# DearCaat/MHIM-MIL

Hardware: AMD Instinct MI355X
Metric: patch-instances/sec through MHIM fwd+bwd, N=10k D=1024 (higher is better)
Workload: dtype f32; 1 GPU; c2: MHIM(ABMIL) train step, one bag N=10000 D=1024 per GPU per step (teacher fwd + select + student fwd + bwd + Adam + EMA); rotating_bags_per_gpu=8, matrix_core_form=bf16x3, parallelism=dp1, launch=hipGraph replay, one graph per resident bag

## Files before the change

include/mhimx.h:

```cpp
#ifndef MHIMX_H
#define MHIMX_H

#include <stdint.h>

#ifdef __cplusplus
extern "C" {
#endif

#define MHIMX_VERSION 620

enum { MHIMX_ACT_NONE = 0, MHIMX_ACT_RELU = 1, MHIMX_ACT_GELU = 2, MHIMX_ACT_TANH = 3 };

enum { MHIMX_PREC_F32 = 0, MHIMX_PREC_F16S = 1, MHIMX_PREC_BF16X3 = 2 };

const char* mhimx_last_error(void);
int mhimx_version(void);


typedef struct {
  const float* A; int64_t lda; const int64_t* rows;
  const float* B; int64_t ldb;
  float* C; int64_t ldc;
  int64_t M, N, K;
  const float* bias;
  const float* rowv; const float* colv;
  float* pre; int64_t ldpre;
  int32_t act;
  float drop_p; uint64_t drop_seed; const uint8_t* drop_mask;
  int32_t accumulate;
  int32_t prec;
  const uint64_t* drop_tick;
  int32_t paired;
  float* ws; int64_t ws_floats;
  float* dact; int64_t lddact;
} mhimx_gemm_nt_args;
int mhimx_gemm_nt(void* stream, const mhimx_gemm_nt_args* a);

#define MHIMX_PROJ_MAX_HEADS 2
typedef struct {
  const float* wp;
  const float* bias;
  float* H; int64_t ldh;
  void* dact;
  float drop_p; uint64_t drop_seed; const uint8_t* drop_mask;
  const float* resid; int64_t ldr;
} mhimx_proj_head;
typedef struct {
  const float* wa16;
  const float* wc;
  int32_t act;
  int32_t C;
  float* s;
  float* cproj;
  float* pm; float* pl; float* pz;
  float* xch;
  uint32_t* gate;
} mhimx_proj_score;
int mhimx_pool_finalize(void* stream, const float* pm, const float* pl, const float* pz, int64_t G, int64_t E, float* stats, float* z,
                        const float* s, const float* cproj, const float* bp, int64_t C, int64_t M1, float* pscore);
int64_t mhimx_proj_score_parts(int64_t N);
int64_t mhimx_proj_score_xch_floats(int64_t N);
typedef struct {
  const float* X; int64_t ldx;
  int64_t N, D, E;
  int32_t act;
  int32_t n_heads;
  mhimx_proj_head head[MHIMX_PROJ_MAX_HEADS];
  const uint64_t* drop_tick;
  const mhimx_proj_score* score0;
} mhimx_bag_project_args;
int mhimx_bag_project(void* stream, const mhimx_bag_project_args* a);
int mhimx_bag_project_multi(void* stream, const mhimx_bag_project_args* bags, int32_t n_bags);

int mhimx_gemm_nn(void* stream, const mhimx_gemm_nt_args* a, float alpha, int32_t splits, float* ws );
int mhimx_gemm_batched(void* stream, int32_t mode, const mhimx_gemm_nt_args* args, int32_t batch, int64_t strideA,
                       int64_t strideB, int64_t strideC, float alpha, int32_t splits, float* ws);
int mhimx_bmm_affine(void* stream, int32_t mode, const mhimx_gemm_nt_args* args, int32_t batch, int64_t strideA, int64_t strideB,
                     int64_t strideC, float alpha, float ident);
int mhimx_bmm_affine2(void* stream, int32_t mode, const mhimx_gemm_nt_args* a, int32_t batch, int64_t strideA, int64_t strideB,
                      int64_t strideC, float alpha, float ident, float* C2, float alpha2, float ident2);
typedef struct {
  const void* A; const void* B; float* C; void* PN; void* PT; void* PN2; void* PT2; const float* D; const float* D2;
  float alpha, ident, alpha2, ident2, dscale, d2scale;
  int32_t kind;
} mhimx_bmm_step;
int mhimx_bmm_chain(void* stream, const mhimx_bmm_step* steps, int32_t stages, int32_t groups, uint32_t* counters);
int mhimx_bmm_affine_pair(void* stream, int32_t mode0, const mhimx_gemm_nt_args* a0, float alpha0, float ident0, int32_t mode1,
                          const mhimx_gemm_nt_args* a1, float alpha1, float ident1, int32_t batch, int64_t stride);

typedef struct {
  int32_t kind; int32_t accumulate;
  const float* parts; float* out;
  int64_t G, W, ld, K1, K2, ldo;
} mhimx_reduce_job;
#define MHIMX_REDUCE_MAX 16
#define MHIMX_SIDE_BYTES 512
typedef struct { int32_t pending; int32_t reserved; unsigned char blob[MHIMX_SIDE_BYTES]; } mhimx_side_work;
typedef struct { int32_t pending; int32_t reserved ;
                 unsigned char blob[128]; } mhimx_parked_gemm;
typedef struct { mhimx_reduce_job j[MHIMX_REDUCE_MAX]; int32_t n; mhimx_side_work side; mhimx_parked_gemm parked; mhimx_side_work pre; } mhimx_reduce_list;
int mhimx_reduce_flush(void* stream, mhimx_reduce_list* list);

typedef struct {
  const float* A; int64_t lda;
  const float* B; int64_t ldb; const int64_t* rows;
  float* C; int64_t ldc;
  int64_t M, K1, K2;
  int32_t splits; float* ws;
  int32_t accumulate;
  int32_t prec;
  int64_t ws_floats;
  mhimx_reduce_list* defer;
} mhimx_gemm_tn_args;
int mhimx_gemm_tn(void* stream, const mhimx_gemm_tn_args* a);

int mhimx_pair_planes(void* stream, const float* x, int64_t ldx, int64_t M, int64_t K, float* out);

#define MHIMX_PREP_MAX 32
typedef struct { int32_t kind; const float* in; float* out; int64_t R, C; } mhimx_prep_job;
int mhimx_prep_batch(void* stream, const mhimx_prep_job* jobs, int32_t n);

int mhimx_transpose(void* stream, const float* in, float* out, int64_t R, int64_t C);

typedef struct {
  int64_t E;
  int64_t A;
  int32_t act;
  int32_t gated;
  int32_t prec;
  const float* wa; const float* ba;
  const float* wb; const float* bb;
  const float* wc; const float* bc;
  const float* wa_frag;
  float gate_drop_p;
  uint64_t gate_drop_seed;
} mhimx_scorer;

typedef struct {
  const float* T1; int64_t M1; const float* T2; int64_t M2;
  float* s; float* stats; float* z;
  float* u_pre;
  const float* wp; int64_t C; float* cproj;
  void* ws; int64_t ws_bytes;
  const float* bp; float* pscore;
  const int64_t* rows1;
  const uint8_t* excl;
  const mhimx_prep_job* ride_jobs;
  int32_t n_ride_jobs;
  int32_t phase; int32_t tail_tokens;
  const void* ride_merge;
  const float* ride_X; int64_t ride_R; void* ride_ws; int64_t ride_ws_bytes;
  int32_t rode_merge;
  const float* tail_wa_t;
  int64_t tail_row0;
  int32_t no_backward;
} mhimx_pool_io;
int64_t mhimx_abmil_pool_ws_bytes(int64_t M, int64_t E, int64_t A, int32_t gated);
int mhimx_abmil_pool_fwd(void* stream, const mhimx_scorer* sc, mhimx_pool_io* io);

typedef struct {
  const float* g_z;
  float* dT1; float* dT2;
  float* d_wa; float* d_ba; float* d_wb; float* d_bb; float* d_wc; float* d_bc;
  const float* wa_t; const float* wb_t;
  int32_t accumulate;
  int32_t splits;
  mhimx_reduce_list* defer;
  const float* wa_t_frag;
  void* img; const void* img_dact; float* img_part; int64_t img_rows;
} mhimx_pool_grad;
int mhimx_abmil_pool_bwd(void* stream, const mhimx_scorer* sc, const mhimx_pool_io* io, const mhimx_pool_grad* g);

int mhimx_softmax_from_stats(void* stream, const float* s, const float* stats, float* attn, int64_t M);

int mhimx_lse_merge(void* stream, const float* parts, int64_t W, int64_t E, float* stats, float* z);

int mhimx_pseudo_score(void* stream, const float* s, const float* stats, const float* cproj, const float* bp,
                       float* score, float* attn_out, int64_t M, int64_t C);

int mhimx_layernorm_fwd(void* stream, const float* x, int64_t M, int64_t E, const float* w, const float* b, float* y, float* mean,
                        float* rstd);
int mhimx_layernorm_bwd(void* stream, const float* dy, const float* x, int64_t M, int64_t E, const float* w, const float* mean,
                        const float* rstd, float* dx, float* d_w, float* d_b, int32_t accumulate, float* ws);
int mhimx_layernorm_bwd_res(void* stream, const float* dy, const float* x, int64_t M, int64_t E, const float* w, const float* mean,
                            const float* rstd, const float* resid, float* dx, float* d_w, float* d_b, int32_t accumulate, float* ws);
int mhimx_dropout_apply(void* stream, const float* x, float* out, int64_t M, int64_t E, float p, uint64_t seed, const uint64_t* tick);
int mhimx_dropout_apply_proj(void* stream, const float* x, float* out, int64_t M, int64_t E, float p, uint64_t seed, const uint64_t* tick);
int mhimx_softmax_rows(void* stream, const float* x, float* y, int64_t R, int64_t L, float alpha);
int mhimx_softmax_rows_bwd(void* stream, const float* y, const float* dy, float* dx, int64_t R, int64_t L, float alpha);
int mhimx_landmark_mean(void* stream, const float* x, int64_t ldx, int64_t T, int64_t l, int64_t C, float* out);
int mhimx_landmark_mean_bwd(void* stream, const float* dout, int64_t T, int64_t l, int64_t C, float* dx, int64_t ldx, int32_t accumulate);
int mhimx_affine_ident(void* stream, const float* x, float* y, int64_t B, int64_t n, float a, float b);
int mhimx_axpby(void* stream, const float* x, float* y, int64_t n, float alpha, float beta);
int mhimx_pinv_init(void* stream, const float* a, int64_t B, int64_t n, float* z, float* stats, float* ws);
int mhimx_pinv_init_bwd(void* stream, const float* dz, const float* z0, const float* stats, int64_t B, int64_t n, float* da, float* ws);
int mhimx_resconv(void* stream, const float* v, int64_t ldv, const float* w, int64_t KS, int64_t dh, int64_t T, int64_t C, float* out,
                  int64_t ldo, int32_t accumulate, int32_t flip);
int64_t mhimx_resconv_dw_ws_floats(int64_t T, int64_t C, int64_t dh, int64_t KS);
int mhimx_resconv_dw(void* stream, const float* dout, int64_t ldo, const float* v, int64_t ldv, int64_t KS, int64_t dh, int64_t T,
                     int64_t C, float* dw, float* ws);
typedef struct mhimx_nys {
  const float* q; const float* k; const float* v;
  int64_t ld, T;
  const float* ql; const float* kl;
  int64_t ldl;
  float scale;
  float* ws;
  int64_t ws_floats;
} mhimx_nys;
int64_t mhimx_nys_ws_floats(int64_t T);
int mhimx_nys_a3v_fwd(void* stream, const mhimx_nys* a, float* a3v, float* lse3);
int mhimx_nys_out_fwd(void* stream, const mhimx_nys* a, const float* w2, float* out, int64_t ldo, float* lse1, int32_t accumulate);
int mhimx_nys_out_bwd(void* stream, const mhimx_nys* a, const float* w2, const float* dout, int64_t ldd, const float* lse1,
                      float* delta1, float* dq, int64_t lddq, float* dkl, int64_t lddl, float* dw2);
int mhimx_nys_a3v_bwd(void* stream, const mhimx_nys* a, const float* a3v, const float* da3v, const float* lse3, float* dk, float* dv,
                      int64_t lddk, int32_t accumulate_dv, float* dql, int64_t lddl);
int mhimx_nys_cls_attn(void* stream, const mhimx_nys* a, const float* lse3, const float* u, float* r);
int64_t mhimx_bn_ws_floats(int64_t M, int64_t C);
int mhimx_bn_fwd(void* stream, const float* x, int64_t M, int64_t C, const float* w, const float* b, float eps, int32_t training, float* mean,
                 float* rstd, float* var_out, float* y, float* ws);
int mhimx_bn_bwd(void* stream, const float* dy, const float* x, int64_t M, int64_t C, const float* w, const float* mean, const float* rstd,
                 int32_t training, float* dx, float* dw, float* db, float* ws);
int mhimx_sincos_add(void* stream, const float* x, const int64_t* pos_xy, int64_t N, int64_t C, float* out);
int mhimx_ppeg_combine(void* stream, const float* w7, const float* w5, const float* w3, const float* b7, const float* b5,
                       const float* b3, int64_t C, float* wc, float* bc);
int mhimx_ppeg_fwd(void* stream, const float* x, int64_t N, int64_t C, const float* wc, const float* bc, float* y,
                   int64_t grid );
int64_t mhimx_ppeg_bwd_ws_floats(int64_t N, int64_t C);
int mhimx_ppeg_bwd(void* stream, const float* dy, const float* x, int64_t N, int64_t C, const float* wc, float* dx, float* dwc, float* dbc,
                   float* ws, int64_t grid);
typedef struct { int64_t H, cell0, ncell, out0, out1; } mhimx_ppeg_band;
int64_t mhimx_ppeg_side(int64_t N, int64_t* wrapN);
int mhimx_ppeg_band_fwd(void* stream, const float* xb, const mhimx_ppeg_band* band, int64_t C, const float* wc, const float* bc, float* y);
int64_t mhimx_ppeg_band_bwd_ws_floats(int64_t n_out, int64_t C);
int mhimx_ppeg_band_bwd(void* stream, const float* dyb, const float* xb, const mhimx_ppeg_band* band, int64_t n_dw, int64_t C, const float* wc,
                        float* dx, float* dwc, float* dbc, float* ws);
int mhimx_scale_heads(void* stream, const float* v, int64_t ldv, const float* a, int64_t lda, int64_t dh, int64_t T, int64_t C, float* out);

int64_t mhimx_select_ws_bytes(int64_t N);
int mhimx_select_mask(void* stream, const float* score, int64_t N, int64_t k, int64_t n_sel, int32_t largest,
                      const int64_t* perm, const int64_t* other, int64_t n_other,
                      int64_t* mask_ids, int64_t* len_keep_dev, int64_t* topk_sorted ,
                      void* ws, int64_t ws_bytes);

int mhimx_select_rows(void* stream, const float* score, int64_t N, int64_t k, int64_t n_sel, int32_t largest,
                      uint64_t rand_seed, const uint64_t* tick, int64_t merge_R, int64_t* rows_out, int64_t* mask_ids,
                      void* ws, int64_t ws_bytes, int32_t merge_first );

int mhimx_select_rows_img(void* stream, const float* score, int64_t N, int64_t k, int64_t n_sel, int32_t largest, uint64_t rand_seed,
                          const uint64_t* tick, int64_t merge_R, int64_t* rows_out, int64_t* rows_img, int64_t img_merge_off, void* ws,
                          int64_t ws_bytes, int32_t merge_first);
int mhimx_vote_scores(void* stream, const float* attn, int64_t H, int64_t N, int64_t k, int32_t largest,
                      float* vote, void* ws, int64_t ws_bytes);

int mhimx_compose_ids(void* stream, const int64_t* a, const int64_t* b, int64_t* out, int64_t n);
int mhimx_random_perm(void* stream, int64_t n, uint64_t seed, const uint64_t* tick, const int64_t* src, int64_t* out);

typedef struct { int64_t row0, N, k, n_sel, merge_R, out0; uint64_t seed; } mhimx_select_bag;
int64_t mhimx_select_rows_many_ws_bytes(int32_t n_bags, const mhimx_select_bag* bags);
int mhimx_select_rows_many(void* stream, const float* score, int32_t n_bags, const mhimx_select_bag* bags, const uint64_t* tick,
                           int64_t* rows_out, void* ws, int64_t ws_bytes, int32_t merge_first);

typedef struct {
  int64_t E; int64_t k;
  int64_t heads; int64_t dim_head;
  const float* q_param;
  const float* ln_w; const float* ln_b;
  const float* wkv; const float* wq; const float* wo; const float* bo;
  const float* wkv_t; const float* wq_t; const float* wo_t;
  float mm;
  float drop_p; uint64_t drop_seed;
  int32_t prec;
  const uint64_t* drop_tick;
  const float* wkv_frag;
  const int64_t* x_rows;
  int32_t prepared;
  int64_t own_lo, own_n;
  float rep;
  int32_t rows_done;
} mhimx_merge;
int64_t mhimx_merge_ws_bytes(int64_t R, int64_t E, int64_t k, int64_t heads, int64_t dim_head);
int mhimx_merge_fwd(void* stream, const mhimx_merge* m, const float* X, int64_t R, float* z, float* q_new,
                    int32_t update_q, void* ws, int64_t ws_bytes);
typedef struct {
  float* d_ln_w; float* d_ln_b; float* d_wkv; float* d_wq; float* d_wo; float* d_bo;
  int32_t accumulate; int32_t splits;
  mhimx_reduce_list* defer;
} mhimx_merge_grad;
int64_t mhimx_merge_part_floats(void);
int mhimx_merge_fwd_part(void* stream, const mhimx_merge* m, const float* X, int64_t R, float* part, void* ws, int64_t ws_bytes);
int mhimx_merge_fwd_finish(void* stream, const mhimx_merge* m, const float* parts, int32_t W, int64_t R, float* z, float* q_new,
                           int32_t update_q, void* ws, int64_t ws_bytes);
int mhimx_merge_bwd(void* stream, const mhimx_merge* m, const float* X, int64_t R, const float* dz, float* dX,
                    const mhimx_merge_grad* g, void* ws, int64_t ws_bytes);
int mhimx_merge_bwd_park(const mhimx_merge* m, const float* X, int64_t R, const float* dz, float* dX, const mhimx_merge_grad* g, void* ws,
                         int64_t ws_bytes);

int mhimx_act_bwd(void* stream, float* dH, const float* H, const float* pre, int64_t M, int64_t E, int32_t act,
                  float drop_p, uint64_t drop_seed, const uint8_t* drop_mask, const int64_t* rows, float* colsum_out,
                  int32_t accumulate, void* ws, int64_t ws_bytes, const uint64_t* drop_tick);
int mhimx_mul_colsum(void* stream, float* dH, const float* dact, int64_t M, int64_t E, float* colsum_out, int32_t accumulate,
                     void* ws, int64_t ws_bytes, mhimx_reduce_list* defer );
int mhimx_rows_dpre(void* stream, const float* dH, const void* dact16, const int64_t* rows, int64_t L, int64_t E, float* dpre,
                    float* colsum_out, int32_t accumulate, void* ws, int64_t ws_bytes, mhimx_reduce_list* defer );
int64_t mhimx_wgrad_image_bytes(int64_t L, int64_t E);
int mhimx_rows_dpre_image(void* stream, const float* dH, const void* dact16, const int64_t* rows, int64_t L, int64_t E, void* img,
                          float* colsum_out, int32_t accumulate, void* ws, int64_t ws_bytes, mhimx_reduce_list* defer );
int mhimx_rows_dpre_image_c(void* stream, const float* dH_compact, const void* dact16, const int64_t* rows, int64_t L, int64_t E, void* img,
                            float* colsum_out, int32_t accumulate, void* ws, int64_t ws_bytes, mhimx_reduce_list* defer );
int mhimx_rows_dpre_image_k(void* stream, const float* dH, const void* dact16, const uint8_t* keep, int64_t N, int64_t E, void* img,
                            float* colsum_out, int32_t accumulate, void* ws, int64_t ws_bytes, mhimx_reduce_list* defer );
typedef struct {
  const void* img;
  const float* X; int64_t ldx; int64_t n_bag_rows;
  const int64_t* rows;
  int64_t L, E, D;
  float* C; int64_t ldc; int32_t accumulate;
  float* ws; int64_t ws_floats;
  mhimx_reduce_list* defer;
  int32_t ride_tail;
  const void* ximg;
} mhimx_bag_wgrad_args;
int64_t mhimx_wgrad_ws_floats(int64_t L, int64_t E, int64_t D);
int mhimx_bag_wgrad(void* stream, const mhimx_bag_wgrad_args* a);
int64_t mhimx_wgrad_multi_ws_floats(int64_t L, int64_t E, int64_t D, int32_t n_bags);
int mhimx_bag_wgrad_multi(void* stream, const mhimx_bag_wgrad_args* bags, int32_t n_bags);
int mhimx_shard_flags(void* stream, const int64_t* rows_all, int64_t R, int64_t Lk, int64_t lo, int64_t n, int64_t k_tokens,
                      int32_t tokens_live, uint8_t* excl);
int mhimx_shard_gather(void* stream, const float* H, int64_t E, const int64_t* rows, int64_t R, int64_t lo, int64_t n, float* out);
int mhimx_shard_scatter(void* stream, const float* dX, int64_t E, const int64_t* rows, int64_t R, int64_t lo, int64_t n, float* dH);
int mhimx_colsum(void* stream, const float* X, int64_t M, int64_t E, float* out, int32_t accumulate,
                 void* ws, int64_t ws_bytes);

int mhimx_head_fwd_bwd(void* stream, const float* z, const float* t, const float* wp, const float* bp,
                       const int64_t* label_dev, int64_t E, int64_t C, float temp_t, float main_alpha,
                       float aux_alpha, float inv_accum, float* logits, float* losses, float* g_z, float* d_wp,
                       float* d_bp, int32_t accumulate, const float* g_logits_in, const float* g_cl_in);

int mhimx_softmax_cols(void* stream, const float* x, float* y, int64_t M, int64_t C, float alpha);
int mhimx_softmax_cols_bwd(void* stream, const float* y, const float* dy, float* dx, int64_t M, int64_t C, float alpha);
int mhimx_colmax(void* stream, const float* x, int64_t M, int64_t C, float* vals, int64_t* idx);
int mhimx_rowmax(void* stream, const float* x, int64_t M, int64_t C, float* out);
int mhimx_dsmil_head(void* stream, const float* logits_bag, const float* logits_ins, const int64_t* label_dev, const float* Bs,
                     const float* Bt, int64_t C, int64_t V, float temp_t, float main_alpha, float aux_alpha, float inv_accum,
                     float* losses, float* g_logits_bag, float* g_logits_ins, float* g_B, const float* g_cl_in);

int mhimx_adam_ema(void* stream, float* p, const float* g, float* m, float* v, float* teacher, int64_t n_train,
                   int64_t n_all, int64_t step, float lr, float beta1, float beta2, float eps, float weight_decay,
                   float grad_scale, float ema_mm, int32_t zero_grad ,
                   const uint64_t* step_dev ,
                   const float* mm_table, int64_t mm_len );

typedef struct {
  float* p; float* g; float* m; float* v; float* teacher;
  int64_t n_train, n_all;
  int64_t step; const uint64_t* step_dev;
  float lr; const float* lr_table; int64_t lr_len;
  float beta1, beta2, eps, weight_decay, grad_scale;
  float ema_mm; const float* mm_table; int64_t mm_len;
  int32_t zero_grad;
  const float* g_extra; int64_t n_extra; int64_t extra_pitch;
  float clip_norm;
  float* ws; int64_t ws_floats;
  mhimx_reduce_list* fold;
  int64_t extra_lo;
  int32_t extra_only;
} mhimx_optim_args;
int mhimx_optim_step(void* stream, const mhimx_optim_args* a);

#define MHIMX_STEP_MAX_ROWS 262144
#define MHIMX_WINDOW_MAX 8
typedef struct {
  const float* w1; const float* b1;
  const float* wa; const float* wc;
  const float* wp; const float* bp;
  float* q;
  const float* ln_w; const float* ln_b;
  const float* wkv; const float* wq; const float* wo; const float* bo;
} mhimx_step_params;
typedef struct {
  float* w1; float* b1; float* wa; float* wc; float* wp; float* bp; float* ln_w; float* ln_b; float* wkv; float* wq; float* wo; float* bo;
} mhimx_step_grads;
typedef struct {
  int64_t D, E, A, C, k;
  int32_t act, da_act;
  int32_t attn2score;
  float drop_p_teacher, drop_p_student;
  float merge_drop_p, merge_mm;
  float temp_t, main_alpha, aux_alpha;
  mhimx_step_params student, teacher;
  mhimx_step_grads grad;
  float* p; float* g; float* m; float* v; float* p_teacher;
  int64_t n_train, n_all;
  float lr, beta1, beta2, eps, weight_decay, ema_mm;
  const float* mm_table; int64_t mm_len; const float* lr_table; int64_t lr_len;
  uint64_t* tick; uint64_t* opt_step;
  float* q_out;
  int32_t time_project;
  void* side_stream;
} mhimx_step_cfg;
typedef struct { int64_t k_top, n_sel, len_keep, Lk, R; } mhimx_step_counts;
int mhimx_step_counts_of(int64_t N, double mask_ratio_h, double mask_ratio_hr, double merge_ratio, mhimx_step_counts* out);
typedef struct { uint64_t drop_teacher, drop_student, select, mca; } mhimx_step_seeds;
typedef struct {
  int64_t total;
  int64_t logits, losses;
  int64_t score;
  int64_t rows_all;
  int64_t H_teacher, H_student;
  int64_t dact;
  int64_t z_teacher, z_student, g_z;
  int64_t dH;
} mhimx_step_layout;
int mhimx_step_layout_of(const mhimx_step_cfg* cfg, int64_t N, const mhimx_step_counts* cnt, mhimx_step_layout* out);
int mhimx_step_run(void* stream, const mhimx_step_cfg* cfg, const float* X, int64_t ldx, int64_t N, const int64_t* label_dev,
                   const mhimx_step_counts* cnt, const mhimx_step_seeds* seeds, int64_t host_step, void* ws, int64_t ws_bytes, int32_t update);
int mhimx_step_project_ms(float* ms_out, float* empty_ms_out, int32_t cap);
int mhimx_step_run_many(void* stream, const mhimx_step_cfg* cfg, int32_t n_bags, const float* const* X, const int64_t* ldx, const int64_t* N,
                        const int64_t* const* labels_dev, const mhimx_step_counts* cnt, const mhimx_step_seeds* seeds, int64_t host_step0,
                        void* ws, int64_t ws_bytes);

int mhimx_pure_step_layout_of(const mhimx_step_cfg* cfg, int64_t N, mhimx_step_layout* out);
int mhimx_pure_step_run(void* stream, const mhimx_step_cfg* cfg, const float* X, int64_t ldx, int64_t N, const int64_t* label_dev,
                        uint64_t drop_seed, int64_t host_step, void* ws, int64_t ws_bytes, int32_t update);
int mhimx_pure_step_run_many(void* stream, const mhimx_step_cfg* cfg, int32_t n_bags, const float* const* X, const int64_t* ldx, const int64_t* N,
                             const int64_t* const* labels_dev, const uint64_t* drop_seeds, int64_t host_step0, void* ws, int64_t ws_bytes);

typedef struct { int64_t total, bag0, bag_stride, grad_slab; mhimx_step_layout bag; } mhimx_window_layout;
int mhimx_window_layout_of(const mhimx_step_cfg* cfg, int32_t n_bags, int64_t N, const mhimx_step_counts* cnt, mhimx_window_layout* out);
int mhimx_window_run(void* stream, const mhimx_step_cfg* cfg, int32_t n_bags, const float* const* X, int64_t ldx, int64_t N,
                     const int64_t* const* labels_dev, const mhimx_step_counts* cnt, const mhimx_step_seeds* seeds, int64_t host_step, void* ws,
                     int64_t ws_bytes, int32_t update);
// ... 266 lines not shown
```

mhim_mil_amd/_lib.py:

```python
from __future__ import annotations

import ctypes as C
import os

HERE = os.path.dirname(os.path.abspath(__file__))
LIB_PATH = os.path.join(HERE, os.environ.get("MHIMX_LIB_NAME", "libmhimx.so"))

c_f32p = C.c_void_p
c_i64p = C.c_void_p
c_u8p = C.c_void_p

ABI_VERSION = 620

ACT = {None: 0, "none": 0, "identity": 0, "relu": 1, "gelu": 2, "tanh": 3}
PREC = {"f32": 0, "f16s": 1, "bf16x3": 2}


def act_code(name, allowed):
    n = name.lower() if isinstance(name, str) else None
    return ACT[n] if n in allowed else 0


class GemmNT(C.Structure):
    _fields_ = [("A", c_f32p), ("lda", C.c_int64), ("rows", c_i64p),
                ("B", c_f32p), ("ldb", C.c_int64),
                ("C", c_f32p), ("ldc", C.c_int64),
                ("M", C.c_int64), ("N", C.c_int64), ("K", C.c_int64),
                ("bias", c_f32p), ("rowv", c_f32p), ("colv", c_f32p),
                ("pre", c_f32p), ("ldpre", C.c_int64),
                ("act", C.c_int32),
                ("drop_p", C.c_float), ("drop_seed", C.c_uint64), ("drop_mask", c_u8p),
                ("accumulate", C.c_int32), ("prec", C.c_int32), ("drop_tick", C.c_void_p),
                ("paired", C.c_int32), ("ws", C.c_void_p), ("ws_floats", C.c_int64),
                ("dact", C.c_void_p), ("lddact", C.c_int64)]


class ProjHead(C.Structure):
    _fields_ = [("wp", c_f32p), ("bias", c_f32p), ("H", c_f32p), ("ldh", C.c_int64), ("dact", C.c_void_p),
                ("drop_p", C.c_float), ("drop_seed", C.c_uint64), ("drop_mask", c_u8p), ("resid", c_f32p), ("ldr", C.c_int64)]


class ProjScore(C.Structure):
    _fields_ = [("wa16", c_f32p), ("wc", c_f32p), ("act", C.c_int32), ("C", C.c_int32), ("s", c_f32p), ("cproj", c_f32p),
                ("pm", c_f32p), ("pl", c_f32p), ("pz", c_f32p), ("xch", c_f32p), ("gate", C.c_void_p)]


class BagProject(C.Structure):
    _fields_ = [("X", c_f32p), ("ldx", C.c_int64), ("N", C.c_int64), ("D", C.c_int64), ("E", C.c_int64),
                ("act", C.c_int32), ("n_heads", C.c_int32), ("head", ProjHead * 2), ("drop_tick", C.c_void_p), ("score0", C.c_void_p)]


class BagWgrad(C.Structure):
    _fields_ = [("img", C.c_void_p), ("X", c_f32p), ("ldx", C.c_int64), ("n_bag_rows", C.c_int64), ("rows", C.c_void_p),
                ("L", C.c_int64), ("E", C.c_int64), ("D", C.c_int64), ("C", c_f32p), ("ldc", C.c_int64), ("accumulate", C.c_int32),
                ("ws", c_f32p), ("ws_floats", C.c_int64), ("defer", C.c_void_p), ("ride_tail", C.c_int32), ("ximg", C.c_void_p)]


class PpegBand(C.Structure):
    _fields_ = [("H", C.c_int64), ("cell0", C.c_int64), ("ncell", C.c_int64), ("out0", C.c_int64), ("out1", C.c_int64)]


class PrepJob(C.Structure):
    _fields_ = [("kind", C.c_int32), ("inp", C.c_void_p), ("out", C.c_void_p), ("R", C.c_int64), ("C", C.c_int64)]


class ReduceJob(C.Structure):
    _fields_ = [("kind", C.c_int32), ("accumulate", C.c_int32), ("parts", c_f32p), ("out", c_f32p),
                ("G", C.c_int64), ("W", C.c_int64), ("ld", C.c_int64), ("K1", C.c_int64), ("K2", C.c_int64), ("ldo", C.c_int64)]


REDUCE_MAX = 16


SIDE_BYTES = 512


class SideWork(C.Structure):
    _fields_ = [("pending", C.c_int32), ("reserved", C.c_int32), ("blob", C.c_ubyte * SIDE_BYTES)]


class ParkedGemm(C.Structure):
    _fields_ = [("pending", C.c_int32), ("reserved", C.c_int32), ("blob", C.c_ubyte * 128)]


class ReduceListC(C.Structure):
    _fields_ = [("j", ReduceJob * REDUCE_MAX), ("n", C.c_int32), ("side", SideWork), ("parked", ParkedGemm), ("pre", SideWork)]


class GemmTN(C.Structure):
    _fields_ = [("A", c_f32p), ("lda", C.c_int64),
                ("B", c_f32p), ("ldb", C.c_int64), ("rows", c_i64p),
                ("C", c_f32p), ("ldc", C.c_int64),
                ("M", C.c_int64), ("K1", C.c_int64), ("K2", C.c_int64),
                ("splits", C.c_int32), ("ws", c_f32p),
                ("accumulate", C.c_int32), ("prec", C.c_int32), ("ws_floats", C.c_int64),
                ("defer", C.c_void_p)]


class Scorer(C.Structure):
    _fields_ = [("E", C.c_int64), ("A", C.c_int64), ("act", C.c_int32), ("gated", C.c_int32), ("prec", C.c_int32),
                ("wa", c_f32p), ("ba", c_f32p), ("wb", c_f32p), ("bb", c_f32p), ("wc", c_f32p), ("bc", c_f32p),
                ("wa_frag", c_f32p), ("gate_drop_p", C.c_float), ("gate_drop_seed", C.c_uint64)]


class PoolIO(C.Structure):
    _fields_ = [("T1", c_f32p), ("M1", C.c_int64), ("T2", c_f32p), ("M2", C.c_int64),
                ("s", c_f32p), ("stats", c_f32p), ("z", c_f32p), ("u_pre", c_f32p),
                ("wp", c_f32p), ("C", C.c_int64), ("cproj", c_f32p),
                ("ws", C.c_void_p), ("ws_bytes", C.c_int64), ("bp", c_f32p), ("pscore", c_f32p), ("rows1", c_i64p),
                ("excl", C.c_void_p), ("ride_jobs", C.c_void_p), ("n_ride_jobs", C.c_int32),
                ("phase", C.c_int32), ("tail_tokens", C.c_int32), ("ride_merge", C.c_void_p), ("ride_X", c_f32p), ("ride_R", C.c_int64),
                ("ride_ws", C.c_void_p), ("ride_ws_bytes", C.c_int64), ("rode_merge", C.c_int32), ("tail_wa_t", c_f32p), ("tail_row0", C.c_int64),
                ("no_backward", C.c_int32)]


class PoolGrad(C.Structure):
    _fields_ = [("g_z", c_f32p), ("dT1", c_f32p), ("dT2", c_f32p),
                ("d_wa", c_f32p), ("d_ba", c_f32p), ("d_wb", c_f32p), ("d_bb", c_f32p), ("d_wc", c_f32p),
                ("d_bc", c_f32p), ("wa_t", c_f32p), ("wb_t", c_f32p),
                ("accumulate", C.c_int32), ("splits", C.c_int32), ("defer", C.c_void_p), ("wa_t_frag", c_f32p),
                ("img", C.c_void_p), ("img_dact", C.c_void_p), ("img_part", c_f32p), ("img_rows", C.c_int64)]


class Merge(C.Structure):
    _fields_ = [("E", C.c_int64), ("k", C.c_int64), ("heads", C.c_int64), ("dim_head", C.c_int64),
                ("q_param", c_f32p), ("ln_w", c_f32p), ("ln_b", c_f32p),
                ("wkv", c_f32p), ("wq", c_f32p), ("wo", c_f32p), ("bo", c_f32p),
                ("wkv_t", c_f32p), ("wq_t", c_f32p), ("wo_t", c_f32p),
                ("mm", C.c_float), ("drop_p", C.c_float), ("drop_seed", C.c_uint64), ("prec", C.c_int32), ("drop_tick", C.c_void_p),
                ("wkv_frag", c_f32p), ("x_rows", c_i64p), ("prepared", C.c_int32), ("own_lo", C.c_int64), ("own_n", C.c_int64),
                ("rep", C.c_float), ("rows_done", C.c_int32)]


class MergeGrad(C.Structure):
    _fields_ = [("d_ln_w", c_f32p), ("d_ln_b", c_f32p), ("d_wkv", c_f32p), ("d_wq", c_f32p), ("d_wo", c_f32p),
                ("d_bo", c_f32p), ("accumulate", C.c_int32), ("splits", C.c_int32), ("defer", C.c_void_p)]


_P = C.c_void_p
_I64 = C.c_int64
_I32 = C.c_int32
_F = C.c_float
_U64 = C.c_uint64


class Nys(C.Structure):
    _fields_ = [("q", C.c_void_p), ("k", C.c_void_p), ("v", C.c_void_p), ("ld", C.c_int64), ("T", C.c_int64),
                ("ql", C.c_void_p), ("kl", C.c_void_p), ("ldl", C.c_int64), ("scale", C.c_float),
                ("ws", C.c_void_p), ("ws_floats", C.c_int64)]


class BmmStep(C.Structure):
    _fields_ = [("A", C.c_void_p), ("B", C.c_void_p), ("C", C.c_void_p), ("PN", C.c_void_p), ("PT", C.c_void_p),
                ("PN2", C.c_void_p), ("PT2", C.c_void_p), ("D", C.c_void_p), ("D2", C.c_void_p), ("alpha", C.c_float), ("ident", C.c_float),
                ("alpha2", C.c_float), ("ident2", C.c_float), ("dscale", C.c_float), ("d2scale", C.c_float), ("kind", C.c_int32)]


class OptimArgs(C.Structure):
    _fields_ = [("p", C.c_void_p), ("g", C.c_void_p), ("m", C.c_void_p), ("v", C.c_void_p), ("teacher", C.c_void_p),
                ("n_train", C.c_int64), ("n_all", C.c_int64), ("step", C.c_int64), ("step_dev", C.c_void_p),
                ("lr", C.c_float), ("lr_table", C.c_void_p), ("lr_len", C.c_int64),
                ("beta1", C.c_float), ("beta2", C.c_float), ("eps", C.c_float), ("weight_decay", C.c_float), ("grad_scale", C.c_float),
                ("ema_mm", C.c_float), ("mm_table", C.c_void_p), ("mm_len", C.c_int64), ("zero_grad", C.c_int32),
                ("g_extra", C.c_void_p), ("n_extra", C.c_int64), ("extra_pitch", C.c_int64), ("clip_norm", C.c_float),
                ("ws", C.c_void_p), ("ws_floats", C.c_int64), ("fold", C.c_void_p), ("extra_lo", C.c_int64), ("extra_only", C.c_int32)]


class StepParams(C.Structure):
    _fields_ = [(n, C.c_void_p) for n in ("w1", "b1", "wa", "wc", "wp", "bp", "q", "ln_w", "ln_b", "wkv", "wq", "wo", "bo")]


class StepGrads(C.Structure):
    _fields_ = [(n, C.c_void_p) for n in ("w1", "b1", "wa", "wc", "wp", "bp", "ln_w", "ln_b", "wkv", "wq", "wo", "bo")]


class StepCfg(C.Structure):
    _fields_ = [("D", C.c_int64), ("E", C.c_int64), ("A", C.c_int64), ("C", C.c_int64), ("k", C.c_int64),
                ("act", C.c_int32), ("da_act", C.c_int32), ("attn2score", C.c_int32),
                ("drop_p_teacher", C.c_float), ("drop_p_student", C.c_float), ("merge_drop_p", C.c_float), ("merge_mm", C.c_float),
                ("temp_t", C.c_float), ("main_alpha", C.c_float), ("aux_alpha", C.c_float),
                ("student", StepParams), ("teacher", StepParams), ("grad", StepGrads),
                ("p", C.c_void_p), ("g", C.c_void_p), ("m", C.c_void_p), ("v", C.c_void_p), ("p_teacher", C.c_void_p),
                ("n_train", C.c_int64), ("n_all", C.c_int64),
                ("lr", C.c_float), ("beta1", C.c_float), ("beta2", C.c_float), ("eps", C.c_float), ("weight_decay", C.c_float), ("ema_mm", C.c_float),
                ("mm_table", C.c_void_p), ("mm_len", C.c_int64), ("lr_table", C.c_void_p), ("lr_len", C.c_int64),
                ("tick", C.c_void_p), ("opt_step", C.c_void_p), ("q_out", C.c_void_p), ("time_project", C.c_int32), ("side_stream", C.c_void_p)]


class StepCounts(C.Structure):
    _fields_ = [("k_top", C.c_int64), ("n_sel", C.c_int64), ("len_keep", C.c_int64), ("Lk", C.c_int64), ("R", C.c_int64)]


class StepSeeds(C.Structure):
    _fields_ = [("drop_teacher", C.c_uint64), ("drop_student", C.c_uint64), ("select", C.c_uint64), ("mca", C.c_uint64)]


class StepLayout(C.Structure):
    _fields_ = [(n, C.c_int64) for n in ("total", "logits", "losses", "score", "rows_all", "H_teacher", "H_student", "dact", "z_teacher",
                                        "z_student", "g_z", "dH")]


class WindowLayout(C.Structure):
    _fields_ = [("total", C.c_int64), ("bag0", C.c_int64), ("bag_stride", C.c_int64), ("grad_slab", C.c_int64), ("bag", StepLayout)]


WINDOW_MAX = 8
STEP_MAX_ROWS = 262144


class InferCfg(C.Structure):
    _fields_ = [("D", C.c_int64), ("E", C.c_int64), ("A", C.c_int64), ("C", C.c_int64), ("act", C.c_int32), ("da_act", C.c_int32),
                ("p", StepParams)]


class InferBag(C.Structure):
    _fields_ = [("X", c_f32p), ("ldx", C.c_int64), ("N", C.c_int64)]


class InferOut(C.Structure):
    _fields_ = [(n, c_f32p) for n in ("logits", "z", "stats", "score", "attn", "loss")]


class InferDsmilCfg(C.Structure):
    _fields_ = [("D", C.c_int64), ("E", C.c_int64), ("C", C.c_int64), ("act", C.c_int32), ("cls_attn", C.c_int32), ("no_norm", C.c_int32),
                ("pad", C.c_int32)] + [(n, c_f32p) for n in ("w1", "b1", "wi", "bi", "wq0", "bq0", "wq2", "bq2", "wv", "bv", "wfcc", "bfcc")]


class InferDsmilOut(C.Structure):
    _fields_ = [(n, c_f32p) for n in ("logits_bag", "logits_ins", "logits", "B")] + [("crit", C.c_void_p)] + [(n, c_f32p) for n in ("attn", "loss")]


INFER_MAX = 32


class TransmilLayer(C.Structure):
    _fields_ = [(n, c_f32p) for n in ("ln_w", "ln_b", "w_qkv", "w_out", "b_out", "conv_w")]


class InferTransmilCfg(C.Structure):
    _fields_ = ([("D", C.c_int64), ("C", C.c_int64), ("act", C.c_int32), ("pad", C.c_int32)]
                + [(n, c_f32p) for n in ("w1", "b1", "cls_token")] + [("layer", TransmilLayer * 2)]
                + [(n, c_f32p) for n in ("w7", "w5", "w3", "b7", "b5", "b3", "norm_w", "norm_b", "wp", "bp")])


class InferTransmilLayout(C.Structure):
    _fields_ = ([("n_bags", C.c_int64), ("tokens", C.c_int64)] + [(n, C.c_int64 * INFER_MAX) for n in ("tok0", "T", "pad")]
                + [(n, C.c_int64 * 2) for n in ("x", "qkv", "lm", "a2", "z", "a3v", "lse3", "w2", "out", "y")]
                + [("cls", C.c_int64), ("total", C.c_int64)])
INFER_MAX_ROWS = 4194304
X_F32, X_F16, X_BF16 = 0, 1, 2

TOPK_MAX_K = 4096

SURV_MAX_N = 16777216
CINDEX_MAX_N = 4194304
CINDEX_MAX_B = 65535
CINDEX_MAX_BN = 134217728


class TopkSeg(C.Structure):
    _fields_ = [("row0", C.c_int64), ("N", C.c_int64)]


class SelectBag(C.Structure):
    _fields_ = [(n, C.c_int64) for n in ("row0", "N", "k", "n_sel", "merge_R", "out0")] + [("seed", C.c_uint64)]


PURE_WINDOW_MAX = 32
PURE_WINDOW_MAX_ROWS = 524288


class PureWindowBag(C.Structure):
    _fields_ = [("X", c_f32p), ("ldx", C.c_int64), ("N", C.c_int64), ("label_dev", C.c_void_p), ("drop_seed", C.c_uint64)]


class PureWindowLayout(C.Structure):
    _fields_ = [(n, C.c_int64) for n in ("total", "rows", "logits", "losses", "H", "dact", "s", "stats", "z", "g_z")] + [
        ("row0", C.c_int64 * PURE_WINDOW_MAX)]


DSMIL_WINDOW_MAX = 32
DSMIL_WINDOW_MAX_ROWS = 262144
_DSMIL_NAMES = ("w1", "b1", "wi", "bi", "wq0", "bq0", "wq2", "bq2", "wv", "bv", "wfcc", "bfcc")

# ... 247 lines not shown
```

mhim_mil_amd/csrc/mca2.hip:

```cpp
#include <math.h>
#include <string.h>

#include "mca2_rows.hpp"

namespace mhimx {

int64_t merge2_part_floats() { return M2_PART_FLOATS; }
int64_t merge2_rows_tiles(int64_t R) { return cdiv(R, m2_tile_rows(R)); }
int64_t merge2_ws_bytes(int64_t R, int64_t k) {
  Arena ar(nullptr, 0);
  return merge2_ws_layout(ar, R, k, nullptr);
}

bool merge2_ok(const mhimx_merge* m, int64_t R) {
  return m->E == M2_E && m->heads == M2_H && m->dim_head == M2_DH && m->k >= 1 && m->heads * m->k <= M2_JP && R >= 1 && R <= 32768 &&
         m->prec != MHIMX_PREC_F32 && aligned16(m->wq) && aligned16(m->wkv) && aligned16(m->wo) && aligned16(m->ln_w) && aligned16(m->ln_b) &&
         aligned16(m->q_param);
}

__global__ __launch_bounds__(M2_THREADS) void merge2_prep_kernel(Merge2PrepArgs a) {
  __shared__ __attribute__((aligned(16))) float lds[6 * M2_E + 6 * 64];
  merge2_prep_body((int)blockIdx.x, lds, a.q_param, a.ln_w, a.ln_b, a.wq, a.wkv, a.k, a.scale, a.w);
}

template <int RT>
__global__ __launch_bounds__(M2_THREADS) void merge2_rows_fwd_kernel(const float* __restrict__ X, const int64_t* __restrict__ xrows, int64_t R,
                                                                    const float* __restrict__ ln_w, const float* __restrict__ ln_b, int J,
                                                                    float drop_p, uint64_t seed0, const uint64_t* __restrict__ tick, Merge2Ws w, BagBatch bb) {
  extern __shared__ __attribute__((aligned(16))) float m2sm[];
  if (blockIdx.z) {
    MHIMX_BAG(X); MHIMX_BAG(xrows);
    seed0 = bag_mca_seed(seed0, bb);
    bag_move(w, bb);
  }
  merge2_rows_fwd_body<RT>((int)blockIdx.x, m2sm, X, xrows, R, ln_w, ln_b, J, drop_p, seed0, tick, w);
}

template <int MODE>
__global__ __launch_bounds__(M2_THREADS) void merge2_partials_kernel(M2Parts in, int live_only, const float* __restrict__ ln_w,
                                                                    const float* __restrict__ ln_b, float* __restrict__ out,
                                                                    float* __restrict__ stats, float* __restrict__ raw_stats, BagBatch bb) {
  __shared__ float lds[M2_PARTIALS_LDS];
  if (blockIdx.z) {
    in.pm = bag_ptr(in.pm, bb); in.pl = bag_ptr(in.pl, bb); in.psd = bag_ptr(in.psd, bb); in.y = bag_ptr(in.y, bb);
    MHIMX_BAG(out); MHIMX_BAG(stats); MHIMX_BAG(raw_stats);
  }
  merge2_partials_body<MODE>((int)blockIdx.x, lds, in, live_only != 0, ln_w, ln_b, out, stats, raw_stats);
}

__global__ __launch_bounds__(M2_THREADS) void merge2_o_kernel(const float* __restrict__ wkv, int k, Merge2Ws w, BagBatch bb) {
  __shared__ __attribute__((aligned(16))) float ys[6 * M2_E];
  bag_move(w, bb);
  const int tid = threadIdx.x;
  const int h = blockIdx.x >> 2, qd = blockIdx.x & 3;
  M2HeadRows wr;
  m2_head_rows_load<16>(wkv + (int64_t)(M2_I + h * 64 + qd * 16) * M2_E, wr);
  m2_zero_tail(ys, k);
  for (int idx = tid; idx < k * (M2_E / 4); idx += M2_THREADS)
    reinterpret_cast<m2_f4*>(ys)[idx] = reinterpret_cast<const m2_f4*>(w.Y + (int64_t)h * k * M2_E)[idx];
  __syncthreads();
  m2_head_dots_use<16>(wr, ys, k, nullptr, 16, w.O + h * 64 + qd * 16);
}

__global__ __launch_bounds__(M2_THREADS) void merge2_bwd_pre_kernel(const float* __restrict__ dz, const float* __restrict__ wo_t,
                                                                   const float* __restrict__ wkv, int k, float drop_p, uint64_t seed0,
                                                                   const uint64_t* __restrict__ tick, float* __restrict__ d_bo, int accumulate,
                                                                   Merge2Ws w, float rep, BagBatch bb) {
  __shared__ __attribute__((aligned(16))) float lds[M2_BWD_PRE_LDS];
  if (blockIdx.z) {
    MHIMX_BAG(dz); MHIMX_BAG(wo_t); MHIMX_BAG(d_bo);
    seed0 = bag_mca_seed(seed0, bb);
    bag_move(w, bb);
  }
  merge2_bwd_pre_body((int)blockIdx.x, lds, dz, wo_t, wkv, k, drop_p, seed0, tick, d_bo, accumulate, w, rep);
}

template <int RT>
__global__ __launch_bounds__(M2_THREADS) void merge2_rows_bwd_kernel(const float* __restrict__ X, const int64_t* __restrict__ xrows, int64_t R,
                                                                    const float* __restrict__ ln_w, const float* __restrict__ ln_b, int J,
                                                                    float drop_p, uint64_t seed0, const uint64_t* __restrict__ tick,
                                                                    float* __restrict__ dX, Merge2Ws w, BagBatch bb) {
  extern __shared__ __attribute__((aligned(16))) float m2sm[];
  if (blockIdx.z) {
    MHIMX_BAG(X); MHIMX_BAG(xrows); MHIMX_BAG(dX);
    seed0 = bag_mca_seed(seed0, bb);
    bag_move(w, bb);
  }
  merge2_rows_bwd_body<RT>((int)blockIdx.x, m2sm, X, xrows, R, ln_w, ln_b, J, drop_p, seed0, tick, dX, w);
}

__global__ __launch_bounds__(M2_THREADS) void merge2_grads1_kernel(Merge2Side a, BagBatch bb) {
  __shared__ __attribute__((aligned(16))) float lds[M2_GRADS1_LDS];
  bag_move(a, bb);
  merge2_grads1_body((int)blockIdx.x, lds, a);
}

__global__ __launch_bounds__(M2_THREADS) void merge2_grads2_kernel(Merge2Side a, BagBatch bb) {
  __shared__ __attribute__((aligned(16))) float lds[M2_GRADS2_LDS];
  bag_move(a, bb);
  merge2_grads2_body((int)blockIdx.x, lds, a);
}

int mca_out(hipStream_t st, const float* O, const float* wo, const float* bo, int k, int E, int I, float p, uint64_t seed0, const uint64_t* tick,
            float* z, const float* q, float* q_new, float mm);
int reduce_parts2(hipStream_t st, const float* part0, const float* part1, int G, int W, int ld, float* out0, float* out1, int accumulate);

int merge2_side_launch(hipStream_t st, int stage, const Merge2Side& sd) {
  if (stage == 1) hipLaunchKernelGGL(merge2_partials_kernel<0>, bgrid((unsigned)(sd.J * 4)), dim3(M2_THREADS), 0, st, m2_parts_tiles(sd.w, sd.w.upart),
                                     sd.w.own_n > 0 ? 1 : 0, sd.ln_w, sd.ln_b, const_cast<float*>(sd.U), (float*)nullptr, (float*)nullptr, cur_batch());
  else if (stage == 2) hipLaunchKernelGGL(merge2_grads1_kernel, bgrid(M2_GRADS1_BLOCKS), dim3(M2_THREADS), 0, st, sd, cur_batch());
  else hipLaunchKernelGGL(merge2_grads2_kernel, bgrid(M2_GRADS2_BLOCKS), dim3(M2_THREADS), 0, st, sd, cur_batch());
  MHIMX_LAUNCH_CHECK();
  return 0;
}
int merge2_side_finish(hipStream_t st, mhimx_side_work* side, int upto_stage) {
  Merge2Side sd;
  while (side->pending != 0 && side->pending <= upto_stage) {
    memcpy(&sd, side->blob, sizeof(sd));
    if (int r = merge2_side_launch(st, side->pending, sd)) return r;
    side->pending = side->pending == 3 ? 0 : side->pending + 1;
  }
  return 0;
}

int merge2_fwd_rows_args(const mhimx_merge* m, const float* X, int64_t R, void* ws, int64_t ws_bytes, M2RowsFwd* out) {
  if (!m || !X || !merge2_ok(m, R) || !m->prepared || m->own_n != 0) return 1;
  Arena ar(ws, ws_bytes);
  Merge2Ws w;
  merge2_ws_layout(ar, R, m->k, &w);
  MHIMX_CHECK_ARG(ar.ok(), "merge rows rider: workspace too small (%lld < %lld)", (long long)ws_bytes, (long long)ar.off);
  if (w.rt != 16) return 1;
  w.own_lo = 0; w.own_n = 0;
  *out = M2RowsFwd{X, m->x_rows, R, m->ln_w, m->ln_b, M2_H * (int)m->k, m->drop_p, m->drop_seed, m->drop_tick, w};
  return 0;
}

static int merge2_fwd_rows(hipStream_t st, const mhimx_merge* m, const float* X, int64_t R, void* ws, int64_t ws_bytes, Merge2Ws* wout) {
  Arena ar(ws, ws_bytes);
  Merge2Ws w;
  merge2_ws_layout(ar, R, m->k, &w);
  MHIMX_CHECK_ARG(ar.ok(), "merge_fwd: workspace too small (%lld < %lld)", (long long)ws_bytes, (long long)ar.off);
  MHIMX_CHECK_ARG(m->own_n >= 0 && (m->own_n == 0 || m->x_rows), "merge_fwd: a shard's row range needs the bag-level row list (x_rows)");
  w.own_lo = m->own_n > 0 ? m->own_lo : 0;
  w.own_n = m->own_n;
  const int k = (int)m->k, J = M2_H * k;
  const float scale = 1.0f / sqrtf((float)M2_DH);
  if (m->rows_done) {
    *wout = w;
    return 0;
  }
  if (!m->prepared) {
    hipLaunchKernelGGL(merge2_prep_kernel, dim3(64), dim3(M2_THREADS), 0, st, Merge2PrepArgs{m->q_param, m->ln_w, m->ln_b, m->wq, m->wkv, k, scale, w});
    MHIMX_LAUNCH_CHECK();
  }
  MHIMX_ONCE_PER_DEVICE(MHIMX_HIP(hipFuncSetAttribute((const void*)merge2_rows_fwd_kernel<32>, hipFuncAttributeMaxDynamicSharedMemorySize, (int)m2_fwd_smem(32)));
                        MHIMX_HIP(hipFuncSetAttribute((const void*)merge2_rows_fwd_kernel<16>, hipFuncAttributeMaxDynamicSharedMemorySize, (int)m2_fwd_smem(16))));
  if (w.rt == 16)
    hipLaunchKernelGGL(merge2_rows_fwd_kernel<16>, bgrid((unsigned)w.T), dim3(M2_THREADS), m2_fwd_smem(16), st, X, m->x_rows, R, m->ln_w, m->ln_b, J, m->drop_p,
                       m->drop_seed, m->drop_tick, w, cur_batch());
  else
    hipLaunchKernelGGL(merge2_rows_fwd_kernel<32>, bgrid((unsigned)w.T), dim3(M2_THREADS), m2_fwd_smem(32), st, X, m->x_rows, R, m->ln_w, m->ln_b, J, m->drop_p,
                       m->drop_seed, m->drop_tick, w, cur_batch());
  MHIMX_LAUNCH_CHECK();
  *wout = w;
  return 0;
}
static int merge2_fwd_tail(hipStream_t st, const mhimx_merge* m, float* z, float* q_new, int update_q, const Merge2Ws& w) {
  const int k = (int)m->k;
  hipLaunchKernelGGL(merge2_o_kernel, bgrid(M2_H * 4), dim3(M2_THREADS), 0, st, m->wkv, k, w, cur_batch());
  MHIMX_LAUNCH_CHECK();
  return mca_out(st, w.O, m->wo, m->bo, k, M2_E, M2_I, m->drop_p, m->drop_seed + 0x9E3779B97F4A7C15ull, m->drop_tick, z, m->q_param,
                 update_q ? q_new : (float*)nullptr, m->mm);
}

int merge2_fwd(hipStream_t st, const mhimx_merge* m, const float* X, int64_t R, float* z, float* q_new, int update_q, void* ws, int64_t ws_bytes) {
  MHIMX_CHECK_ARG(!update_q || q_new, "merge_fwd: update_q needs q_new");
  MHIMX_CHECK_ARG(m->own_n == 0, "merge_fwd: a shard of an instance-sharded bag runs mhimx_merge_fwd_part + mhimx_merge_fwd_finish");
  Merge2Ws w;
  if (int r = merge2_fwd_rows(st, m, X, R, ws, ws_bytes, &w)) return r;
  const int J = M2_H * (int)m->k;
  hipLaunchKernelGGL(merge2_partials_kernel<1>, bgrid((unsigned)(J * 4)), dim3(M2_THREADS), 0, st, m2_parts_tiles(w, w.ypart), 0, m->ln_w, m->ln_b, w.Y,
                     w.stats, (float*)nullptr, cur_batch());
  MHIMX_LAUNCH_CHECK();
  return merge2_fwd_tail(st, m, z, q_new, update_q, w);
}

int merge2_fwd_part(hipStream_t st, const mhimx_merge* m, const float* X, int64_t R, float* part, void* ws, int64_t ws_bytes) {
  MHIMX_CHECK_ARG(part && aligned16(part), "merge_fwd_part: null / unaligned output block");
  Merge2Ws w;
  if (int r = merge2_fwd_rows(st, m, X, R, ws, ws_bytes, &w)) return r;
  const int J = M2_H * (int)m->k;
  hipLaunchKernelGGL(merge2_partials_kernel<2>, dim3((unsigned)(J * 4)), dim3(M2_THREADS), 0, st, m2_parts_tiles(w, w.ypart), 0, m->ln_w, m->ln_b,
                     part + 3 * M2_JP, (float*)nullptr, part, BagBatch{});
  MHIMX_LAUNCH_CHECK();
  return 0;
}
int merge2_fwd_finish(hipStream_t st, const mhimx_merge* m, const float* parts, int W, int64_t R, float* z, float* q_new, int update_q, void* ws,
                      int64_t ws_bytes) {
  MHIMX_CHECK_ARG(parts && W >= 1 && W <= 256 && z, "merge_fwd_finish: 1..256 shard blocks");
  MHIMX_CHECK_ARG(!update_q || q_new, "merge_fwd_finish: update_q needs q_new");
  Arena ar(ws, ws_bytes);
  Merge2Ws w;
  merge2_ws_layout(ar, R, m->k, &w);
  MHIMX_CHECK_ARG(ar.ok(), "merge_fwd_finish: workspace too small");
  const int J = M2_H * (int)m->k;
  hipLaunchKernelGGL(merge2_partials_kernel<1>, dim3((unsigned)(J * 4)), dim3(M2_THREADS), 0, st, m2_parts_shards(parts, W), 0, m->ln_w, m->ln_b, w.Y,
                     w.stats, (float*)nullptr, BagBatch{});
  MHIMX_LAUNCH_CHECK();
  return merge2_fwd_tail(st, m, z, q_new, update_q, w);
}

int gemm_tn_rider(hipStream_t st, const mhimx_gemm_tn_args& g, const Merge2Side* rider, int stage);

static int merge2_side_of(const mhimx_merge* m, const float* X, int64_t R, const float* dz, float* dX, const mhimx_merge_grad* gr, void* ws,
                          int64_t ws_bytes, Merge2Side* out) {
  Arena ar(ws, ws_bytes);
  Merge2Ws w;
  merge2_ws_layout(ar, R, m->k, &w);
  MHIMX_CHECK_ARG(ar.ok(), "merge_bwd: workspace too small");
  MHIMX_CHECK_ARG(m->own_n >= 0 && (m->own_n == 0 || m->x_rows), "merge_bwd: a shard's row range needs the bag-level row list (x_rows)");
  w.own_lo = m->own_n > 0 ? m->own_lo : 0;
  w.own_n = m->own_n;
  MHIMX_CHECK_ARG(m->wo_t && aligned16(m->wo_t), "merge_bwd: transposed to_out weight missing");
  const int k = (int)m->k, J = M2_H * k;
  Merge2Side sd = {};
  sd.w = w; sd.dz = dz; sd.U = w.aq; sd.ln_w = m->ln_w; sd.ln_b = m->ln_b; sd.wkv = m->wkv; sd.wq = m->wq; sd.q_param = m->q_param; sd.wo_t = m->wo_t;
  sd.d_wkv = gr->d_wkv; sd.d_wo = gr->d_wo; sd.d_wq = gr->d_wq; sd.d_ln_w = gr->d_ln_w; sd.d_ln_b = gr->d_ln_b; sd.d_bo = gr->d_bo; sd.tick = m->drop_tick;
  sd.oseed = m->drop_seed + 0x9E3779B97F4A7C15ull; sd.scale = 1.0f / sqrtf((float)M2_DH); sd.drop_p = m->drop_p; sd.k = k; sd.accumulate = gr->accumulate;
  sd.J = J;
  sd.rep = m->own_n > 0 ? m->rep : 1.f;
  sd.X = X; sd.xrows = m->x_rows; sd.R = R; sd.dX = dX; sd.seed0 = m->drop_seed;
  *out = sd;
  return 0;
}

int merge2_bwd_park(const mhimx_merge* m, const float* X, int64_t R, const float* dz, float* dX, const mhimx_merge_grad* gr, void* ws, int64_t ws_bytes) {
  if (!gr->defer || gr->defer->pre.pending != 0) return 0;
  Merge2Side sd;
  if (int r = merge2_side_of(m, X, R, dz, dX, gr, ws, ws_bytes, &sd)) return r;
  static_assert(sizeof(Merge2Side) <= sizeof(gr->defer->pre.blob), "Merge2Side must fit mhimx_reduce_list.pre");
  memcpy(gr->defer->pre.blob, &sd, sizeof(sd));
  gr->defer->pre.pending = 1;
  return 0;
}

int merge2_bwd(hipStream_t st, const mhimx_merge* m, const float* X, int64_t R, const float* dz, float* dX, const mhimx_merge_grad* gr, void* ws,
               int64_t ws_bytes) {
  Merge2Side sd;
  if (int r = merge2_side_of(m, X, R, dz, dX, gr, ws, ws_bytes, &sd)) return r;
  const Merge2Ws& w = sd.w;
  const int k = sd.k, J = sd.J;
  const int acc = gr->accumulate;
  const uint64_t oseed = sd.oseed;
  bool pre_done = false, rows_done = false;
  if (gr->defer && gr->defer->pre.pending) {
    pre_done = gr->defer->pre.pending == 2;
    gr->defer->pre.pending = 0;
  }
  if (gr->defer && gr->defer->parked.pending) {
    mhimx_gemm_tn_args pg;
    memcpy(&pg, gr->defer->parked.blob, sizeof(pg));
    gr->defer->parked.pending = 0;
    if (pre_done) {
      const int rc = gemm_tn_rider(st, pg, &sd, 4);
      if (rc < 0) return rc;
      rows_done = rc == 1;
    } else {
      const int rc = gemm_tn_rider(st, pg, pre_done ? nullptr : &sd, 0);
      if (rc < 0) return rc;
      pre_done = pre_done || rc == 1;
    }
  }
  if (!pre_done) {
    hipLaunchKernelGGL(merge2_bwd_pre_kernel, bgrid(M2_BWD_PRE_BLOCKS), dim3(M2_THREADS), 0, st, dz, m->wo_t, m->wkv, k, m->drop_p, oseed, m->drop_tick, gr->d_bo, acc, w, sd.rep, cur_batch());
    MHIMX_LAUNCH_CHECK();
  }
  if (!rows_done) {
    MHIMX_ONCE_PER_DEVICE(MHIMX_HIP(hipFuncSetAttribute((const void*)merge2_rows_bwd_kernel<32>, hipFuncAttributeMaxDynamicSharedMemorySize, (int)m2_bwd_smem(32)));
                          MHIMX_HIP(hipFuncSetAttribute((const void*)merge2_rows_bwd_kernel<16>, hipFuncAttributeMaxDynamicSharedMemorySize, (int)m2_bwd_smem(16))));
    if (w.rt == 16)
      hipLaunchKernelGGL(merge2_rows_bwd_kernel<16>, bgrid((unsigned)w.T), dim3(M2_THREADS), m2_bwd_smem(16), st, X, m->x_rows, R, m->ln_w, m->ln_b, J, m->drop_p,
                         m->drop_seed, m->drop_tick, dX, w, cur_batch());
    else
      hipLaunchKernelGGL(merge2_rows_bwd_kernel<32>, bgrid((unsigned)w.T), dim3(M2_THREADS), m2_bwd_smem(32), st, X, m->x_rows, R, m->ln_w, m->ln_b, J, m->drop_p,
                         m->drop_seed, m->drop_tick, dX, w, cur_batch());
    MHIMX_LAUNCH_CHECK();
  }
  if (gr->defer && gr->defer->side.pending == 0) {
    memcpy(gr->defer->side.blob, &sd, sizeof(sd));
    gr->defer->side.pending = 1;
  } else {
    for (int stage = 1; stage <= 3; ++stage)
      if (int r = merge2_side_launch(st, stage, sd)) return r;
  }
  return 0;
}

}

namespace mhimx {
int merge2_prep_args(const mhimx_merge* m, int64_t R, void* ws, int64_t ws_bytes, Merge2PrepArgs* out) {
  MHIMX_CHECK_ARG(m && merge2_ok(m, R), "prep_batch: the Merge preparation job needs the projection-free form (E = 512, 8 x 64, k <= 6, R <= 32768)");
  Arena ar(ws, ws_bytes);
  Merge2Ws w;
  merge2_ws_layout(ar, R, m->k, &w);
  MHIMX_CHECK_ARG(ar.ok(), "prep_batch: Merge workspace too small (%lld < %lld)", (long long)ws_bytes, (long long)ar.off);
  *out = Merge2PrepArgs{m->q_param, m->ln_w, m->ln_b, m->wq, m->wkv, (int)m->k, 1.0f / sqrtf((float)M2_DH), w};
  return 0;
}
}
```

mhim_mil_amd/csrc/rows.hip:

```cpp
#include <math.h>
#include <string.h>

#include "mca2_rows.hpp"
#include "reduce_jobs.hpp"

namespace mhimx {

int gemm_nt(hipStream_t st, const mhimx_gemm_nt_args& g);
int gemm_tn(hipStream_t st, const mhimx_gemm_tn_args& g);
bool scorer_fused_ok(int64_t E, int64_t A, int gated, int prec, const float* T, const float* wa, const float* wp, int64_t C);
int scorer_fused_fwd(hipStream_t st, const float* T, int64_t M, const float* wa, const float* wa_frag, const float* ba, int act, const float* wc,
                     const float* bc, const float* wp, int C, float* u_pre, float* s_out, float* cproj, float* pm, float* pl,
                     float* pz, int max_parts, const int64_t* rows, const uint8_t* excl, const mhimx_prep_job* ride_jobs, int n_ride_jobs,
                     const void* merge_rows);
int merge2_fwd_rows_args(const mhimx_merge* m, const float* X, int64_t R, void* ws, int64_t ws_bytes, M2RowsFwd* out);
int prep_batch(hipStream_t st, const mhimx_prep_job* jobs, int n);
int scorer_fused_bwd(hipStream_t st, const float* T, int64_t M, const float* u_pre, const float* s_in, const float* stats,
                     const float* g_z, const float* z, const float* wc, int act, const float* wa_t, const float* wa_t_frag, float* du,
                     float* dT, float* dwc_part, float* dbc_part, int max_parts, const int64_t* rows, const void* pre_side, int64_t gate_row0,
                     void* img, const void* img_dact, float* img_part, int64_t img_rows);

constexpr int ROWS_THREADS = 256;
constexpr int MAX_PART = 512;
constexpr int TN_SLABS = 128;

MHIMX_DEV float sigmoidf_(float x) { return 1.f / (1.f + __expf(-x)); }

constexpr int FWD_WAVES = 16;
template <int EPL>
__global__ __launch_bounds__(64 * FWD_WAVES) void score_rows_fwd_kernel(
    const float* __restrict__ T, int64_t M, int E, int A, int act, int gated, const float* __restrict__ u_pre,
    const float* __restrict__ wc, const float* __restrict__ bc, const float* __restrict__ wp, int C,
    float* __restrict__ s_out, float* __restrict__ cproj, float* __restrict__ pm, float* __restrict__ pl,
    float* __restrict__ pz, float gdrop_p, uint64_t gdrop_seed, int64_t row0 ) {
  extern __shared__ __attribute__((aligned(16))) float sm[];
  constexpr int NWV = FWD_WAVES;
  const int lane = threadIdx.x & 63, wave = threadIdx.x >> 6;
  const int ldu = A * (1 + gated);
  const float bias_c = bc ? bc[0] : 0.f;

  float mw = -INFINITY, lw = 0.f, zacc[EPL];
#pragma unroll
  for (int q = 0; q < EPL; ++q) zacc[q] = 0.f;

  for (int64_t n = (int64_t)blockIdx.x * NWV + wave; n < M; n += (int64_t)gridDim.x * NWV) {
    const float* up = u_pre + n * ldu;
    float part = 0.f;
    const bool gdrop = gated && gdrop_p > 0.f;
    const uint32_t rkey = gdrop ? drop_row_key(gdrop_seed, (uint64_t)(row0 + n)) : 0u;
    const float ginv = gdrop ? 1.f / (1.f - gdrop_p) : 1.f;
    for (int j = lane; j < A; j += 64) {
      float u = act_fwd(up[j], act);
      if (gated) {
        float sg = sigmoidf_(up[A + j]);
        if (gdrop) {
          u = drop_keep_k(rkey, (uint32_t)j, gdrop_p) ? u * ginv : 0.f;
          sg = drop_keep_k(rkey, (uint32_t)(A + j), gdrop_p) ? sg * ginv : 0.f;
        }
        u *= sg;
      }
      part += wc[j] * u;
    }
    const float s = wave_sum(part) + bias_c;
    const float* h = T + n * (int64_t)E;
    float hv[EPL];
#pragma unroll
    for (int q = 0; q < EPL; ++q) hv[q] = h[lane + 64 * q];
    if (wp) {
      for (int c = 0; c < C; ++c) {
        float d = 0.f;
#pragma unroll
        for (int q = 0; q < EPL; ++q) d += hv[q] * wp[c * E + lane + 64 * q];
        d = wave_sum(d);
        if (lane == 0) cproj[n * C + c] = d;
      }
    }
    if (lane == 0) s_out[n] = s;
    if (s > mw) {
      const float sc = (mw == -INFINITY) ? 0.f : __expf(mw - s);
      lw = lw * sc + 1.f;
#pragma unroll
      for (int q = 0; q < EPL; ++q) zacc[q] = zacc[q] * sc + hv[q];
      mw = s;
    } else {
      const float p = __expf(s - mw);
      lw += p;
#pragma unroll
      for (int q = 0; q < EPL; ++q) zacc[q] += p * hv[q];
    }
  }
  float* zs = sm;
  float* ms = sm + NWV * E;
  float* ls = ms + NWV;
#pragma unroll
  for (int q = 0; q < EPL; ++q) zs[wave * E + lane + 64 * q] = zacc[q];
  if (lane == 0) { ms[wave] = mw; ls[wave] = lw; }
  __syncthreads();
  float mb = ms[0];
#pragma unroll
  for (int i = 1; i < NWV; ++i) mb = fmaxf(mb, ms[i]);
  float w[NWV];
#pragma unroll
  for (int i = 0; i < NWV; ++i) w[i] = (ms[i] == -INFINITY) ? 0.f : __expf(ms[i] - mb);
  for (int e = threadIdx.x; e < E; e += 64 * NWV) {
    float a = 0.f;
#pragma unroll
    for (int i = 0; i < NWV; ++i) a += zs[i * E + e] * w[i];
    pz[(int64_t)blockIdx.x * E + e] = a;
  }
  if (threadIdx.x == 0) {
    float l = 0.f;
#pragma unroll
    for (int i = 0; i < NWV; ++i) l += ls[i] * w[i];
    pm[blockIdx.x] = mb;
    pl[blockIdx.x] = l;
  }
}

constexpr int FIN_THREADS = 1024;
__global__ __launch_bounds__(FIN_THREADS) void pool_finalize_kernel(const float* __restrict__ pm, const float* __restrict__ pl,
                                                                     const float* __restrict__ pz, int G, int E,
                                                                     float* __restrict__ stats, float* __restrict__ z,
                                                                     const float* __restrict__ s, const float* __restrict__ cproj,
                                                                     const float* __restrict__ bp, int C, int64_t M1,
                                                                     float* __restrict__ pscore, BagBatch bb) {
  __shared__ float red[16];
  __shared__ float wgt[2 * MAX_PART];
  __shared__ float acc16[16][64];
  if (blockIdx.z) {
    MHIMX_BAG(pm); MHIMX_BAG(pl); MHIMX_BAG(pz); MHIMX_BAG(stats); MHIMX_BAG(z); MHIMX_BAG(s); MHIMX_BAG(cproj); MHIMX_BAG(pscore);
  }
  const int lane = threadIdx.x & 63, wave = threadIdx.x >> 6;
  const int b1 = threadIdx.x;
  const float pm1 = b1 < G ? pm[b1] : -INFINITY, pl1 = b1 < G ? pl[b1] : 0.f;
  float m = wave_max(pm1);
  if (lane == 0) red[wave] = m;
  __syncthreads();
  float mx = red[0];
#pragma unroll
  for (int w = 1; w < 16; ++w) mx = fmaxf(mx, red[w]);
  __syncthreads();
  float lp = 0.f;
  if (b1 < G) {
    const float w = (pm1 == -INFINITY) ? 0.f : __expf(pm1 - mx);
    wgt[b1] = w;
    lp = pl1 * w;
  }
  lp = wave_sum(lp);
  if (lane == 0) red[wave] = lp;
  __syncthreads();
  float L = 0.f;
#pragma unroll
  for (int w = 0; w < 16; ++w) L += red[w];
  const int zblocks = (E + 63) / 64;
  if ((int)blockIdx.x >= zblocks) {
    const float invL = 1.f / L, b0 = bp ? bp[0] : 0.f;
    const int nb = (int)gridDim.x - zblocks;
    for (int64_t n = (int64_t)((int)blockIdx.x - zblocks) * FIN_THREADS + threadIdx.x; n < M1; n += (int64_t)nb * FIN_THREADS) {
      const float an = __expf(s[n] - mx) * invL;
      float cm = -INFINITY;
      for (int c = 0; c < C; ++c) cm = fmaxf(cm, an * cproj[n * C + c] + b0);
      float den = 0.f;
      for (int c = 0; c < C; ++c) den += expf((an * cproj[n * C + c] + b0) - cm);
      pscore[n] = 1.f / den;
    }
    return;
  }
  const int e = blockIdx.x * 64 + lane;
  float acc = 0.f;
  if (e < E) {
#pragma unroll 8
    for (int b = wave; b < G; b += 16) acc += pz[(int64_t)b * E + e] * wgt[b];
  }
  acc16[wave][lane] = acc;
  __syncthreads();
  if (wave == 0 && e < E) {
    float a = 0.f;
#pragma unroll
    for (int w = 0; w < 16; ++w) a += acc16[w][lane];
    z[e] = a / L;
  }
  if (blockIdx.x == 0 && threadIdx.x == 0) { stats[0] = mx; stats[1] = L; }
}

constexpr int FIN_MAXTOK = 6;
#ifdef MHIMX_FT_PROF
__device__ unsigned long long ft_prof[16];
#define FT_STAMP(i) do { __syncthreads(); if (threadIdx.x == 0 && blockIdx.x == 0) ft_prof[i] = wall_clock64(); } while (0)
#else
#define FT_STAMP(i)
#endif
__global__ __launch_bounds__(FIN_THREADS) void pool_finalize_tok_kernel(const float* __restrict__ pm, const float* __restrict__ pl,
                                                                         const float* __restrict__ pz, int G, int E, float* __restrict__ stats,
                                                                         float* __restrict__ z, const float* __restrict__ T,
                                                                         const int64_t* __restrict__ rows_tail, int64_t row0, int K,
                                                                         const float* __restrict__ wa, const float* __restrict__ wa_t,
                                                                         const float* __restrict__ ba, const float* __restrict__ wc,
                                                                         const float* __restrict__ bc, int A, int act,
                                                                         float* __restrict__ u_pre_tail, float* __restrict__ s_tail, BagBatch bb) {
  if (blockIdx.z) {
    MHIMX_BAG(pm); MHIMX_BAG(pl); MHIMX_BAG(pz); MHIMX_BAG(stats); MHIMX_BAG(z); MHIMX_BAG(T); MHIMX_BAG(rows_tail); MHIMX_BAG(wa_t); MHIMX_BAG(u_pre_tail);
    MHIMX_BAG(s_tail);
  }
  __shared__ float red[16];
  __shared__ float wgt[2 * MAX_PART];
  __shared__ float acc16[16][64];
  __shared__ __attribute__((aligned(16))) float tks[FIN_MAXTOK][512];
  __shared__ float up[8][FIN_MAXTOK][128];
  __shared__ float us[FIN_MAXTOK][128];
  __shared__ float stok[8];
  const int tid = threadIdx.x, lane = tid & 63, wave = tid >> 6;
  FT_STAMP(0);
  const float pm1 = tid < G ? pm[tid] : -INFINITY, pl1 = tid < G ? pl[tid] : 0.f;
  const int e = blockIdx.x * 64 + lane;
  float pzv[8];
#pragma unroll
  for (int q = 0; q < 8; ++q) {
    const int b = wave + 16 * q;
    pzv[q] = (e < E && b < G) ? pz[(int64_t)b * E + e] : 0.f;
  }
  for (int idx = tid; idx < FIN_MAXTOK * (E / 4); idx += FIN_THREADS) {
    const int i = idx / (E / 4), c4 = idx - i * (E / 4);
    float4 v = make_float4(0.f, 0.f, 0.f, 0.f);
    if (i < K) {
      const int64_t r = rows_tail ? rows_tail[i] : row0 + i;
      v = reinterpret_cast<const float4*>(T + r * E)[c4];
    }
    reinterpret_cast<float4*>(&tks[i][0])[c4] = v;
  }
  if (wa_t && A == 128 && E == 512) {
    const int a = tid & 127, ch = tid >> 7;
    const float* wp = wa_t + (int64_t)(ch * 64) * A + a;
    float acc[FIN_MAXTOK];
#pragma unroll
    for (int i = 0; i < FIN_MAXTOK; ++i) acc[i] = 0.f;
    float wv[64];
#pragma unroll
    for (int u = 0; u < 64; ++u) wv[u] = wp[(int64_t)u * A];
    asm volatile("s_waitcnt vmcnt(0)" ::: "memory");
    __syncthreads();
    FT_STAMP(1);
#pragma unroll
    for (int u4 = 0; u4 < 64; u4 += 4) {
#pragma unroll
      for (int i = 0; i < FIN_MAXTOK; ++i) {
        const float4 tv = *reinterpret_cast<const float4*>(&tks[i][ch * 64 + u4]);
        acc[i] += tv.x * wv[u4] + tv.y * wv[u4 + 1] + tv.z * wv[u4 + 2] + tv.w * wv[u4 + 3];
      }
    }
#pragma unroll
    for (int i = 0; i < FIN_MAXTOK; ++i) up[ch][i][a] = acc[i];
    __syncthreads();
    if (tid < K * 128) {
      const int i = tid >> 7, aa = tid & 127;
      float v = ((up[0][i][aa] + up[1][i][aa]) + (up[2][i][aa] + up[3][i][aa])) + ((up[4][i][aa] + up[5][i][aa]) + (up[6][i][aa] + up[7][i][aa]));
      us[i][aa] = v + (ba ? ba[aa] : 0.f);
    }
  } else {
    float4 w0[8], w1[8];
#pragma unroll
    for (int q = 0; q < 8; ++q) {
      const int a = wave * 8 + q;
      const float* wr = wa + (int64_t)(a < A ? a : 0) * E + lane * 8;
      w0[q] = *reinterpret_cast<const float4*>(wr);
      w1[q] = *reinterpret_cast<const float4*>(wr + 4);
    }
    __syncthreads();
#pragma unroll
    for (int q = 0; q < 8; ++q) {
      const int a = wave * 8 + q;
      for (int i = 0; i < K; ++i) {
        const float4 t0 = *reinterpret_cast<const float4*>(&tks[i][lane * 8]), t1 = *reinterpret_cast<const float4*>(&tks[i][lane * 8 + 4]);
        float d = t0.x * w0[q].x + t0.y * w0[q].y + t0.z * w0[q].z + t0.w * w0[q].w + t1.x * w1[q].x + t1.y * w1[q].y + t1.z * w1[q].z + t1.w * w1[q].w;
        d = wave_sum(d);
        if (lane == 0 && a < A) us[i][a] = d + (ba ? ba[a] : 0.f);
      }
    }
  }
  __syncthreads();
  FT_STAMP(2);
  if (blockIdx.x == 0)
    for (int idx = tid; idx < K * A; idx += FIN_THREADS) u_pre_tail[idx] = us[idx / A][idx % A];
  if (wave < K) {
    float v = 0.f;
    for (int a = lane; a < A; a += 64) v += wc[a] * act_fwd(us[wave][a], act);
    v = wave_sum(v) + (bc ? bc[0] : 0.f);
    if (lane == 0) {
      stok[wave] = v;
      if (blockIdx.x == 0) s_tail[wave] = v;
    }
  }
  FT_STAMP(3);
  float m = wave_max(pm1);
  if (lane == 0) red[wave] = m;
  __syncthreads();
  float mx = red[0];
#pragma unroll
  for (int w = 1; w < 16; ++w) mx = fmaxf(mx, red[w]);
  for (int i = 0; i < K; ++i) mx = fmaxf(mx, stok[i]);
  __syncthreads();
  float lp = 0.f;
  if (tid < G) {
    const float w = (pm1 == -INFINITY) ? 0.f : __expf(pm1 - mx);
    wgt[tid] = w;
    lp = pl1 * w;
  }
  lp = wave_sum(lp);
  if (lane == 0) red[wave] = lp;
  __syncthreads();
  float L = 0.f;
#pragma unroll
  for (int w = 0; w < 16; ++w) L += red[w];
  float wt[FIN_MAXTOK];
#pragma unroll
  for (int i = 0; i < FIN_MAXTOK; ++i) {
    wt[i] = i < K ? __expf(stok[i] - mx) : 0.f;
    L += wt[i];
  }
  FT_STAMP(4);
  float acc = 0.f;
  if (e < E) {
#pragma unroll
    for (int q = 0; q < 8; ++q)
      if (wave + 16 * q < G) acc += pzv[q] * wgt[wave + 16 * q];
#pragma unroll 8
    for (int b = wave + 128; b < G; b += 16) acc += pz[(int64_t)b * E + e] * wgt[b];
  }
  acc16[wave][lane] = acc;
  __syncthreads();
  if (wave == 0 && e < E) {
    float a = 0.f;
#pragma unroll
    for (int w = 0; w < 16; ++w) a += acc16[w][lane];
#pragma unroll
    for (int i = 0; i < FIN_MAXTOK; ++i)
      if (i < K) a += wt[i] * tks[i][e];
    z[e] = a / L;
  }
  if (blockIdx.x == 0 && tid == 0) { stats[0] = mx; stats[1] = L; }
  FT_STAMP(5);
}

template <int EPL>
__global__ __launch_bounds__(ROWS_THREADS) void score_rows_bwd_kernel(
    const float* __restrict__ T, int64_t M, int E, int A, int act, int gated, const float* __restrict__ u_pre,
    const float* __restrict__ wc, const float* __restrict__ s_in, const float* __restrict__ stats,
    const float* __restrict__ g_z, const float* __restrict__ z, float* __restrict__ du, float* __restrict__ attn,
    float* __restrict__ dwc_part, float* __restrict__ dbc_part, float gdrop_p, uint64_t gdrop_seed, int64_t row0) {
  extern __shared__ __attribute__((aligned(16))) float sm[];
  const int lane = threadIdx.x & 63, wave = threadIdx.x >> 6;
  const int ldu = A * (1 + gated);
  float gz[EPL];
  float c0 = 0.f;
#pragma unroll
  for (int q = 0; q < EPL; ++q) {
    gz[q] = g_z[lane + 64 * q];
    c0 += gz[q] * z[lane + 64 * q];
  }
  c0 = wave_sum(c0);
  const float mx = stats[0], invL = 1.f / stats[1];
  constexpr int MAXJ = 8;
  float dwc[MAXJ];
#pragma unroll
  for (int i = 0; i < MAXJ; ++i) dwc[i] = 0.f;
  float dbc = 0.f;

  for (int64_t n = (int64_t)blockIdx.x * 4 + wave; n < M; n += (int64_t)gridDim.x * 4) {
    const float* h = T + n * (int64_t)E;
    float gh = 0.f;
#pragma unroll
    for (int q = 0; q < EPL; ++q) gh += gz[q] * h[lane + 64 * q];
    gh = wave_sum(gh);
    const float an = __expf(s_in[n] - mx) * invL;
    const float ds = an * (gh - c0);
    if (lane == 0) attn[n] = an;
    dbc += ds;
    const float* up = u_pre + n * ldu;
    float* dp = du + n * ldu;
    const bool gdrop = gated && gdrop_p > 0.f;
    const uint32_t rkey = gdrop ? drop_row_key(gdrop_seed, (uint64_t)(row0 + n)) : 0u;
    const float ginv = gdrop ? 1.f / (1.f - gdrop_p) : 1.f;
#pragma unroll
    for (int i = 0; i < MAXJ; ++i) {
      const int j = lane + 64 * i;
      if (j < A) {
        const float a = up[j];
        const float ya = act_fwd(a, act);
        const float ga = act_grad(a, ya, act);
        if (gated) {
          const float sg = sigmoidf_(up[A + j]);
          const float ma = gdrop ? (drop_keep_k(rkey, (uint32_t)j, gdrop_p) ? ginv : 0.f) : 1.f;
          const float mb = gdrop ? (drop_keep_k(rkey, (uint32_t)(A + j), gdrop_p) ? ginv : 0.f) : 1.f;
          dp[j] = ds * wc[j] * (sg * mb) * ga * ma;
          dp[A + j] = ds * wc[j] * (ya * ma) * sg * (1.f - sg) * mb;
          dwc[i] += ds * (ya * ma) * (sg * mb);
        } else {
          dp[j] = ds * wc[j] * ga;
          dwc[i] += ds * ya;
        }
      }
    }
  }
  float* ws = sm;
  float* bs = sm + 4 * A;
#pragma unroll
  for (int i = 0; i < MAXJ; ++i) {
    const int j = lane + 64 * i;
    if (j < A) ws[wave * A + j] = dwc[i];
  }
  if (lane == 0) bs[wave] = dbc;
  __syncthreads();
  for (int j = threadIdx.x; j < A; j += ROWS_THREADS)
    dwc_part[(int64_t)blockIdx.x * A + j] = ws[j] + ws[A + j] + ws[2 * A + j] + ws[3 * A + j];
  if (threadIdx.x == 0) dbc_part[blockIdx.x] = bs[0] + bs[1] + bs[2] + bs[3];
}

constexpr int RP_THREADS = 1024;
__global__ __launch_bounds__(RP_THREADS) void reduce_parts_kernel(const float* __restrict__ part, int G, int W, int ld,
                                                                   float* __restrict__ out, int accumulate) {
  __shared__ float red[32][33];
  const int c = threadIdx.x & 31, rg = threadIdx.x >> 5;
  for (int j0 = blockIdx.x * 32; j0 < W; j0 += gridDim.x * 32) {
    const int j = j0 + c;
    float acc = 0.f;
    if (j < W) {
#pragma unroll 8
      for (int b = rg; b < G; b += 32) acc += part[(int64_t)b * ld + j];
    }
    red[rg][c] = acc;
    __syncthreads();
    if (rg == 0 && j < W) {
      float v = 0.f;
#pragma unroll
      for (int q = 0; q < 32; ++q) v += red[q][c];
      out[j] = accumulate ? out[j] + v : v;
    }
    __syncthreads();
  }
}

int reduce_parts_now(hipStream_t st, const float* part, int64_t G, int64_t W, int64_t ld, float* out, int accumulate) {
  MHIMX_CHECK_ARG(cur_batch().n == 0, "reduce: a bag-batched launch queues its reductions (mhimx_reduce_list full?)");
  hipLaunchKernelGGL(reduce_parts_kernel, dim3((unsigned)cdiv(W, 32)), dim3(RP_THREADS), 0, st, part, (int)G, (int)W, (int)ld, out, accumulate);
  MHIMX_LAUNCH_CHECK();
  return 0;
}

struct ReduceJobs { ReduceTable t; int side_blocks; Merge2Side side; };
__global__ __launch_bounds__(RP_THREADS) void reduce_batch_kernel(ReduceJobs rj, BagBatch bb) {
  if ((int)blockIdx.x < rj.side_blocks) {
    __shared__ __attribute__((aligned(16))) float side_lds[M2_GRADS2_LDS];
    Merge2Side side = rj.side;
    bag_move(side, bb);
    if (threadIdx.x < M2_THREADS) merge2_side_stage(3, (int)blockIdx.x, side_lds, side);
    return;
  }
  __shared__ float red[32][33];
  reduce_jobs_block<RP_THREADS, true>(rj.t, (int)blockIdx.x - rj.side_blocks, red, bb);
}

__global__ __launch_bounds__(RP_THREADS) void reduce_parts2_kernel(const float* __restrict__ part0, const float* __restrict__ part1,
                                                                    int G, int W, int ld, float* __restrict__ out0,
                                                                    float* __restrict__ out1, int accumulate) {
  __shared__ float red[32][33];
  const float* part = blockIdx.y ? part1 : part0;
  float* out = blockIdx.y ? out1 : out0;
  const int c = threadIdx.x & 31, rg = threadIdx.x >> 5;
  for (int j0 = blockIdx.x * 32; j0 < W; j0 += gridDim.x * 32) {
    const int j = j0 + c;
    float acc = 0.f;
    if (j < W) {
#pragma unroll 8
      for (int b = rg; b < G; b += 32) acc += part[(int64_t)b * ld + j];
    }
    red[rg][c] = acc;
    __syncthreads();
    if (rg == 0 && j < W) {
      float v = 0.f;
#pragma unroll
      for (int q = 0; q < 32; ++q) v += red[q][c];
      out[j] = accumulate ? out[j] + v : v;
    }
    __syncthreads();
  }
}

__global__ void softmax_from_stats_kernel(const float* __restrict__ s, const float* __restrict__ stats,
                                          float* __restrict__ attn, int64_t M, BagBatch bb) {
  if (blockIdx.z) { MHIMX_BAG(s); MHIMX_BAG(stats); MHIMX_BAG(attn); }
  const float mx = stats[0], invL = 1.f / stats[1];
  for (int64_t n = (int64_t)blockIdx.x * blockDim.x + threadIdx.x; n < M; n += (int64_t)gridDim.x * blockDim.x)
    attn[n] = __expf(s[n] - mx) * invL;
// ... 269 lines not shown
  if ((int)blockIdx.x < side_blocks) {
    __shared__ float side_lds[M2_PARTIALS_LDS];
    merge2_side_stage(1, (int)blockIdx.x, side_lds, side);
    return;
  }
  const int bid = (int)blockIdx.x - side_blocks;
  typedef _Float16 h4v __attribute__((ext_vector_type(4)));
  const int e4 = E / 4;
  const int64_t mb = (int64_t)bid * chunk;
  const int64_t me = mb + chunk < L ? mb + chunk : L;
  for (int c = threadIdx.x; c < e4; c += 256) {
    f4v cs = f4v{0.f, 0.f, 0.f, 0.f};
    for (int64_t m = mb; m < me; ++m) {
      const int64_t r = rows ? rows[m] : m;
      const h4v d = reinterpret_cast<const h4v*>(dact + r * E)[c];
      const f4v g = reinterpret_cast<const f4v*>(dH + r * E)[c] * f4v{(float)d[0], (float)d[1], (float)d[2], (float)d[3]};
      reinterpret_cast<f4v*>(dpre + m * E)[c] = g;
      cs += g;
    }
    if (part) *(reinterpret_cast<f4v*>(part + (int64_t)bid * E) + c) = cs;
  }
}

__global__ __launch_bounds__(1024) void colmax_kernel(const float* __restrict__ x, int64_t M, int C, float* __restrict__ vals,
                                                      int64_t* __restrict__ idx) {
  __shared__ float bv[16][16];
  __shared__ int64_t bi[16][16];
  const int lane = threadIdx.x & 63, wave = threadIdx.x >> 6;
  for (int c = 0; c < C; ++c) {
    float best = -INFINITY;
    int64_t arg = 0;
    for (int64_t m = threadIdx.x; m < M; m += 1024) {
      const float v = x[m * C + c];
      if (v > best) { best = v; arg = m; }
    }
#pragma unroll
    for (int o = 32; o > 0; o >>= 1) {
      const float ov = __shfl_xor(best, o, 64);
      const int64_t oi = __shfl_xor(arg, o, 64);
      if (ov > best || (ov == best && oi < arg)) { best = ov; arg = oi; }
    }
    if (lane == 0) { bv[c][wave] = best; bi[c][wave] = arg; }
  }
  __syncthreads();
  if (threadIdx.x < C) {
    const int c = threadIdx.x;
    float best = bv[c][0];
    int64_t arg = bi[c][0];
    for (int w = 1; w < 16; ++w)
      if (bv[c][w] > best || (bv[c][w] == best && bi[c][w] < arg)) { best = bv[c][w]; arg = bi[c][w]; }
    vals[c] = best;
    idx[c] = arg;
  }
}
__global__ void rowmax_kernel(const float* __restrict__ x, int64_t M, int C, float* __restrict__ out) {
  for (int64_t m = (int64_t)blockIdx.x * blockDim.x + threadIdx.x; m < M; m += (int64_t)gridDim.x * blockDim.x) {
    float v = x[m * C];
    for (int c = 1; c < C; ++c) v = fmaxf(v, x[m * C + c]);
    out[m] = v;
  }
}

__global__ void colsum_part_kernel(const float* __restrict__ X, int64_t M, int E, int64_t chunk, float* __restrict__ part) {
  const int e = blockIdx.x * blockDim.x + threadIdx.x;
  if (e >= E) return;
  const int64_t mb = (int64_t)blockIdx.y * chunk;
  const int64_t me = mb + chunk < M ? mb + chunk : M;
  float acc = 0.f;
#pragma unroll 8
  for (int64_t m = mb; m < me; ++m) acc += X[m * (int64_t)E + e];
  part[(int64_t)blockIdx.y * E + e] = acc;
}

__global__ void compose_ids_kernel(const int64_t* __restrict__ a, const int64_t* __restrict__ b, int64_t* __restrict__ out, int64_t n) {
  for (int64_t i = (int64_t)blockIdx.x * blockDim.x + threadIdx.x; i < n; i += (int64_t)gridDim.x * blockDim.x) out[i] = a[b[i]];
}

static int grid_for_ln(int64_t M) {
  int64_t g = cdiv(M, 4);
  if (g < 1) g = 1;
  if (g > MAX_PART) g = MAX_PART;
  return (int)g;
}

static int grid_for_rows(int64_t M) {
  int64_t g = cdiv(M, 20);
  if (g < 1) g = 1;
  if (g > MAX_PART) g = MAX_PART;
  return (int)g;
}

struct PoolWs {
  float *pm, *pl, *pz, *attn, *du, *dwc_part, *dbc_part, *u_pre, *tn_ws, *nt_ws;
};

static int64_t pool_ws_layout(Arena& ar, int64_t M, int64_t E, int64_t A, int gated, PoolWs* w) {
  const int64_t G = 2 * MAX_PART;
  PoolWs t;
  t.pm = ar.take<float>(G);
  t.pl = ar.take<float>(G);
  t.pz = ar.take<float>(G * E);
  t.attn = ar.take<float>(M);
  t.du = ar.take<float>(M * A * (1 + gated));
  t.dwc_part = ar.take<float>(G * A);
  t.dbc_part = ar.take<float>(G);
  t.u_pre = ar.take<float>(M * A * (1 + gated));
  t.tn_ws = ar.take<float>((int64_t)TN_SLABS * A * E);
  t.nt_ws = ar.take<float>(4 * M * A);
  if (w) *w = t;
  return ar.off;
}

template <typename F>
static int dispatch_epl(int64_t E, F&& f) {
  switch (E) {
    case 256: return f(std::integral_constant<int, 4>());
    case 512: return f(std::integral_constant<int, 8>());
    case 1024: return f(std::integral_constant<int, 16>());
    default: return fail(-1, "token width E=%lld unsupported (256, 512 or 1024)", (long long)E);
  }
}

static int check_scorer(const mhimx_scorer* sc) {
  MHIMX_CHECK_ARG(sc && sc->wa && sc->wc, "scorer: null weights");
  MHIMX_CHECK_ARG(sc->A > 0 && sc->A <= 512 && sc->A % 4 == 0, "scorer: A must be a multiple of 4, <= 512");
  MHIMX_CHECK_ARG(!sc->gated || sc->wb, "scorer: gated needs wb");
  return 0;
}

int abmil_pool_fwd(hipStream_t st, const mhimx_scorer* sc, mhimx_pool_io* io) {
  if (int r = check_scorer(sc)) return r;
  MHIMX_CHECK_ARG(io && io->T1 && io->M1 > 0 && io->s && io->stats && io->z, "pool_fwd: null io");
  MHIMX_CHECK_ARG(io->M2 == 0 || io->T2, "pool_fwd: M2>0 needs T2");
  MHIMX_CHECK_ARG(!io->cproj || (io->wp && io->C > 0), "pool_fwd: cproj needs wp, C");
  MHIMX_CHECK_ARG(!io->rows1 || (io->M2 == 0 && scorer_fused_ok(sc->E, sc->A, sc->gated, sc->prec, io->T1, sc->wa, io->cproj ? io->wp : nullptr, io->C)),
                  "pool_fwd: gathered tokens (rows1) need the one-pass scorer (E = 512, A = 128, plain form, not f32) and a single segment");
  MHIMX_CHECK_ARG(!io->excl || scorer_fused_ok(sc->E, sc->A, sc->gated, sc->prec, io->T1, sc->wa, io->cproj ? io->wp : nullptr, io->C),
                  "pool_fwd: excluded rows (excl) need the one-pass scorer (E = 512, A = 128, plain form, not f32)");
  const int64_t M = io->M1 + io->M2, E = sc->E, A = sc->A;
  const int gated = sc->gated ? 1 : 0;
  Arena ar(io->ws, io->ws_bytes);
  PoolWs w;
  pool_ws_layout(ar, M, E, A, gated, &w);
  MHIMX_CHECK_ARG(ar.ok(), "pool_fwd: workspace too small (%lld < %lld)", (long long)io->ws_bytes, (long long)ar.off);
  float* u_pre = io->u_pre ? io->u_pre : w.u_pre;
  const int64_t ldu = A * (1 + gated);
  if (io->phase != 0) {
    const int64_t K = io->tail_tokens, Ms1 = io->M1 - K;
    MHIMX_CHECK_ARG((io->phase == 1 || io->phase == 2) && K >= 1 && K <= FIN_MAXTOK && Ms1 >= 1 && io->M2 == 0 && !io->cproj && !io->pscore && !io->excl &&
                        E == 512 && A == 128 && scorer_fused_ok(E, A, gated, sc->prec, io->T1, sc->wa, nullptr, 0),
                    "pool_fwd: the two-call forward takes the one-pass scorer shapes, one segment, 1..%d tail tokens, no class projections", FIN_MAXTOK);
    const int tiles = (int)cdiv(Ms1, 32);
    const int G1 = tiles < MAX_PART ? tiles : MAX_PART;
    if (io->phase == 1) {
      M2RowsFwd mfbuf;
      const void* mf = nullptr;
      io->rode_merge = 0;
      if (io->ride_merge) {
        const int rc = merge2_fwd_rows_args(reinterpret_cast<const mhimx_merge*>(io->ride_merge), io->ride_X, io->ride_R, io->ride_ws, io->ride_ws_bytes,
                                            &mfbuf);
        if (rc < 0) return rc;
        if (rc == 0) { mf = &mfbuf; io->rode_merge = 1; }
      }
      const int g1 = scorer_fused_fwd(st, io->T1, Ms1, sc->wa, sc->wa_frag, sc->ba, sc->act, sc->wc, sc->bc, nullptr, 0, u_pre, io->s, nullptr, w.pm, w.pl,
                                      w.pz, MAX_PART, io->rows1, nullptr, io->ride_jobs, io->n_ride_jobs, mf);
      return g1 < 0 ? g1 : 0;
    }
    hipLaunchKernelGGL(pool_finalize_tok_kernel, bgrid((unsigned)cdiv(E, 64)), dim3(FIN_THREADS), 0, st, w.pm, w.pl, w.pz, G1, (int)E, io->stats, io->z, io->T1,
                       (io->rows1 && io->tail_row0 < 0) ? io->rows1 + Ms1 : nullptr, io->rows1 ? io->tail_row0 : Ms1, (int)K, sc->wa, io->tail_wa_t, sc->ba, sc->wc,
                       sc->bc, (int)A, sc->act, u_pre + Ms1 * ldu, io->s + Ms1, cur_batch());
    MHIMX_LAUNCH_CHECK();
    return 0;
  }

  const float* Ts[2] = {io->T1, io->T2};
  const int64_t Ms[2] = {io->M1, io->M2};
  int64_t off = 0;
  int G = 0;
  bool rode = false;
  for (int seg = 0; seg < 2; ++seg) {
    if (Ms[seg] == 0) continue;
    if (scorer_fused_ok(E, A, gated, sc->prec, Ts[seg], sc->wa, io->cproj ? io->wp : nullptr, io->C)) {
      const int g1 = scorer_fused_fwd(st, Ts[seg], Ms[seg], sc->wa, sc->wa_frag, sc->ba, sc->act, sc->wc, sc->bc, io->cproj ? io->wp : nullptr,
                                      (int)io->C, io->no_backward ? nullptr : u_pre + off * ldu, io->s + off, io->cproj ? io->cproj + off * io->C : nullptr,
                                      w.pm + G, w.pl + G, w.pz + (int64_t)G * E, MAX_PART, seg == 0 ? io->rows1 : nullptr,
                                      seg == 0 ? io->excl : nullptr, rode ? nullptr : io->ride_jobs, rode ? 0 : io->n_ride_jobs, nullptr);
      if (g1 < 0) return g1;
      rode = true;
      G += g1;
      off += Ms[seg];
      continue;
    }
    MHIMX_CHECK_ARG(cur_batch().n == 0, "pool_fwd: a bag-batched launch needs the one-pass scorer");
    mhimx_gemm_nt_args g = {};
    g.A = Ts[seg]; g.lda = E; g.B = sc->wa; g.ldb = E; g.C = u_pre + off * ldu; g.ldc = ldu;
    g.M = Ms[seg]; g.N = A; g.K = E; g.bias = sc->ba;
    g.ws = w.nt_ws; g.ws_floats = 4 * M * A;
    g.prec = sc->prec == MHIMX_PREC_F32 ? MHIMX_PREC_F32 : MHIMX_PREC_BF16X3;
    if (int r = gemm_nt(st, g)) return r;
    if (gated) {
      g.B = sc->wb; g.bias = sc->bb; g.C = u_pre + off * ldu + A;
      if (int r = gemm_nt(st, g)) return r;
    }
    int grid = (int)cdiv(Ms[seg], 5 * FWD_WAVES);
    if (grid < 1) grid = 1;
    if (grid > MAX_PART) grid = MAX_PART;
    const float* Tseg = Ts[seg];
    const int64_t Mseg = Ms[seg];
    int r = dispatch_epl(E, [&](auto epl) {
      constexpr int EPL = decltype(epl)::value;
      const size_t smem = (size_t)(FWD_WAVES * E + 2 * FWD_WAVES) * sizeof(float);
      if (smem > 48 * 1024)
        MHIMX_ONCE_PER_DEVICE(MHIMX_HIP(hipFuncSetAttribute((const void*)score_rows_fwd_kernel<EPL>, hipFuncAttributeMaxDynamicSharedMemorySize, (int)smem)));
      hipLaunchKernelGGL(score_rows_fwd_kernel<EPL>, dim3(grid), dim3(64 * FWD_WAVES), smem, st, Tseg, Mseg, (int)E, (int)A,
                         sc->act, gated, u_pre + off * ldu, sc->wc, sc->bc, io->cproj ? io->wp : nullptr, (int)io->C,
                         io->s + off, io->cproj ? io->cproj + off * io->C : nullptr, w.pm + G, w.pl + G,
                         w.pz + (int64_t)G * E, sc->gate_drop_p, sc->gate_drop_seed, off);
      MHIMX_LAUNCH_CHECK();
      return 0;
    });
    if (r) return r;
    G += grid;
    off += Ms[seg];
  }
  if (!rode && io->ride_jobs && io->n_ride_jobs > 0)
    if (int r = prep_batch(st, io->ride_jobs, io->n_ride_jobs)) return r;
  MHIMX_CHECK_ARG(!io->pscore || io->cproj, "pool_fwd: pscore needs cproj (and wp)");
  static_assert(2 * MAX_PART <= FIN_THREADS, "pool_finalize_kernel reads one partial per thread");
  const int64_t ps_blocks = io->pscore ? (cdiv(io->M1, FIN_THREADS) < 64 ? cdiv(io->M1, FIN_THREADS) : 64) : 0;
  hipLaunchKernelGGL(pool_finalize_kernel, bgrid((unsigned)(cdiv(E, 64) + ps_blocks)), dim3(FIN_THREADS), 0, st, w.pm, w.pl, w.pz, G, (int)E, io->stats,
                     io->z, io->s, io->cproj, io->bp, (int)io->C, io->M1, io->pscore, cur_batch());
  MHIMX_LAUNCH_CHECK();
  return 0;
}

int abmil_pool_bwd(hipStream_t st, const mhimx_scorer* sc, const mhimx_pool_io* io, const mhimx_pool_grad* gr) {
  if (int r = check_scorer(sc)) return r;
  MHIMX_CHECK_ARG(io && gr && gr->g_z && gr->dT1 && gr->d_wa && gr->d_wc && gr->wa_t, "pool_bwd: null args");
  MHIMX_CHECK_ARG(io->M2 == 0 || gr->dT2, "pool_bwd: M2>0 needs dT2");
  const int64_t M = io->M1 + io->M2, E = sc->E, A = sc->A;
  const int gated = sc->gated ? 1 : 0;
  MHIMX_CHECK_ARG(!gated || (gr->d_wb && gr->wb_t), "pool_bwd: gated needs d_wb, wb_t");
  Arena ar(io->ws, io->ws_bytes);
  PoolWs w;
  pool_ws_layout(ar, M, E, A, gated, &w);
  MHIMX_CHECK_ARG(ar.ok(), "pool_bwd: workspace too small");
  const float* u_pre = io->u_pre ? io->u_pre : w.u_pre;
  const int64_t ldu = A * (1 + gated);
  const float* Ts[2] = {io->T1, io->T2};
  float* dTs[2] = {gr->dT1, gr->dT2};
  const int64_t Ms[2] = {io->M1, io->M2};

  int64_t off = 0;
  int G = 0;
  const bool fused = scorer_fused_ok(E, A, gated, sc->prec, io->T1, gr->wa_t, nullptr, 0) && aligned16(gr->dT1) &&
                     (io->M2 == 0 || (aligned16(io->T2) && aligned16(gr->dT2))) && aligned16(u_pre) && aligned16(w.du);
  MHIMX_CHECK_ARG(!io->rows1 || (fused && io->M2 == 0), "pool_bwd: gathered tokens (rows1) need the one-pass backward and a single segment");
  MHIMX_CHECK_ARG(!gr->img || (fused && io->M2 == 0 && E == 512), "pool_bwd: the dPRE image (img) needs the one-pass backward and a single segment");
  MHIMX_CHECK_ARG(cur_batch().n == 0 || (fused && io->M2 == 0 && !gated && gr->defer && !gr->d_bc && !gr->d_ba && !gr->d_bb),
                  "pool_bwd: a bag-batched launch needs the one-pass backward with its reductions queued");
  for (int seg = 0; seg < 2 && fused; ++seg) {
    if (Ms[seg] == 0) continue;
    const void* pre_side = nullptr;
    int64_t gate_row0 = -1;
    if (seg == 0 && io->M2 == 0 && gr->defer && gr->defer->pre.pending == 1) {
      Merge2Side psd;
      memcpy(&psd, gr->defer->pre.blob, sizeof(psd));
      const int64_t d = psd.dz - dTs[0];
      if (psd.dz >= dTs[0] && d % E == 0) {
        pre_side = gr->defer->pre.blob;
        gate_row0 = d / E;
        gr->defer->pre.pending = 2;
      }
    }
    const int g1 = scorer_fused_bwd(st, Ts[seg], Ms[seg], u_pre + off * ldu, io->s + off, io->stats, gr->g_z, io->z, sc->wc, sc->act,
                                    gr->wa_t, gr->wa_t_frag, w.du + off * ldu, dTs[seg], w.dwc_part + (int64_t)G * A, w.dbc_part + G,
                                    MAX_PART, seg == 0 ? io->rows1 : nullptr, pre_side, gate_row0, seg == 0 ? gr->img : nullptr, gr->img_dact, gr->img_part,
                                    gr->img_rows);
    if (g1 < 0) return g1;
    G += g1;
    off += Ms[seg];
  }
  for (int seg = 0; seg < 2 && !fused; ++seg) {
    if (Ms[seg] == 0) continue;
    const int grid = grid_for_rows(Ms[seg]);
    const float* Tseg = Ts[seg];
    const int64_t Mseg = Ms[seg];
    int r = dispatch_epl(E, [&](auto epl) {
      constexpr int EPL = decltype(epl)::value;
      const size_t smem = (size_t)(4 * A + 8) * sizeof(float);
      hipLaunchKernelGGL(score_rows_bwd_kernel<EPL>, dim3(grid), dim3(ROWS_THREADS), smem, st, Tseg, Mseg, (int)E, (int)A,
                         sc->act, gated, u_pre + off * ldu, sc->wc, io->s + off, io->stats, gr->g_z, io->z,
                         w.du + off * ldu, w.attn + off, w.dwc_part + (int64_t)G * A, w.dbc_part + G, sc->gate_drop_p,
                         sc->gate_drop_seed, off);
      MHIMX_LAUNCH_CHECK();
      return 0;
    });
    if (r) return r;
    G += grid;
    off += Ms[seg];
  }
  if (!defer_push(gr->defer, reduce_job_parts(w.dwc_part, G, A, A, gr->d_wc, gr->accumulate)))
    hipLaunchKernelGGL(reduce_parts_kernel, dim3((unsigned)cdiv(A, 32)), dim3(RP_THREADS), 0, st, w.dwc_part, G, (int)A, (int)A, gr->d_wc, gr->accumulate);
  MHIMX_LAUNCH_CHECK();
  if (gr->d_bc) {
    if (!defer_push(gr->defer, reduce_job_parts(w.dbc_part, G, 1, 1, gr->d_bc, gr->accumulate)))
      hipLaunchKernelGGL(reduce_parts_kernel, dim3(1), dim3(RP_THREADS), 0, st, w.dbc_part, G, 1, 1, gr->d_bc, gr->accumulate);
    MHIMX_LAUNCH_CHECK();
  }
  off = 0;
  for (int seg = 0; seg < 2; ++seg) {
    if (Ms[seg] == 0) continue;
    mhimx_gemm_nt_args g = {};
    g.A = w.du + off * ldu; g.lda = ldu; g.B = gr->wa_t; g.ldb = A; g.C = dTs[seg]; g.ldc = E;
    g.M = Ms[seg]; g.N = E; g.K = A; g.rowv = w.attn + off; g.colv = gr->g_z; g.prec = sc->prec == MHIMX_PREC_F32 ? MHIMX_PREC_F32 : MHIMX_PREC_BF16X3;
    if (!fused)
      if (int r = gemm_nt(st, g)) return r;
    if (gated) {
      g.A = w.du + off * ldu + A; g.B = gr->wb_t; g.rowv = nullptr; g.colv = nullptr; g.accumulate = 1;
      if (int r = gemm_nt(st, g)) return r;
    }
    mhimx_gemm_tn_args t = {};
    t.A = w.du + off * ldu; t.lda = ldu; t.B = Ts[seg]; t.ldb = E; t.C = gr->d_wa; t.ldc = E;
// ... 341 lines not shown
```

mhim_mil_amd/csrc/step.hip:

```cpp
#include <math.h>
#include <string.h>

#include "infer_tab.hpp"
#include "step_mid.hpp"

namespace mhimx {

int64_t merge2_rows_tiles(int64_t R);

namespace {

struct DagEvents {
  hipEvent_t e[64][6];
  bool have[64] = {};
  int get(hipEvent_t** out) {
    int dev = 0;
    MHIMX_HIP(hipGetDevice(&dev));
    MHIMX_CHECK_ARG(dev >= 0 && dev < 64, "step: device index %d", dev);
    if (!have[dev]) {
      for (int i = 0; i < 6; ++i) MHIMX_HIP(hipEventCreateWithFlags(&e[dev][i], hipEventDisableTiming));
      have[dev] = true;
    }
    *out = e[dev];
    return 0;
// ... 49 lines not shown
  int64_t q_scr, gslab;
  int64_t rows_img, P0, L_img;
  int64_t bag0, bag_stride;
  int64_t total;
};

int dpre_merge_rows(void* stream, const float* dH, const void* dact, const int64_t* rows_merge, int64_t R, int64_t E, char* img, int64_t P0, float* d_b1,
                    float* ws_b, int64_t ws_b_bytes, mhimx_reduce_list* lst) {
  const int64_t t0 = P0 / 32;
  const int n0 = lst->n;
  float* part_m = ws_b + t0 * E;
  if (int r = mhimx_rows_dpre_image(stream, dH, dact, rows_merge, R, E, img + t0 * (E / 128) * 16384, d_b1, 0, part_m, ws_b_bytes - t0 * E * 4, lst)) return r;
  MHIMX_CHECK_ARG(lst->n == n0 + 1 && lst->j[n0].kind == 0 && lst->j[n0].parts == part_m, "step: the bias gradient's partial sum was not queued");
  lst->j[n0].parts = ws_b;
  lst->j[n0].G += t0;
  return 0;
}

int check_cfg(const mhimx_step_cfg* c, int64_t N, const mhimx_step_counts* n) {
  MHIMX_CHECK_ARG(c && n, "step: null configuration / counts");
  MHIMX_CHECK_ARG(c->E == 512 && c->A == 128 && c->C >= 1 && c->C <= 4 && c->k >= 1 && 8 * c->k <= 48 && c->D > 0 && c->D % 256 == 0,
                  "step: shapes outside the single-pass ABMIL step (E = 512, A = 128, C <= 4, 8 k <= 48, D %% 256 == 0)");
  MHIMX_CHECK_ARG(N >= 64 && N <= MHIMX_STEP_MAX_ROWS && n->k_top >= 1 && n->k_top <= (N <= 16384 ? 4096 : 16384) && n->n_sel >= 1 && n->n_sel <= n->k_top &&
                      n->len_keep == N - n->n_sel && n->Lk >= 1 && n->R >= 1 && n->R <= 32768 && n->Lk + n->R == n->len_keep,
                  "step: row counts outside the device-drawn select (64 <= N <= %d, k_top <= 4096 up to 16384 rows / 16384 above, rows to merge "
                  "<= 32768, rows to merge and rows that stay >= 1)", MHIMX_STEP_MAX_ROWS);
  const mhimx_step_params &s = c->student, &t = c->teacher;
  MHIMX_CHECK_ARG(s.w1 && s.b1 && s.wa && s.wc && s.wp && s.bp && s.q && s.ln_w && s.ln_b && s.wkv && s.wq && s.wo && s.bo, "step: null student parameter");
  MHIMX_CHECK_ARG(t.w1 && t.b1 && t.wa && t.wc && (!c->attn2score || (t.wp && t.bp)), "step: null teacher parameter");
  const mhimx_step_grads& g = c->grad;
  MHIMX_CHECK_ARG(g.w1 && g.b1 && g.wa && g.wc && g.wp && g.bp && g.ln_w && g.ln_b && g.wkv && g.wq && g.wo && g.bo, "step: null gradient view");
  MHIMX_CHECK_ARG(c->tick, "step: the device dropout / draw counter (tick) is required");
  return 0;
}

void layout(const mhimx_step_cfg* c, int64_t N, const mhimx_step_counts* n, StepBufs* b, int n_bags = 1) {
  const int64_t D = c->D, E = c->E, A = c->A, C = c->C, k = c->k, I = 512;
  Carve cv(nullptr);
  const int64_t F = sizeof(float);
  b->w1p_t = cv.take_off(E * D * F);
  b->wa_frag_t = cv.take_off(A * E * F);
  b->w1p_s = cv.take_off(E * D * F);
  b->wa_frag_s = cv.take_off(A * E * F);
  b->wa_t = cv.take_off(E * A * F);
  b->wa_t_frag = cv.take_off(E * A * F);
  b->wo_t = cv.take_off(I * E * F);
  b->q_old = cv.take_off(k * E * F);
  if (n_bags > 1) {
    b->wg_ws_floats = mhimx_wgrad_multi_ws_floats(N <= 16384 ? (n->Lk + k + 31) / 32 * 32 + n->R : n->len_keep, E, D, n_bags);
    b->wg_ws = cv.take_off(b->wg_ws_floats * F);
  }
  b->bag0 = cv.off;
  b->merge_ws_bytes = mhimx_merge_ws_bytes(n->R, E, k, 8, 64);
  b->merge_ws = cv.take_off(b->merge_ws_bytes);
  const bool fuse_img = N <= 16384;
  b->P0 = fuse_img ? (n->Lk + k + 31) / 32 * 32 : 0;
  b->L_img = fuse_img ? b->P0 + n->R : n->len_keep;
  b->H_t = cv.take_off(N * E * F);
  b->Hbuf = cv.take_off((N + k) * E * F);
  b->dact = cv.take_off(N * E * 2);
  b->s_t = cv.take_off(N * F);
  b->stats_t = cv.take_off(2 * F);
  b->z_t = cv.take_off(E * F);
  b->cproj_t = cv.take_off(N * C * F);
  b->pscore = cv.take_off(N * F);
  b->attn = cv.take_off(N * F);
  b->pool_ws_t_bytes = mhimx_abmil_pool_ws_bytes(N, E, A, 0);
  b->pool_ws_t = cv.take_off(b->pool_ws_t_bytes);
  b->rows_all = cv.take_off((n->len_keep + k) * 8);
  b->sel_ws_bytes = mhimx_select_ws_bytes(N);
  b->sel_ws = cv.take_off(b->sel_ws_bytes);
  b->rows_img = fuse_img ? cv.take_off((b->L_img + 31) / 32 * 32 * 8) : 0;
  b->sel_perm = b->sel_ids = b->sel_rows = b->sel_lk = 0;
  if (N > 16384) {
    b->sel_perm = cv.take_off(n->k_top * 8);
    b->sel_ids = cv.take_off(N * 8);
    b->sel_rows = cv.take_off(n->len_keep * 8);
    b->sel_lk = cv.take_off(8);
  }
  const int64_t M = n->Lk + k;
  b->s_s = cv.take_off(M * F);
  b->stats_s = cv.take_off(2 * F);
  b->z_s = cv.take_off(E * F);
  b->pool_ws_s_bytes = mhimx_abmil_pool_ws_bytes(M, E, A, 0);
  b->pool_ws_s = cv.take_off(b->pool_ws_s_bytes);
  b->logits = cv.take_off(16 * F);
  b->losses = cv.take_off(4 * F);
  b->g_z = cv.take_off(E * F);
  b->dH = cv.take_off((N + k) * E * F);
  b->img = cv.take_off(mhimx_wgrad_image_bytes(b->L_img, E));
  b->ws_b_bytes = (fuse_img ? b->P0 / 32 + (n->R + 31) / 32 : (n->len_keep + 31) / 32) * E * F;
  b->ws_b = cv.take_off(b->ws_b_bytes);
  b->q_scr = b->gslab = 0;
  if (n_bags > 1) {
    b->q_scr = cv.take_off(k * E * F);
    b->gslab = cv.take_off(c->n_all * F);
  } else {
    b->wg_ws_floats = mhimx_wgrad_ws_floats(b->L_img, E, D);
    b->wg_ws = cv.take_off(b->wg_ws_floats * F);
  }
  b->bag_stride = cv.off - b->bag0;
  b->total = b->bag0 + (int64_t)n_bags * b->bag_stride;
}

}

int step_check_cfg(const mhimx_step_cfg* c, int64_t N, const mhimx_step_counts* n) { return check_cfg(c, N, n); }

mhimx_merge mid_merge_params(const mhimx_step_cfg& c) {
  const mhimx_step_params& S = c.student;
  mhimx_merge m = {};
  m.E = c.E; m.k = c.k; m.heads = 8; m.dim_head = 64;
  m.q_param = S.q; m.ln_w = S.ln_w; m.ln_b = S.ln_b; m.wkv = S.wkv; m.wq = S.wq; m.wo = S.wo; m.bo = S.bo;
  m.mm = c.merge_mm; m.prec = MHIMX_PREC_BF16X3; m.drop_tick = c.tick; m.rep = 1.f;
  return m;
}

int mid_prep_head(const mhimx_step_cfg& c, const MidImages& im, mhimx_prep_job* j) {
  int n = prep_counters(c, j);
  j[n++] = mhimx_prep_job{1, c.teacher.w1, im.w1p_t, c.E, c.D};
  j[n++] = mhimx_prep_job{4, c.teacher.wa, im.wa_frag_t, c.A, c.E};
  j[n++] = mhimx_prep_job{1, c.student.w1, im.w1p_s, c.E, c.D};
  return n;
}

int mid_prep_student(const mhimx_step_cfg& c, const MidImages& im, mhimx_prep_job* j) {
  const mhimx_step_params& S = c.student;
  j[0] = mhimx_prep_job{4, S.wa, im.wa_frag_s, c.A, c.E};
  j[1] = mhimx_prep_job{0, S.wa, im.wa_t, c.A, c.E};
  j[2] = mhimx_prep_job{5, S.wa, im.wa_t_frag, c.A, c.E};
  j[3] = mhimx_prep_job{0, S.wo, im.wo_t, c.E, 512};
  j[4] = mhimx_prep_job{2, S.q, im.q_old, 1, c.k * c.E};
  return 5;
}

mhimx_scorer mid_scorer(const mhimx_step_cfg& c, const mhimx_step_params& p, const float* wa_frag) {
  mhimx_scorer sc = {};
  sc.E = c.E; sc.A = c.A; sc.act = c.da_act; sc.prec = MHIMX_PREC_BF16X3; sc.wa = p.wa; sc.wc = p.wc; sc.wa_frag = wa_frag;
  return sc;
}

int mid_student_fwd(void* stream, const mhimx_step_cfg& c, const MidImages& im, const mhimx_merge& mw_prep, const MidBag& g, const MidDag* dag, MidFwd* f) {
  const int64_t E = c.E, k = c.k;
  mhimx_merge& mw = f->mw;
  mw = mw_prep;
  mw.drop_p = c.merge_drop_p; mw.drop_seed = g.mca_seed; mw.x_rows = g.rows_all; mw.prepared = 1;
  f->sc_s = mid_scorer(c, c.student, im.wa_frag_s);
  mhimx_pool_io& io = f->io_s;
  io = mhimx_pool_io{};
  io.T1 = g.Hbuf; io.M1 = g.Lk + k; io.s = g.s_s; io.stats = g.stats_s; io.z = g.z_s;
  io.ws = g.pool_ws; io.ws_bytes = g.pool_ws_bytes; io.rows1 = g.rows_all + g.R;
  io.tail_row0 = -1;
  io.phase = 1; io.tail_tokens = (int32_t)k;
  if (dag) {
    if (int r = dag_edge(dag->ev[0], dag->main_st, dag->side_st)) return r;
  } else {
    io.ride_merge = &mw; io.ride_X = g.Hbuf; io.ride_R = g.R; io.ride_ws = g.merge_ws; io.ride_ws_bytes = g.merge_ws_bytes;
  }
  if (int r = mhimx_abmil_pool_fwd(dag ? dag->side_st : stream, &f->sc_s, &io)) return r;
  mw.rows_done = io.rode_merge;
  if (int r = mhimx_merge_fwd(stream, &mw, g.Hbuf, g.R, g.Hbuf + g.N * E, g.q_out, 1, g.merge_ws, g.merge_ws_bytes)) return r;
  mw.rows_done = 0;
  if (dag)
    if (int r = dag_edge(dag->ev[1], dag->side_st, dag->main_st)) return r;
  io.phase = 2; io.tail_wa_t = im.wa_t; io.tail_row0 = g.N;
  if (int r = mhimx_abmil_pool_fwd(stream, &f->sc_s, &io)) return r;
  io.phase = 0; io.ride_merge = nullptr;
  return 0;
}

int mid_head(void* stream, const mhimx_step_cfg& c, const MidBag& g, const float* z_t, const int64_t* label, float loss_scale, float* logits,
             float* losses, const mhimx_step_grads& gr, int accumulate, const MidSurv* sv) {
  if (sv)
    return mhimx_head_surv_fwd_bwd(stream, g.z_s, c.aux_alpha != 0.f ? z_t : nullptr, c.student.wp, c.student.bp, label, sv->censor, c.E, c.C, c.temp_t,
                                   c.main_alpha, c.aux_alpha, loss_scale, sv->alpha, sv->eps, logits, losses, sv->risk, g.g_z, gr.wp, gr.bp, accumulate);
  return mhimx_head_fwd_bwd(stream, g.z_s, c.aux_alpha != 0.f ? z_t : nullptr, c.student.wp, c.student.bp, label, c.E, c.C, c.temp_t, c.main_alpha,
                            c.aux_alpha, loss_scale, logits, losses, g.g_z, gr.wp, gr.bp, accumulate, nullptr, nullptr);
}

int mid_bwd_rows(void* stream, const MidImages& im, const MidFwd& f, const MidBag& g, const mhimx_step_grads& gr, int accumulate, const MidImg* img,
                 const MidDag* dag, mhimx_reduce_list* lst) {
  const int64_t E = f.mw.E;
  float* d_tok = g.dH + g.N * E;
  mhimx_merge mwb = f.mw;
  mwb.q_param = im.q_old; mwb.wo_t = im.wo_t; mwb.prepared = 0;
  mhimx_merge_grad mg = {};
  mg.d_ln_w = gr.ln_w; mg.d_ln_b = gr.ln_b; mg.d_wkv = gr.wkv; mg.d_wq = gr.wq; mg.d_wo = gr.wo; mg.d_bo = gr.bo;
  mg.accumulate = accumulate; mg.splits = 8; mg.defer = lst;
  if (int r = mhimx_merge_bwd_park(&mwb, g.Hbuf, g.R, d_tok, g.dH, &mg, g.merge_ws, g.merge_ws_bytes)) return r;
  {
    mhimx_scorer sc_b = f.sc_s;
    sc_b.wa_frag = nullptr;
    mhimx_pool_grad pg = {};
    pg.g_z = g.g_z; pg.dT1 = g.dH; pg.d_wa = gr.wa; pg.d_wc = gr.wc; pg.wa_t = im.wa_t; pg.accumulate = accumulate; pg.splits = 8; pg.defer = lst;
    pg.wa_t_frag = im.wa_t_frag;
    if (img) { pg.img = img->img; pg.img_dact = img->dact; pg.img_part = img->part; pg.img_rows = g.Lk; }
    if (int r = mhimx_abmil_pool_bwd(stream, &sc_b, &f.io_s, &pg)) return r;
  }
  if (dag) {
    if (int r = dag_edge(dag->ev[2], dag->main_st, dag->side_st)) return r;
    if (lst->parked.pending && lst->pre.pending == 2) lst->parked.reserved = (int32_t)merge2_rows_tiles(g.R) + 1;
    if (int r = mhimx_reduce_flush(dag->side_st, lst)) return r;
  }
  if (int r = mhimx_merge_bwd(stream, &mwb, g.Hbuf, g.R, d_tok, g.dH, &mg, g.merge_ws, g.merge_ws_bytes)) return r;
  if (dag) {
    if (int r = dag_edge(dag->ev[3], dag->main_st, dag->side_st)) return r;
    if (int r = mhimx_reduce_flush(dag->side_st, lst)) return r;
  }
  return 0;
}

void q_chain_weights(double mm, int n, float* wq, float* w) {
  *wq = (float)pow(mm, (double)n);
  for (int b = 0; b < n; ++b) w[b] = (float)((1.0 - mm) * pow(mm, (double)(n - 1 - b)));
}

}

using namespace mhimx;

extern "C" int mhimx_step_counts_of(int64_t N, double mask_ratio_h, double mask_ratio_hr, double merge_ratio, mhimx_step_counts* out) {
  MHIMX_CHECK_ARG(out && N >= 1 && mask_ratio_h > 0.0 && mask_ratio_hr > 0.0 && merge_ratio > 0.0, "step_counts: bad arguments");
  double eff = mask_ratio_h / mask_ratio_hr, rr = mask_ratio_hr;
  if (eff > 1.0) { rr = mask_ratio_h; eff = 1.0; }
  const int64_t k = (int64_t)ceil((double)N * eff);
  const int64_t n_sel = rr < 1.0 ? (int64_t)ceil((double)k * rr) : k;
  const int64_t len_keep = N - n_sel;
  const int64_t Lk = (int64_t)((double)len_keep * merge_ratio);
  *out = mhimx_step_counts{k, n_sel, len_keep, Lk, len_keep - Lk};
  MHIMX_CHECK_ARG(k >= 1 && n_sel >= 1 && len_keep >= 1 && Lk >= 1 && len_keep - Lk >= 1, "step_counts: the recipe leaves nothing to mask, keep or merge");
  return 0;
}

extern "C" int mhimx_step_layout_of(const mhimx_step_cfg* cfg, int64_t N, const mhimx_step_counts* cnt, mhimx_step_layout* out) {
  MHIMX_CHECK_ARG(out, "step_layout: null output");
  if (int r = check_cfg(cfg, N, cnt)) return r;
  StepBufs b;
  layout(cfg, N, cnt, &b);
  *out = mhimx_step_layout{b.total, b.logits, b.losses, cfg->attn2score ? b.pscore : b.attn, b.rows_all, b.H_t, b.Hbuf, b.dact, b.z_t, b.z_s, b.g_z, b.dH};
  return 0;
}

extern "C" int mhimx_step_run(void* stream, const mhimx_step_cfg* cfg, const float* X, int64_t ldx, int64_t N, const int64_t* label_dev,
                              const mhimx_step_counts* cnt, const mhimx_step_seeds* seeds, int64_t host_step, void* ws, int64_t ws_bytes, int32_t update) {
  if (int r = check_cfg(cfg, N, cnt)) return r;
  MHIMX_CHECK_ARG(X && label_dev && seeds && ws && ldx >= cfg->D && ldx % 4 == 0 && N * ldx * 4 < ((int64_t)1 << 32) && aligned16(X),
                  "step: null bag / label / seeds / workspace, or a row pitch the weight-gradient product does not take");
  MHIMX_CHECK_ARG(!update || (cfg->p && cfg->g && cfg->m && cfg->v && cfg->n_train > 0 && cfg->n_all >= cfg->n_train), "step: update needs the flat optimiser buffers");
  StepBufs b;
  layout(cfg, N, cnt, &b);
  MHIMX_CHECK_ARG(ws_bytes >= b.total && (reinterpret_cast<uintptr_t>(ws) & 255) == 0, "step: workspace too small (%lld < %lld) or not 256-byte aligned",
                  (long long)ws_bytes, (long long)b.total);
  const mhimx_step_cfg& c = *cfg;
  const mhimx_step_params &S = c.student, &T = c.teacher;
  const int64_t D = c.D, E = c.E, C = c.C, k = c.k;
  const int64_t R = cnt->R, Lk = cnt->Lk, len_keep = cnt->len_keep;
  const bool fuse_img = N <= 16384;
  const hipStream_t main_st = (hipStream_t)stream;
  Carve cv(ws);
  const MidImages im = {cv.at<float>(b.w1p_t), cv.at<float>(b.wa_frag_t), cv.at<float>(b.w1p_s), cv.at<float>(b.wa_frag_s),
                        cv.at<float>(b.wa_t),  cv.at<float>(b.wa_t_frag), cv.at<float>(b.wo_t),  cv.at<float>(b.q_old)};
  void* merge_ws = cv.at<char>(b.merge_ws);
  float* H_t = cv.at<float>(b.H_t);
  float* Hbuf = cv.at<float>(b.Hbuf);
  void* dact = cv.at<char>(b.dact);
  int64_t* rows_all = cv.at<int64_t>(b.rows_all);
  float* dH = cv.at<float>(b.dH);
  const uint64_t* tick = c.tick;
  MidDag dag_st = {main_st, (hipStream_t)c.side_stream, nullptr};
  const MidDag* dag = c.side_stream != nullptr && c.side_stream != stream ? &dag_st : nullptr;
  if (dag)
    if (int r = g_dag_events.get(&dag_st.ev)) return r;

  const mhimx_merge mw_prep = mid_merge_params(c);
  {
    mhimx_prep_job early[8];
    int n = mid_prep_head(c, im, early);
    early[n++] = mhimx_prep_job{10, nullptr, reinterpret_cast<float*>(rows_all + len_keep), N, k};
    if (int r = mhimx_prep_batch(stream, early, n)) return r;
  }
  mhimx_prep_job late[6];
  mid_prep_student(c, im, late);
  late[5] = mhimx_prep_job{6, reinterpret_cast<const float*>(&mw_prep), static_cast<float*>(merge_ws), R, b.merge_ws_bytes};

  {
    mhimx_bag_project_args a = {};
    a.X = X; a.ldx = ldx; a.N = N; a.D = D; a.E = E; a.act = c.act; a.n_heads = 2; a.drop_tick = tick;
    a.head[0].wp = im.w1p_t; a.head[0].bias = T.b1; a.head[0].H = H_t; a.head[0].ldh = E; a.head[0].drop_p = c.drop_p_teacher; a.head[0].drop_seed = seeds->drop_teacher;
    a.head[1].wp = im.w1p_s; a.head[1].bias = S.b1; a.head[1].H = Hbuf; a.head[1].ldh = E; a.head[1].dact = dact; a.head[1].drop_p = c.drop_p_student;
    a.head[1].drop_seed = seeds->drop_student;
    hipEvent_t* tp = nullptr;
    int tp_dev = 0;
    if (c.time_project) {
      hipStreamCaptureStatus cs = hipStreamCaptureStatusNone;
      MHIMX_HIP(hipStreamIsCapturing(main_st, &cs));
      if (cs == hipStreamCaptureStatusNone)
        if (int r = g_proj_times.next(&tp_dev, &tp)) return r;
    }
    if (tp) MHIMX_HIP(hipEventRecord(tp[0], main_st));
    if (int r = mhimx_bag_project(stream, &a)) return r;
    if (tp) {
      MHIMX_HIP(hipEventRecord(tp[1], main_st));
      MHIMX_HIP(hipEventRecord(tp[2], main_st));
      ++g_proj_times.n[tp_dev];
    }
  }

  const mhimx_scorer sc_t = mid_scorer(c, T, im.wa_frag_t);
  const float* score = nullptr;
  {
    mhimx_pool_io io = {};
    io.T1 = H_t; io.M1 = N; io.s = cv.at<float>(b.s_t); io.stats = cv.at<float>(b.stats_t); io.z = cv.at<float>(b.z_t);
    io.ws = cv.at<char>(b.pool_ws_t); io.ws_bytes = b.pool_ws_t_bytes;
    if (c.attn2score) { io.wp = T.wp; io.C = C; io.cproj = cv.at<float>(b.cproj_t); io.bp = T.bp; io.pscore = cv.at<float>(b.pscore); }
    io.no_backward = 1;
    io.ride_jobs = late; io.n_ride_jobs = 6;
    if (int r = mhimx_abmil_pool_fwd(stream, &sc_t, &io)) return r;
    if (c.attn2score) score = io.pscore;
    else {
      if (int r = mhimx_softmax_from_stats(stream, io.s, io.stats, cv.at<float>(b.attn), N)) return r;
// ... 430 lines not shown
```

mhim_mil_amd/csrc/step_mid.hpp:

```cpp
#pragma once
#include "common.hpp"

namespace mhimx {

struct MidImages { float *w1p_t, *wa_frag_t, *w1p_s, *wa_frag_s, *wa_t, *wa_t_frag, *wo_t, *q_old; };

struct MidBag {
  float *Hbuf, *dH;
  int64_t* rows_all;
  int64_t N, R, Lk;
  uint64_t mca_seed;
  float* q_out;
  float *s_s, *stats_s, *z_s, *g_z;
  void* pool_ws; int64_t pool_ws_bytes;
  void* merge_ws; int64_t merge_ws_bytes;
};
struct MidDag { hipStream_t main_st, side_st; hipEvent_t* ev; };
struct MidFwd { mhimx_merge mw; mhimx_scorer sc_s; mhimx_pool_io io_s; };
struct MidImg { void* img; const void* dact; float* part; };

mhimx_merge mid_merge_params(const mhimx_step_cfg& c);
int mid_prep_head(const mhimx_step_cfg& c, const MidImages& im, mhimx_prep_job* j);
int mid_prep_student(const mhimx_step_cfg& c, const MidImages& im, mhimx_prep_job* j);
mhimx_scorer mid_scorer(const mhimx_step_cfg& c, const mhimx_step_params& p, const float* wa_frag);
int mid_student_fwd(void* stream, const mhimx_step_cfg& c, const MidImages& im, const mhimx_merge& mw_prep, const MidBag& g, const MidDag* dag, MidFwd* f);
struct MidSurv { const float* censor; float alpha, eps; float* risk; };
int mid_head(void* stream, const mhimx_step_cfg& c, const MidBag& g, const float* z_t, const int64_t* label, float loss_scale, float* logits,
             float* losses, const mhimx_step_grads& gr, int accumulate, const MidSurv* sv = nullptr);
int mid_bwd_rows(void* stream, const MidImages& im, const MidFwd& f, const MidBag& g, const mhimx_step_grads& gr, int accumulate, const MidImg* img,
                 const MidDag* dag, mhimx_reduce_list* lst);
void q_chain_weights(double mm, int n, float* wq, float* w);

}
```

mhim_mil_amd/mhim.py:

```python
from __future__ import annotations

import itertools
import math
import os
import types
from typing import Callable, NamedTuple, Optional

import numpy as np

import torch
from torch import nn

from . import _lib as L
from . import dsmil as DS
from . import nystrom as NY
from . import ops

_FEATURE_ACTS = ("relu", "gelu")
_SCORER_ACTS = ("relu", "gelu", "tanh")


class _Lin(nn.Module):

    def __init__(self, i, o, bias=True):
# ... 388 lines not shown
    def _pairable(self, x):
        return self._feature_prec(x.shape[0]) == "bf16x3" and x.shape[1] % 32 == 0 and x.shape[0] > 16

    def _feature(self, x, rows=None, drop_p=0.0, drop_seed=0, drop_mask=None, want_pre=False, out=None, pre_out=None, M=None,
                 xp=None, w1p=None, dact=None):
        f = self.feature[0]
        act = L.act_code(self.act, _FEATURE_ACTS)
        nrows = M if M is not None else (rows.shape[0] if rows is not None else x.shape[0])
        if xp is None and nrows >= 1024:
            xp = self._pair(x)
        if xp is not None and nrows > 16:
            return ops.gemm_nt(xp, w1p if w1p is not None else ops.pair_planes(f.weight.data), out=out, rows=rows, bias=f.bias.data, act=act, pre=pre_out,
                               drop_p=drop_p, drop_seed=drop_seed, drop_mask=drop_mask, prec="bf16x3", M=M, drop_tick=self._tick,
                               paired=True, dact=dact)
        if dact is not None:
            raise L.MhimxError("the dact output needs the paired-plane projection path")
        return ops.gemm_nt(x, f.weight.data, out=out, rows=rows, bias=f.bias.data, act=act, pre=pre_out, drop_p=drop_p,
                           drop_seed=drop_seed, drop_mask=drop_mask, prec=self._feature_prec(nrows), M=M, drop_tick=self._tick)

    def _feature_prec(self, nrows):
        if self.prec != "auto":
            return self.prec
        return "bf16x3"

    @property
    def _op_prec(self):
        return "f32" if self.prec == "f32" else "bf16x3"

    def _next_seed(self, teacher=False):
        self._step += 1
        salt = 0xA24BAED4963EE407 if teacher else 0
        return (torch.initial_seed() * 0x9E3779B97F4A7C15 + self._step * 0xD1B54A32D192ED03 + salt) & 0xFFFFFFFFFFFFFFFF

    def _bag_forward(self, x, plan: BagPlan, xp=None, prep=None):
        prep = prep or {}
        E = self.mlp_dim
        Lrows = plan.L
        dev = x.device
        need_pre = L.act_code(self.act, _FEATURE_ACTS) == L.ACT["gelu"] and plan.training
        merging = self.merge_enable and plan.R > 0
        k = self.merge.k if merging else 0
        Hbuf = torch.empty((Lrows + k, E), device=dev)
        H = Hbuf[:Lrows]
        use_dact = plan.training and xp is not None and E % 128 == 0 and x.shape[1] % 32 == 0 and Lrows >= 64
        DACT = torch.empty((Lrows, E), device=dev) if use_dact else None
        PRE = torch.empty((Lrows, E), device=dev) if (need_pre and not use_dact) else None
        p = self.dropout_p if plan.training else 0.0
        self._feature(x, plan.rows, p, plan.drop_seed, plan.drop_mask, out=H, pre_out=PRE, M=Lrows, xp=xp, w1p=prep.get("w1p"),
                      dact=DACT)
        saved = {"H": H, "Hbuf": Hbuf, "PRE": PRE, "DACT": DACT, "prep": prep}
        sc = self._scorer(prep.get("wa_frag"))
        if merging:
            mw = self._merge_w(plan, need_t=False, wkv_frag=prep.get("wkv_frag"))
            q_old = prep.get("q_old")
            if q_old is None and plan.training:
                q_old = self.merge.global_q_mm.data.clone()
            q_param = getattr(plan, "q_out", None)
            if q_param is None:
                q_param = self.merge.global_q_mm.data.view(self.merge.k, -1)
            Hm = H[:plan.R] if plan.merge_first else H[plan.Lk:]
            z_tok, _, mws = ops.merge_fwd(mw, Hm, z_out=Hbuf[Lrows:], update_q=plan.training,
                                          q_out=q_param if plan.training else None)
            if plan.merge_first:
                st = ops.abmil_pool_fwd(sc, Hbuf[plan.R:], None)
            else:
                st = ops.abmil_pool_fwd(sc, H[:plan.Lk], z_tok)
            saved.update(z_tok=z_tok, mws=mws, q_old=q_old)
        else:
            st = ops.abmil_pool_fwd(sc, H, None)
        saved["pool"] = st
        return st.z, saved

    def _bag_backward(self, x, plan: BagPlan, saved, g_z, out=None, defer=None, mid_hook=None):
        out = out or {}
        E = self.mlp_dim
        dev = x.device
        H, PRE, st = saved["H"], saved["PRE"], saved["pool"]
        prep = saved.get("prep") or {}
        sc = self._scorer()
        att = self.online_encoder.attention
        merging = self.merge_enable and plan.R > 0
        mf = merging and plan.merge_first
        dHbuf = torch.empty_like(saved["Hbuf"])
        dH = dHbuf[:plan.L]
        grads = {}
        pool_g = {"dT1": dHbuf[plan.R:] if mf else (dH[:plan.Lk] if merging else dH)}
        pre = "online_encoder.attention."
        for key, nm in (("d_wa", "attention_a.0.weight" if self.online_encoder.gated else "attention.0.weight"),
                        ("d_wb", "attention_b.0.weight"),
                        ("d_wc", "attention_c.weight" if self.online_encoder.gated else "attention.2.weight")):
            if pre + nm in out:
                pool_g[key] = out[pre + nm]
        if self.online_encoder.gated:
            g = ops.abmil_pool_bwd(sc, st, g_z, prep.get("wa_t") if "wa_t" in prep else ops.transpose(att.attention_a[0].weight.data),
                                   prep.get("wb_t") if "wb_t" in prep else ops.transpose(att.attention_b[0].weight.data), grads=pool_g)
            grads["online_encoder.attention.attention_a.0.weight"] = g["d_wa"]
            grads["online_encoder.attention.attention_b.0.weight"] = g["d_wb"]
            grads["online_encoder.attention.attention_c.weight"] = g["d_wc"]
        else:
            g = ops.abmil_pool_bwd(sc, st, g_z, prep.get("wa_t") if "wa_t" in prep else ops.transpose(att.attention[0].weight.data),
                                   grads=pool_g, defer=defer, wa_t_frag=prep.get("wa_t_frag"))
            grads["online_encoder.attention.attention.0.weight"] = g["d_wa"]
            grads["online_encoder.attention.attention.2.weight"] = g["d_wc"]
        if self.merge_enable and plan.R > 0:
            mw = self._merge_w(plan, need_t=True, q=saved["q_old"], tr=prep.get("merge_t"))
            mgr = {"dX": dH[:plan.R] if mf else dH[plan.Lk:]}
            for key, nm in (("d_ln_w", "merge.norm.weight"), ("d_ln_b", "merge.norm.bias"), ("d_wkv", "merge.attn.to_kv.weight"),
                            ("d_wq", "merge.attn.to_q.weight"), ("d_wo", "merge.attn.to_out.0.weight"),
                            ("d_bo", "merge.attn.to_out.0.bias")):
                if nm in out:
                    mgr[key] = out[nm]
            mg = ops.merge_bwd(mw, H[:plan.R] if mf else H[plan.Lk:], dHbuf[plan.L:] if mf else g["dT2"], saved["mws"], grads=mgr,
                               defer=defer)
            grads["merge.norm.weight"], grads["merge.norm.bias"] = mg["d_ln_w"], mg["d_ln_b"]
            grads["merge.attn.to_kv.weight"], grads["merge.attn.to_q.weight"] = mg["d_wkv"], mg["d_wq"]
            grads["merge.attn.to_out.0.weight"], grads["merge.attn.to_out.0.bias"] = mg["d_wo"], mg["d_bo"]
        if mid_hook is not None:
            if defer is not None:
                ops.reduce_flush(defer)
            mid_hook()
        p = self.dropout_p if plan.training else 0.0
        if saved.get("DACT") is not None:
            _, db1 = ops.mul_colsum(dH, saved["DACT"], colsum_out=out.get("feature.0.bias"), defer=defer)
        else:
            _, db1 = ops.act_bwd(dH, H, PRE, L.act_code(self.act, _FEATURE_ACTS), p, plan.drop_seed, plan.drop_mask, plan.rows,
                                 colsum_out=out.get("feature.0.bias"), want_colsum=True, drop_tick=self._tick)
        splits = 8 if plan.L >= 2048 else 1
        grads["feature.0.weight"] = ops.gemm_tn(dH, x, out=out.get("feature.0.weight"), rows=plan.rows, splits=splits,
                                                prec="f32" if self.prec == "f32" else "bf16x3", M=plan.L, defer=defer)
        grads["feature.0.bias"] = db1
        return grads

    def single_projection_ok(self, x):
        return (self.mlp_dim == 512 and x.shape[1] % 32 == 0 and x.shape[0] >= 64 and self._feature_prec(x.shape[0]) == "bf16x3"
                and ops.bag_wgrad_ok(x, self.mlp_dim, x.shape[0]))

    def bag_ordered_ok(self, x):
        att = self.online_encoder.attention if self.baseline == "attn" else None
        return (self.baseline == "attn" and not self.online_encoder.gated and self.mlp_dim == 512 and x.shape[1] % 32 == 0
                and att.attention[0].weight.shape[0] == 128 and self._feature_prec(x.shape[0]) == "bf16x3" and x.shape[0] >= 64
                and self.n_classes <= 4 and L.act_code(self.da_act, _SCORER_ACTS) in (L.ACT["relu"], L.ACT["gelu"], L.ACT["tanh"], 0))

    def _bag_forward_nat(self, x, plan: BagPlan, Hbuf, DACT, rows_all, prep):
        N = x.shape[0]
        sc = self._scorer(prep.get("wa_frag"))
        saved = {"Hbuf": Hbuf, "DACT": DACT, "rows_all": rows_all, "prep": prep}
        if rows_all is not None:
            mw = self._merge_w(plan, need_t=False, wkv_frag=prep.get("wkv_frag"), x_rows=rows_all[:plan.R], prepared="merge_ws" in prep)
            q_param = getattr(plan, "q_out", None)
            if q_param is None:
                q_param = self.merge.global_q_mm.data.view(self.merge.k, -1)
            k = self.merge.k
            if "merge_ws" in prep and k <= 6 and rows_all.numel() - plan.R > k:
                st, rode = ops.abmil_pool_fwd_split(sc, Hbuf, rows_all[plan.R:], k, ride_merge=(mw, Hbuf, prep["merge_ws"]))
                _, _, mws = ops.merge_fwd(mw, Hbuf, z_out=Hbuf[N:], update_q=plan.training, q_out=q_param if plan.training else None,
                                          ws=prep["merge_ws"], rows_done=rode)
                ops.abmil_pool_fwd_finish(sc, st, wa_t=prep.get("wa_t"), tail_row0=N)
            else:
                _, _, mws = ops.merge_fwd(mw, Hbuf, z_out=Hbuf[N:], update_q=plan.training, q_out=q_param if plan.training else None,
                                          ws=prep.get("merge_ws"))
                st = ops.abmil_pool_fwd(sc, Hbuf, None, rows1=rows_all[plan.R:])
            saved.update(mws=mws, q_old=prep.get("q_old"))
        else:
            st = ops.abmil_pool_fwd(sc, Hbuf[:N], None)
        saved["pool"] = st
        return st.z, saved

    def _bag_backward_nat(self, x, plan: BagPlan, saved, g_z, out, defer=None, mid_hook=None, accumulate=False, wgrad_park=None,
                          ride_tail=False):
        N = x.shape[0]
        Hbuf, rows_all, st, prep = saved["Hbuf"], saved["rows_all"], saved["pool"], saved["prep"]
        sc = self._scorer()
        dHbuf = torch.empty_like(Hbuf)
        grads = {}
        pre = "online_encoder.attention.attention."
        pool_g = {"dT1": dHbuf if rows_all is not None else dHbuf[:N]}
        for key, nm in (("d_wa", "0.weight"), ("d_wc", "2.weight")):
            if pre + nm in out:
                pool_g[key] = out[pre + nm]
        mw = mgr = None
        if rows_all is not None:
            mw = self._merge_w(plan, need_t=True, q=saved["q_old"], tr=prep.get("merge_t"), x_rows=rows_all[:plan.R])
            mgr = {"dX": dHbuf}
            for key, nm in (("d_ln_w", "merge.norm.weight"), ("d_ln_b", "merge.norm.bias"), ("d_wkv", "merge.attn.to_kv.weight"),
                            ("d_wq", "merge.attn.to_q.weight"), ("d_wo", "merge.attn.to_out.0.weight"),
                            ("d_bo", "merge.attn.to_out.0.bias")):
                if nm in out:
                    mgr[key] = out[nm]
            if len(mgr) == 7:
                ops.merge_bwd_park(mw, Hbuf, dHbuf[N:], saved["mws"], mgr, accumulate=accumulate, defer=defer)
        g = ops.abmil_pool_bwd(sc, st, g_z, prep["wa_t"], grads=pool_g, defer=defer, wa_t_frag=prep.get("wa_t_frag"), accumulate=accumulate)
        grads[pre + "0.weight"], grads[pre + "2.weight"] = g["d_wa"], g["d_wc"]
        if rows_all is not None:
            mg = ops.merge_bwd(mw, Hbuf, dHbuf[N:], saved["mws"], grads=mgr, defer=defer, accumulate=accumulate)
            grads["merge.norm.weight"], grads["merge.norm.bias"] = mg["d_ln_w"], mg["d_ln_b"]
            grads["merge.attn.to_kv.weight"], grads["merge.attn.to_q.weight"] = mg["d_wkv"], mg["d_wq"]
            grads["merge.attn.to_out.0.weight"], grads["merge.attn.to_out.0.bias"] = mg["d_wo"], mg["d_bo"]
        if mid_hook is not None:
            if defer is not None:
                ops.reduce_flush(defer)
            mid_hook()
        Lr = plan.L
        rows = None if rows_all is None else rows_all[:Lr]
        if wgrad_park is not None and rows is not None and ops.bag_wgrad_ok(x, dHbuf.shape[1], Lr):
            im = ops.bag_wgrad_image(dHbuf, saved["DACT"], x, rows, Lr, out_b=out.get("feature.0.bias"), accumulate=accumulate, defer=defer)
            wgrad_park.append(im)
            grads["feature.0.weight"], db1 = None, out.get("feature.0.bias")
        elif ops.bag_wgrad_ok(x, dHbuf.shape[1], Lr):
            grads["feature.0.weight"], db1 = ops.bag_wgrad(dHbuf, saved["DACT"], x, rows, Lr, out_w=out.get("feature.0.weight"),
                                                           out_b=out.get("feature.0.bias"), defer=defer, accumulate=accumulate,
                                                           ride_tail=ride_tail)
        else:
            dpre, db1 = ops.rows_dpre(dHbuf, saved["DACT"], rows, Lr, colsum_out=out.get("feature.0.bias"), defer=defer, accumulate=accumulate)
            grads["feature.0.weight"] = ops.gemm_tn(dpre, x, out=out.get("feature.0.weight"), rows=rows, splits=8 if Lr >= 2048 else 1,
                                                    prec="bf16x3", M=Lr, defer=defer, accumulate=accumulate)
        grads["feature.0.bias"] = db1
        return grads

    def get_mask(self, ps, i, attn, mrh=None, perm=None, perms=None, generator=None, seed=None):
        if attn is None:
            return ps, None
        heads = None
        if attn.dim() == 3 or (attn.dim() == 2 and attn.shape[0] != 1):
            heads = attn.reshape(-1, attn.shape[-1]).contiguous().float()
            score = None
        else:
            score = attn.reshape(-1).contiguous().float()
        dev = attn.device
        perms = list(perms) if perms is not None else [None, None, perm]
        masked, n_masked, len_keep, mask_ids = None, 0, ps, None
        n_draws = [0]

        def run(largest, ratio, rratio, pm):
            nonlocal masked, n_masked, len_keep, mask_ids
            eff = ratio / rratio
            if eff > 1:
                rratio, eff = ratio, 1.0
            k = int(np.ceil(ps * eff))
            n_sel = int(np.ceil(k * rratio)) if rratio < 1.0 else k
            if rratio < 1.0 and pm is None:
                if generator is not None:
                    pm = torch.randperm(k, device=dev, generator=generator)
                else:
                    n_draws[0] += 1
                    pm = ops.random_perm(k, (self._next_seed() if seed is None else seed) + 0x51ED270B * n_draws[0], tick=self._tick, device=dev)
            elif pm is not None and not torch.is_tensor(pm):
                pm = torch.as_tensor(np.asarray(pm), dtype=torch.int64, device=dev)
            sc, lg = score, largest
            if heads is not None:
                sc, lg = ops.vote_scores(heads, k, largest), True
            ids, lk_dev, _ = ops.select_mask(sc, k, n_sel, lg, pm if rratio < 1.0 else None, other=masked)
            if masked is None:
                len_keep = ps - n_sel
            else:
                len_keep = int(lk_dev.item())
            mask_ids = ids
            masked = ids[len_keep:].contiguous()

        if self.mask_ratio > 0.:
            run(False, self.mask_ratio, 0.001, perms[0])
        if self.mask_ratio_l > 0.:
            run(False, self.mask_ratio_l, 1.0, None)
        mask_ratio_h = self.mask_ratio_h
        if self.mrh_sche is not None:
            mask_ratio_h = self.mrh_sche[i]
        if mrh is not None:
            mask_ratio_h = mrh
        if mask_ratio_h > 0.:
            run(True, mask_ratio_h, self.mask_ratio_hr, perms[2])
        return len_keep, (None if mask_ids is None else mask_ids.view(1, -1))

    def v2_counts(self, ps, i=None, mrh=None):
        mask_ratio_h = self.mask_ratio_h
        if self.mrh_sche is not None and i is not None:
            mask_ratio_h = self.mrh_sche[i]
        if mrh is not None:
            mask_ratio_h = mrh
        if not (self.mask_ratio == 0 and self.mask_ratio_l == 0 and mask_ratio_h > 0):
            return None
        eff, rr = mask_ratio_h / self.mask_ratio_hr, self.mask_ratio_hr
        if eff > 1:
            rr, eff = mask_ratio_h, 1.0
        k = int(np.ceil(ps * eff))
        n_sel = int(np.ceil(k * rr)) if rr < 1.0 else k
        len_keep = ps - n_sel
        Lk = int(len_keep * self.merge.merge_ratio)
        return k, n_sel, len_keep, Lk, len_keep - Lk

    def device_draw_ok(self, ps, i=None, mrh=None):
        c = self.v2_counts(ps, i, mrh)
        return c is not None and self.baseline in ("attn", "dsmil") and ps <= 16384 and c[0] <= 4096

    def student_rows(self, ps, i, attn, perm=None, ids_shuffle=None, mrh=None, generator=None, merge_first=False, rows_out=None, seed=None):
        mask_ratio_h = self.mask_ratio_h
        if self.mrh_sche is not None:
            mask_ratio_h = self.mrh_sche[i]
        if mrh is not None:
            mask_ratio_h = mrh
        v2 = self.mask_ratio == 0 and self.mask_ratio_l == 0 and mask_ratio_h > 0
        if (v2 and self.baseline in ("attn", "dsmil") and perm is None and ids_shuffle is None and generator is None and attn is not None
                and attn.numel() == ps and ps <= 16384):
            eff, rr = mask_ratio_h / self.mask_ratio_hr, self.mask_ratio_hr
            if eff > 1:
                rr, eff = mask_ratio_h, 1.0
            k = int(np.ceil(ps * eff))
            n_sel = int(np.ceil(k * rr)) if rr < 1.0 else k
            if k <= 4096:
                len_keep = ps - n_sel
                Lk = int(len_keep * self.merge.merge_ratio)
# ... 508 lines not shown
```

mhim_mil_amd/ops.py:

```python
from __future__ import annotations

import collections
import ctypes as C
import functools
import itertools
import math
from typing import Optional

import torch

from . import _lib as L


KERNEL_EVENT_HOOK = None


import threading

_PIN = threading.local()


def _pinned():
    st = getattr(_PIN, "stream", None)
    if st is not None and getattr(_PIN, "device", -1) == torch.cuda.current_device():
# ... 161 lines not shown
    for i, (kind, src, dst) in enumerate(jobs):
        if kind == PREP_TICK:
            arr[i] = L.PrepJob(kind, None, _p(dst), 1, 1)
        elif kind == PREP_MERGE:
            ws, n_rows = dst
            arr[i] = L.PrepJob(kind, C.c_void_p(C.addressof(src.c)), _p(ws), int(n_rows), ws.numel())
        else:
            _chk(src, name="prep in"); _chk(dst, name="prep out")
            R, Cc = (src.shape[0], src.numel() // src.shape[0]) if src.dim() >= 2 else (1, src.numel())
            arr[i] = L.PrepJob(kind, _p(src), _p(dst), R, Cc)
    return arr


def prep_batch(jobs):
    arr = _prep_array(jobs)
    L.check(L.lib().mhimx_prep_batch(_stream(), arr, len(jobs)), "mhimx_prep_batch")


_STEP_IMAGES = {}


def step_images(table=None):
    _STEP_IMAGES.clear()
    if table:
        _STEP_IMAGES.update(table)


def pair_planes(x):
    _chk(x, name="x")
    img = _STEP_IMAGES.get((x.data_ptr(), False))
    if img is not None and img.shape == x.shape:
        return img
    M, K = x.shape
    out = torch.empty_like(x)
    L.check(L.lib().mhimx_pair_planes(_stream(), _p(x), x.stride(0), M, K, _p(out)), "mhimx_pair_planes")
    return out


def pair_planes_t(x):
    _chk(x, name="x")
    img = _STEP_IMAGES.get((x.data_ptr(), True))
    if img is not None and img.shape == (x.shape[1], x.shape[0]):
        return img
    return pair_planes(transpose(x))


class ReduceList:

    def __init__(self):
        self.c = L.ReduceListC()
        self.c.n = 0
        self.c.side.pending = 0
        self.c.parked.pending = 0
        self.c.pre.pending = 0
        self.keep = []

    def ptr(self):
        return C.addressof(self.c)


def _dp(defer):
    return None if defer is None else defer.ptr()


def reduce_flush(lst: "ReduceList"):
    L.check(L.lib().mhimx_reduce_flush(_stream(), lst.ptr()), "mhimx_reduce_flush")
    lst.keep.clear()


def reduce_slabs_job(lst: "ReduceList", slabs, out, accumulate=True):
    _chk(slabs, name="slabs"); _chk(out, name="out")
    G, n = slabs.shape
    if lst.c.n >= L.REDUCE_MAX:
        raise L.MhimxError("reduce list full")
    lst.c.j[lst.c.n] = L.ReduceJob(kind=1, accumulate=int(bool(accumulate)), parts=_p(slabs), out=_p(out), G=G, W=0, ld=0, K1=1, K2=n, ldo=n)
    lst.c.n += 1
    lst.keep.append(slabs)


def gemm_tn(a, b, out=None, rows=None, splits=1, accumulate=False, prec="bf16x3", M=None, defer=None):
    _chk(a, name="a"); _chk(b, name="b"); _chk(out, name="out"); _chk(rows, torch.int64, "rows")
    if M is None:
        M = a.shape[0]
    K1, K2 = a.shape[1], b.shape[1]
    if out is None:
        out = torch.empty((K1, K2), device=a.device, dtype=torch.float32)
    nslab = max(int(splits), 1)
    if splits > 1:
        nslab = max(nslab, min(64, -(-512 // max(1, (K1 // 128) * (K2 // 128)))), -(-M // 4096))
    ws = torch.empty((nslab, K1, K2), device=a.device, dtype=torch.float32) if nslab > 1 else None
    g = L.GemmTN(A=_p(a), lda=a.stride(0), B=_p(b), ldb=b.stride(0), rows=_p(rows), C=_p(out), ldc=out.stride(0), M=M,
                 K1=K1, K2=K2, splits=int(splits), ws=_p(ws), accumulate=int(bool(accumulate)), prec=prec_code(prec),
                 ws_floats=0 if ws is None else ws.numel(), defer=_dp(defer))
    L.check(L.lib().mhimx_gemm_tn(_stream(), C.byref(g)), "mhimx_gemm_tn")
    if defer is not None:
        defer.keep.append(ws)
    return out


def transpose(x, out=None):
    _chk(x, name="x")
    R, Cc = x.shape
    if out is None:
        out = torch.empty((Cc, R), device=x.device, dtype=torch.float32)
    L.check(L.lib().mhimx_transpose(_stream(), _p(x), _p(out), R, Cc), "mhimx_transpose")
    return out


class ScorerW:

    def __init__(self, wa, wc, act, ba=None, wb=None, bb=None, bc=None, prec="bf16x3", wa_frag=None, gate_drop_p=0.0, gate_drop_seed=0):
        self.t = (wa, wc, ba, wb, bb, bc, wa_frag)
        for t in self.t:
            _chk(t, name="scorer weight")
        self.A, self.E = wa.shape
        self.gated = wb is not None
        self.c = L.Scorer(E=self.E, A=self.A, act=int(act), gated=int(self.gated), prec=prec_code(prec), wa=_p(wa),
                          ba=_p(ba), wb=_p(wb), bb=_p(bb), wc=_p(wc), bc=_p(bc), wa_frag=_p(wa_frag),
                          gate_drop_p=float(gate_drop_p), gate_drop_seed=int(gate_drop_seed) & 0xFFFFFFFFFFFFFFFF)


class PoolState:

    def __init__(self, T1, T2, C_classes=0, wp=None, device=None, bp=None, rows1=None, excl=None):
        dev = T1.device
        M1 = T1.shape[0] if rows1 is None else rows1.shape[0]
        self.rows1 = rows1
        self.excl = excl
        M2 = 0 if T2 is None else T2.shape[0]
        self.T1, self.T2, self.M1, self.M2 = T1, T2, M1, M2
        M = M1 + M2
        self.s = torch.empty(M, device=dev)
        self.stats = torch.empty(2, device=dev)
        self.z = torch.empty(T1.shape[1], device=dev)
        self.cproj = torch.empty((M, C_classes), device=dev) if wp is not None else None
        self.wp = wp
        self.bp = bp
        self.pscore = torch.empty(M1, device=dev) if (wp is not None and bp is not None) else None
        self.ws = None
        self.ride = None

    def io(self, sc: ScorerW):
        M = self.M1 + self.M2
        nbytes = L.lib().mhimx_abmil_pool_ws_bytes(M, sc.E, sc.A, int(sc.gated))
        if self.ws is None or self.ws.numel() < nbytes:
            self.ws = torch.empty(nbytes, device=self.T1.device, dtype=torch.uint8)
        return L.PoolIO(T1=_p(self.T1), M1=self.M1, T2=_p(self.T2), M2=self.M2, s=_p(self.s), stats=_p(self.stats),
                        z=_p(self.z), u_pre=None, wp=_p(self.wp), C=0 if self.cproj is None else self.cproj.shape[1],
                        cproj=_p(self.cproj), ws=_p(self.ws), ws_bytes=self.ws.numel(), bp=_p(self.bp), pscore=_p(self.pscore),
                        rows1=_p(self.rows1), excl=_p(self.excl),
                        ride_jobs=None if self.ride is None else C.cast(self.ride[0], C.c_void_p), n_ride_jobs=0 if self.ride is None else self.ride[1])


def abmil_pool_fwd_split(sc: ScorerW, T1, rows1, tail_tokens, ride_merge=None):
    _chk(T1, name="T1"); _chk(rows1, torch.int64, "rows1")
    st = PoolState(T1, None, 0, None, rows1=rows1)
    st.tail_tokens = int(tail_tokens)
    io = st.io(sc)
    io.phase, io.tail_tokens = 1, st.tail_tokens
    if ride_merge is not None:
        mw, X, ws = ride_merge
        io.ride_merge, io.ride_X = C.cast(C.pointer(mw.c), C.c_void_p), _p(X)
        io.ride_R, io.ride_ws, io.ride_ws_bytes = mw.x_rows.shape[0], _p(ws), ws.numel()
    L.check(L.lib().mhimx_abmil_pool_fwd(_stream(), C.byref(sc.c), C.byref(io)), "mhimx_abmil_pool_fwd (phase 1)")
    return st, bool(io.rode_merge)


def abmil_pool_fwd_finish(sc: ScorerW, st: PoolState, wa_t=None, tail_row0=-1):
    io = st.io(sc)
    io.phase, io.tail_tokens = 2, st.tail_tokens
    io.tail_wa_t, io.tail_row0 = _p(wa_t), int(tail_row0)
    L.check(L.lib().mhimx_abmil_pool_fwd(_stream(), C.byref(sc.c), C.byref(io)), "mhimx_abmil_pool_fwd (phase 2)")
    return st


def abmil_pool_fwd(sc: ScorerW, T1, T2=None, wp=None, bp=None, rows1=None, excl=None, ride_jobs=None, no_backward=False):
    _chk(T1, name="T1"); _chk(T2, name="T2"); _chk(wp, name="wp"); _chk(bp, name="bp"); _chk(rows1, torch.int64, "rows1")
    _chk(excl, torch.uint8, "excl")
    st = PoolState(T1, T2, 0 if wp is None else wp.shape[0], wp, bp=bp, rows1=rows1, excl=excl)
    if ride_jobs:
        st.ride = (_prep_array(ride_jobs), len(ride_jobs))
    io = st.io(sc)
    io.no_backward = int(bool(no_backward))
    L.check(L.lib().mhimx_abmil_pool_fwd(_stream(), C.byref(sc.c), C.byref(io)), "mhimx_abmil_pool_fwd")
    st.ride = None
    return st


def abmil_pool_bwd(sc: ScorerW, st: PoolState, g_z, wa_t, wb_t=None, need_bias=False, splits=8, grads=None,
                   accumulate=False, defer=None, wa_t_frag=None, img=None, img_dact=None, img_part=None, img_rows=0):
    dev = g_z.device
    E, A = sc.E, sc.A
    out = grads or {}
    out.setdefault("dT1", torch.empty((st.M1, E), device=dev))
    if st.M2:
        out.setdefault("dT2", torch.empty((st.M2, E), device=dev))
    out.setdefault("d_wa", torch.empty((A, E), device=dev))
    out.setdefault("d_wc", torch.empty((1, A), device=dev))
    if sc.gated:
        out.setdefault("d_wb", torch.empty((A, E), device=dev))
    if need_bias:
        out.setdefault("d_ba", torch.empty(A, device=dev))
        out.setdefault("d_bc", torch.empty(1, device=dev))
        if sc.gated:
            out.setdefault("d_bb", torch.empty(A, device=dev))
    io = st.io(sc)
    g = L.PoolGrad(g_z=_p(g_z), dT1=_p(out["dT1"]), dT2=_p(out.get("dT2")), d_wa=_p(out["d_wa"]), d_ba=_p(out.get("d_ba")),
                   d_wb=_p(out.get("d_wb")), d_bb=_p(out.get("d_bb")), d_wc=_p(out["d_wc"]), d_bc=_p(out.get("d_bc")),
                   wa_t=_p(wa_t), wb_t=_p(wb_t), accumulate=int(bool(accumulate)), splits=int(splits), defer=_dp(defer),
                   wa_t_frag=_p(wa_t_frag), img=_p(img), img_dact=_p(img_dact), img_part=_p(img_part), img_rows=int(img_rows))
    if defer is not None:
        defer.keep.append(st)
    L.check(L.lib().mhimx_abmil_pool_bwd(_stream(), C.byref(sc.c), C.byref(io), C.byref(g)), "mhimx_abmil_pool_bwd")
    return out


def softmax_from_stats(s, stats):
    out = torch.empty_like(s)
    L.check(L.lib().mhimx_softmax_from_stats(_stream(), _p(s), _p(stats), _p(out), s.numel()), "mhimx_softmax_from_stats")
    return out


def pseudo_score(s, stats, cproj, bp, want_attn=False):
    M = cproj.shape[0] if s is None else s.numel()
    score = torch.empty(M, device=cproj.device)
    attn = torch.empty_like(s) if want_attn else None
    L.check(L.lib().mhimx_pseudo_score(_stream(), _p(s), _p(stats), _p(cproj), _p(bp), _p(score), _p(attn), M,
                                       cproj.shape[1]), "mhimx_pseudo_score")
    return (score, attn) if want_attn else score


def lse_merge(parts):
    _chk(parts, name="parts")
    W, E = parts.shape[0], parts.shape[1] - 2
    stats, z = torch.empty(2, device=parts.device), torch.empty(E, device=parts.device)
    L.check(L.lib().mhimx_lse_merge(_stream(), _p(parts), W, E, _p(stats), _p(z)), "mhimx_lse_merge")
    return stats, z


def select_mask(score, k, n_sel, largest=True, perm=None, other=None, want_topk=False):
    _chk(score, name="score"); _chk(perm, torch.int64, "perm"); _chk(other, torch.int64, "other")
    N = score.numel()
    dev = score.device
    mask_ids = torch.empty(N, device=dev, dtype=torch.int64)
    len_keep = torch.empty(1, device=dev, dtype=torch.int64)
    topk = torch.empty(k, device=dev, dtype=torch.int64) if want_topk else None
    ws = torch.empty(L.lib().mhimx_select_ws_bytes(N), device=dev, dtype=torch.uint8)
    L.check(L.lib().mhimx_select_mask(_stream(), _p(score), N, int(k), int(n_sel), int(bool(largest)), _p(perm), _p(other),
                                      0 if other is None else other.numel(), _p(mask_ids), _p(len_keep), _p(topk), _p(ws),
                                      ws.numel()), "mhimx_select_mask")
    return mask_ids, len_keep, topk


def select_rows(score, k, n_sel, merge_R, rand_seed, tick=None, largest=True, want_mask_ids=False, merge_first=False, out=None):
    _chk(score, name="score")
    N = score.numel()
    dev = score.device
    rows = out if out is not None else torch.empty(N - n_sel, device=dev, dtype=torch.int64)
    _chk(rows, torch.int64, "rows out")
    mask_ids = torch.empty(N, device=dev, dtype=torch.int64) if want_mask_ids else None
    ws = torch.empty(L.lib().mhimx_select_ws_bytes(N), device=dev, dtype=torch.uint8)
    L.check(L.lib().mhimx_select_rows(_stream(), _p(score), N, int(k), int(n_sel), int(bool(largest)),
                                      int(rand_seed) & 0xFFFFFFFFFFFFFFFF, _p(tick), int(merge_R), _p(rows), _p(mask_ids), _p(ws),
                                      ws.numel(), int(bool(merge_first))), "mhimx_select_rows")
    return (rows, mask_ids) if want_mask_ids else rows


def select_rows_img(score, k, n_sel, merge_R, rand_seed, img_merge_off, tick=None, largest=True, merge_first=True):
    _chk(score, name="score")
    N = score.numel()
    dev = score.device
    rows = torch.empty(N - n_sel, device=dev, dtype=torch.int64)
    rows_img = torch.empty(-(-(int(img_merge_off) + int(merge_R)) // 32) * 32, device=dev, dtype=torch.int64)
    ws = torch.empty(L.lib().mhimx_select_ws_bytes(N), device=dev, dtype=torch.uint8)
    L.check(L.lib().mhimx_select_rows_img(_stream(), _p(score), N, int(k), int(n_sel), int(bool(largest)), int(rand_seed) & 0xFFFFFFFFFFFFFFFF,
                                          _p(tick), int(merge_R), _p(rows), _p(rows_img), int(img_merge_off), _p(ws), ws.numel(),
                                          int(bool(merge_first))), "mhimx_select_rows_img")
    return rows, rows_img


def vote_scores(attn, k, largest=True):
    _chk(attn, name="attn")
    H, N = attn.shape
    vote = torch.empty(N, device=attn.device)
    L.check(L.lib().mhimx_vote_scores(_stream(), _p(attn), H, N, int(k), int(bool(largest)), _p(vote), None, 0),
            "mhimx_vote_scores")
    return vote


def random_perm(n, seed, tick=None, src=None, out=None, device=None):
    _chk(src, torch.int64, "src"); _chk(out, torch.int64, "out")
    dev = device if device is not None else (src.device if src is not None else (out.device if out is not None else torch.device("cuda")))
    if out is None:
        out = torch.empty(int(n), dtype=torch.int64, device=dev)
    L.check(L.lib().mhimx_random_perm(_stream(), int(n), int(seed) & 0xFFFFFFFFFFFFFFFF, _p(tick), _p(src), _p(out)), "mhimx_random_perm")
    return out


def compose_ids(a, b):
    _chk(a, torch.int64, "a"); _chk(b, torch.int64, "b")
    out = torch.empty_like(b)
    L.check(L.lib().mhimx_compose_ids(_stream(), _p(a), _p(b), _p(out), b.numel()), "mhimx_compose_ids")
    return out


class MergeW:
    def __init__(self, q_param, ln_w, ln_b, wkv, wq, wo, bo, mm, heads=8, dim_head=64, drop_p=0.0, drop_seed=0,
                 prec="bf16x3", transposes=None, drop_tick=None, wkv_frag=None, x_rows=None, prepared=False, own=None, rep=1.0):
        self.t = [q_param, ln_w, ln_b, wkv, wq, wo, bo, wkv_frag]
        _chk(x_rows, torch.int64, "x_rows")
        self.x_rows = x_rows
        for t in self.t:
            _chk(t, name="merge weight")
        self.k, self.E = q_param.shape[-2], q_param.shape[-1]
        self.heads, self.dim_head = heads, dim_head
        self.tr = transposes or (None, None, None)
        self.c = L.Merge(E=self.E, k=self.k, heads=heads, dim_head=dim_head, q_param=_p(q_param), ln_w=_p(ln_w),
                         ln_b=_p(ln_b), wkv=_p(wkv), wq=_p(wq), wo=_p(wo), bo=_p(bo), wkv_t=_p(self.tr[0]),
                         wq_t=_p(self.tr[1]), wo_t=_p(self.tr[2]), mm=float(mm), drop_p=float(drop_p),
                         drop_seed=int(drop_seed) & 0xFFFFFFFFFFFFFFFF, prec=prec_code(prec), drop_tick=_p(drop_tick),
                         wkv_frag=_p(wkv_frag), x_rows=_p(x_rows), prepared=int(bool(prepared)),
                         own_lo=0 if own is None else int(own[0]), own_n=0 if own is None else int(own[1]), rep=float(rep))
        self.own = own

    def ws_for(self, R, device):
        n = L.lib().mhimx_merge_ws_bytes(R, self.E, self.k, self.heads, self.dim_head)
        return torch.empty(n, device=device, dtype=torch.uint8)


def merge_fwd(mw: MergeW, X, z_out=None, update_q=True, ws=None, q_out=None, rows_done=False):
    _chk(X, name="X")
    R = X.shape[0] if mw.x_rows is None else mw.x_rows.shape[0]
    dev = X.device
    z = z_out if z_out is not None else torch.empty((mw.k, mw.E), device=dev)
    q_new = (q_out if q_out is not None else torch.empty((mw.k, mw.E), device=dev)) if update_q else None
    ws = ws if ws is not None else mw.ws_for(R, dev)
    mw.c.rows_done = int(bool(rows_done))
    L.check(L.lib().mhimx_merge_fwd(_stream(), C.byref(mw.c), _p(X), R, _p(z), _p(q_new), int(bool(update_q)), _p(ws),
                                    ws.numel()), "mhimx_merge_fwd")
    mw.c.rows_done = 0
    return z, q_new, ws


def merge_fwd_part(mw: MergeW, X, ws=None, part=None):
    _chk(X, name="X")
    R = mw.x_rows.shape[0]
    dev = X.device
    part = part if part is not None else torch.empty(L.lib().mhimx_merge_part_floats(), device=dev)
    ws = ws if ws is not None else mw.ws_for(R, dev)
    L.check(L.lib().mhimx_merge_fwd_part(_stream(), C.byref(mw.c), _p(X), R, _p(part), _p(ws), ws.numel()), "mhimx_merge_fwd_part")
    return part, ws


def merge_fwd_finish(mw: MergeW, parts, ws, z_out=None, update_q=True, q_out=None):
    _chk(parts, name="parts")
    R = mw.x_rows.shape[0]
    dev = parts.device
    z = z_out if z_out is not None else torch.empty((mw.k, mw.E), device=dev)
    q_new = (q_out if q_out is not None else torch.empty((mw.k, mw.E), device=dev)) if update_q else None
    L.check(L.lib().mhimx_merge_fwd_finish(_stream(), C.byref(mw.c), _p(parts), parts.shape[0], R, _p(z), _p(q_new), int(bool(update_q)),
                                           _p(ws), ws.numel()), "mhimx_merge_fwd_finish")
    return z, q_new


def merge_bwd_park(mw: MergeW, X, dz, ws, grads, accumulate=False, defer=None):
    if defer is None or mw.x_rows is None:
        return
    R = mw.x_rows.shape[0]
    g = L.MergeGrad(d_ln_w=_p(grads["d_ln_w"]), d_ln_b=_p(grads["d_ln_b"]), d_wkv=_p(grads["d_wkv"]), d_wq=_p(grads["d_wq"]),
                    d_wo=_p(grads["d_wo"]), d_bo=_p(grads["d_bo"]), accumulate=int(bool(accumulate)), splits=8, defer=_dp(defer))
    L.check(L.lib().mhimx_merge_bwd_park(C.byref(mw.c), _p(X), R, _p(dz), _p(grads["dX"]), C.byref(g), _p(ws), ws.numel()), "mhimx_merge_bwd_park")


def merge_bwd(mw: MergeW, X, dz, ws, splits=8, grads=None, accumulate=False, defer=None):
    dev = X.device
    R, E = X.shape
    if mw.x_rows is not None:
        R = mw.x_rows.shape[0]
        if not grads or "dX" not in grads:
            raise L.MhimxError("merge_bwd with gathered rows scatters into a caller-provided dX buffer")
    I = mw.heads * mw.dim_head
    out = grads or {}
    out.setdefault("dX", torch.empty((R, E), device=dev))
    out.setdefault("d_ln_w", torch.empty(E, device=dev))
    out.setdefault("d_ln_b", torch.empty(E, device=dev))
    out.setdefault("d_wkv", torch.empty((2 * I, E), device=dev))
    out.setdefault("d_wq", torch.empty((I, E), device=dev))
    out.setdefault("d_wo", torch.empty((E, I), device=dev))
    out.setdefault("d_bo", torch.empty(E, device=dev))
    g = L.MergeGrad(d_ln_w=_p(out["d_ln_w"]), d_ln_b=_p(out["d_ln_b"]), d_wkv=_p(out["d_wkv"]), d_wq=_p(out["d_wq"]),
                    d_wo=_p(out["d_wo"]), d_bo=_p(out["d_bo"]), accumulate=int(bool(accumulate)), splits=int(splits),
                    defer=_dp(defer))
    if defer is not None:
        defer.keep.append(ws)
    L.check(L.lib().mhimx_merge_bwd(_stream(), C.byref(mw.c), _p(X), R, _p(dz), _p(out["dX"]), C.byref(g), _p(ws),
                                    ws.numel()), "mhimx_merge_bwd")
    return out


def act_bwd(dH, H, pre, act, drop_p=0.0, drop_seed=0, drop_mask=None, rows=None, colsum_out=None, want_colsum=False,
            accumulate=False, drop_tick=None):
    M, E = dH.shape
    if want_colsum and colsum_out is None:
        colsum_out = torch.empty(E, device=dH.device)
    ws = torch.empty(1024 * E, device=dH.device) if colsum_out is not None else None
    L.check(L.lib().mhimx_act_bwd(_stream(), _p(dH), _p(H), _p(pre), M, E, int(act), float(drop_p),
                                  int(drop_seed) & 0xFFFFFFFFFFFFFFFF, _p(drop_mask), _p(rows), _p(colsum_out),
                                  int(bool(accumulate)), _p(ws), 0 if ws is None else ws.numel() * 4, _p(drop_tick)), "mhimx_act_bwd")
    return (dH, colsum_out) if colsum_out is not None else dH


def mul_colsum(dH, dact, colsum_out=None, want_colsum=True, accumulate=False, defer=None):
    _chk(dH, name="dH"); _chk(dact, name="dact")
    M, E = dH.shape
    if want_colsum and colsum_out is None:
        colsum_out = torch.empty(E, device=dH.device)
    ws = torch.empty(1024 * E, device=dH.device) if colsum_out is not None else None
    L.check(L.lib().mhimx_mul_colsum(_stream(), _p(dH), _p(dact), M, E, _p(colsum_out), int(bool(accumulate)), _p(ws),
                                     0 if ws is None else ws.numel() * 4, _dp(defer)), "mhimx_mul_colsum")
    if defer is not None:
        defer.keep.append(ws)
    return dH, colsum_out


def rows_dpre(dH, dact16, rows, n_rows, colsum_out=None, accumulate=False, defer=None):
    _chk(dH, name="dH"); _chk(dact16, torch.float16, "dact16"); _chk(rows, torch.int64, "rows")
    E = dH.shape[1]
    dpre = torch.empty((n_rows, E), device=dH.device)
    if colsum_out is None:
        colsum_out = torch.empty(E, device=dH.device)
    ws = torch.empty(1024 * E, device=dH.device)
    L.check(L.lib().mhimx_rows_dpre(_stream(), _p(dH), _p(dact16), _p(rows), int(n_rows), E, _p(dpre), _p(colsum_out), int(bool(accumulate)),
                                      _p(ws), ws.numel() * 4, _dp(defer)), "mhimx_rows_dpre")
    if defer is not None:
        defer.keep.append(ws)
    return dpre, colsum_out


def bag_wgrad_ok(x, E, n_rows):
    return (n_rows >= 1 and E % 128 == 0 and x.shape[1] % 256 == 0 and x.stride(0) % 4 == 0
            and x.shape[0] * x.stride(0) * 4 < (1 << 32))


def bag_ximage_floats(x):
    return -(-x.shape[0] // 32) * 32 * x.shape[1]


def bag_wgrad_ximg_ok(x, E):
    return x.dim() == 2 and x.is_contiguous() and x.shape[1] % 256 == 0 and E % 128 == 0


def bag_wgrad(dH, dact16, x, rows, n_rows, out_w=None, out_b=None, accumulate=False, defer=None, rows_dh="same", want_bias=True,
              dh_compact=False, ride_tail=False, ximg=None, keep=None):
    _chk(dH, name="dH"); _chk(dact16, torch.float16, "dact16"); _chk(rows, torch.int64, "rows")
    if not (x.is_cuda and x.dtype == torch.float32 and x.dim() == 2 and x.stride(1) == 1):
        raise L.MhimxError("x: expected a GPU fp32 matrix with contiguous rows")
    if ximg is not None:
        _chk(ximg, name="ximg"); _chk(keep, torch.uint8, "keep")
        N, E, D = x.shape[0], dH.shape[1], x.shape[1]
        if not bag_wgrad_ximg_ok(x, E) or ximg.numel() < bag_ximage_floats(x) or (keep is not None and keep.numel() < N):
            raise L.MhimxError("bag_wgrad(ximg=): contiguous bag, D % 256 == 0, E % 128 == 0, image / keep flags of the bag's size")
        dev, lib = dH.device, L.lib()
        if out_w is None:
            out_w = torch.empty((E, D), device=dev)
        if out_b is None and want_bias:
            out_b = torch.empty(E, device=dev)
        img = torch.empty(lib.mhimx_wgrad_image_bytes(N, E) // 4, device=dev)
        ws_b = torch.empty(-(-N // 32) * E, device=dev) if want_bias else None
        L.check(lib.mhimx_rows_dpre_image_k(_stream(), _p(dH), _p(dact16), _p(keep), N, E, _p(img), _p(out_b) if want_bias else None,
                                            int(bool(accumulate)), _p(ws_b), ws_b.numel() * 4 if want_bias else 0, _dp(defer)), "mhimx_rows_dpre_image_k")
        ws = torch.empty(lib.mhimx_wgrad_ws_floats(N, E, D), device=dev)
        g = L.BagWgrad(img=_p(img), X=_p(x), ldx=x.stride(0), n_bag_rows=N, rows=None, L=N, E=E, D=D, C=_p(out_w), ldc=out_w.stride(0),
                       accumulate=int(bool(accumulate)), ws=_p(ws), ws_floats=ws.numel(), defer=_dp(defer),
                       ride_tail=int(bool(ride_tail and defer is not None)), ximg=_p(ximg))
        L.check(lib.mhimx_bag_wgrad(_stream(), C.byref(g)), "mhimx_bag_wgrad")
        if defer is not None:
            defer.keep.extend((ws_b, ws, img))
        return out_w, out_b
    rows_h = rows if isinstance(rows_dh, str) else rows_dh
    _chk(rows_h, torch.int64, "rows_dh")
    E, D = dH.shape[1], x.shape[1]
    n_rows = int(n_rows)
    dev = dH.device
    lib = L.lib()
    if out_w is None:
        out_w = torch.empty((E, D), device=dev)
    if out_b is None and want_bias:
        out_b = torch.empty(E, device=dev)
    img = torch.empty(lib.mhimx_wgrad_image_bytes(n_rows, E) // 4, device=dev)
    ws_b = torch.empty(-(-n_rows // 32) * E, device=dev) if want_bias else None
    fn = lib.mhimx_rows_dpre_image_c if dh_compact else lib.mhimx_rows_dpre_image
    L.check(fn(_stream(), _p(dH), _p(dact16), _p(rows_h), n_rows, E, _p(img), _p(out_b) if want_bias else None,
                                      int(bool(accumulate)), _p(ws_b), ws_b.numel() * 4 if want_bias else 0, _dp(defer)), "mhimx_rows_dpre_image")
# ... 707 lines not shown
```

Baseline: 33.04 million patch-instances/s.

## Ride the pool finalize's partial-merge level onto the merge partials kernel

Splits the pool finalize kernel's first stage, which merges the G partial (max, sum, z) tiles into one level-one result, into a rider routine. When armed, that routine runs as extra trailing blocks of the merge partials kernel and writes lvl/z_r to workspace. The later finalize kernel then reads those precomputed values and only combines them with the tail tokens. The goal is to take the serial partial reduction off the critical path of the finalize launch by overlapping it with merge work. The cost is added plumbing: a host-side argument blob passed between the pool and merge calls, plus extra blocks and grid size in the merge kernel.

```diff
diff --git a/include/mhimx.h b/include/mhimx.h
--- a/include/mhimx.h
+++ b/include/mhimx.h
@@ -137,6 +137,12 @@
 } mhimx_scorer;
 
 typedef struct {
+  int32_t armed;
+  int32_t rode;
+  uint64_t blob[14];
+} mhimx_tail_ride;
+
+typedef struct {
   const float* T1; int64_t M1; const float* T2; int64_t M2;
   float* s; float* stats; float* z;
   float* u_pre;
@@ -154,6 +160,7 @@
   const float* tail_wa_t;
   int64_t tail_row0;
   int32_t no_backward;
+  mhimx_tail_ride* tail_ride;
 } mhimx_pool_io;
 int64_t mhimx_abmil_pool_ws_bytes(int64_t M, int64_t E, int64_t A, int32_t gated);
 int mhimx_abmil_pool_fwd(void* stream, const mhimx_scorer* sc, mhimx_pool_io* io);
@@ -278,6 +285,7 @@
   int64_t own_lo, own_n;
   float rep;
   int32_t rows_done;
+  mhimx_tail_ride* tail_ride;
 } mhimx_merge;
 int64_t mhimx_merge_ws_bytes(int64_t R, int64_t E, int64_t k, int64_t heads, int64_t dim_head);
 int mhimx_merge_fwd(void* stream, const mhimx_merge* m, const float* X, int64_t R, float* z, float* q_new,
diff --git a/mhim_mil_amd/_lib.py b/mhim_mil_amd/_lib.py
--- a/mhim_mil_amd/_lib.py
+++ b/mhim_mil_amd/_lib.py
@@ -103,6 +103,10 @@
                 ("wa_frag", c_f32p), ("gate_drop_p", C.c_float), ("gate_drop_seed", C.c_uint64)]
 
 
+class TailRide(C.Structure):
+    _fields_ = [("armed", C.c_int32), ("rode", C.c_int32), ("blob", C.c_uint64 * 14)]
+
+
 class PoolIO(C.Structure):
     _fields_ = [("T1", c_f32p), ("M1", C.c_int64), ("T2", c_f32p), ("M2", C.c_int64),
                 ("s", c_f32p), ("stats", c_f32p), ("z", c_f32p), ("u_pre", c_f32p),
@@ -111,7 +115,7 @@
                 ("excl", C.c_void_p), ("ride_jobs", C.c_void_p), ("n_ride_jobs", C.c_int32),
                 ("phase", C.c_int32), ("tail_tokens", C.c_int32), ("ride_merge", C.c_void_p), ("ride_X", c_f32p), ("ride_R", C.c_int64),
                 ("ride_ws", C.c_void_p), ("ride_ws_bytes", C.c_int64), ("rode_merge", C.c_int32), ("tail_wa_t", c_f32p), ("tail_row0", C.c_int64),
-                ("no_backward", C.c_int32)]
+                ("no_backward", C.c_int32), ("tail_ride", C.POINTER(TailRide))]
 
 
 class PoolGrad(C.Structure):
@@ -129,7 +133,7 @@
                 ("wkv_t", c_f32p), ("wq_t", c_f32p), ("wo_t", c_f32p),
                 ("mm", C.c_float), ("drop_p", C.c_float), ("drop_seed", C.c_uint64), ("prec", C.c_int32), ("drop_tick", C.c_void_p),
                 ("wkv_frag", c_f32p), ("x_rows", c_i64p), ("prepared", C.c_int32), ("own_lo", C.c_int64), ("own_n", C.c_int64),
-                ("rep", C.c_float), ("rows_done", C.c_int32)]
+                ("rep", C.c_float), ("rows_done", C.c_int32), ("tail_ride", C.POINTER(TailRide))]
 
 
 class MergeGrad(C.Structure):
diff --git a/mhim_mil_amd/csrc/fin_tail.hpp b/mhim_mil_amd/csrc/fin_tail.hpp
--- /dev/null
+++ b/mhim_mil_amd/csrc/fin_tail.hpp
@@ -0,0 +1,155 @@
+#pragma once
+#include <string.h>
+
+#include "common.hpp"
+
+namespace mhimx {
+
+constexpr int FIN_MAXTOK = 6;
+constexpr int FIN_E = 512, FIN_A = 128;
+constexpr int FIN_ROWS_NC = 16;
+constexpr int FIN_ROWS_BLOCKS = FIN_E / FIN_ROWS_NC;
+
+struct FinRowsRide { const float *pm, *pl, *pz; float *lvl, *z_r; int G, blocks; };
+
+struct TailRideArgs { const float *pm, *pl, *pz; float *lvl, *z_r; int32_t G, pad; };
+static_assert(sizeof(TailRideArgs) <= sizeof(mhimx_tail_ride::blob), "the riders' arguments fit mhimx_tail_ride.blob");
+inline FinRowsRide fin_tail_ride(const mhimx_tail_ride* ride) {
+  TailRideArgs a;
+  memcpy(&a, ride->blob, sizeof(a));
+  return FinRowsRide{a.pm, a.pl, a.pz, a.lvl, a.z_r, a.G, FIN_ROWS_BLOCKS};
+}
+
+MHIMX_DEV float fin_wgt(float pm, float mx) { return pm == -INFINITY ? 0.f : __expf(pm - mx); }
+MHIMX_DEV float fin_mul(float a, float b) {
+#pragma clang fp contract(off)
+  return a * b;
+}
+
+template <int NC>
+struct FinRowsRegs { float pzv[8], pmv[8], plv[1024 / (16 * NC)], pwv[1024 / (16 * NC)]; };
+template <int NC>
+MHIMX_DEV void fin_rows_load(FinRowsRegs<NC>& r, const float* __restrict__ pm, const float* __restrict__ pl, const float* __restrict__ pz, int G, int E,
+                             int e0) {
+  constexpr int NT = 16 * NC, NW = NT / 64;
+  const int tid = threadIdx.x, lane = tid & 63, wave = tid >> 6;
+  const int g = tid / NC, e = e0 + tid % NC;
+#pragma unroll
+  for (int q = 0; q < 8; ++q) {
+    const int b = g + 16 * q;
+    r.pmv[q] = b < G ? pm[b] : -INFINITY;
+    r.pzv[q] = (e < E && b < G) ? pz[(int64_t)b * E + e] : 0.f;
+  }
+#pragma unroll
+  for (int v = 0; v < 16 / NW; ++v) {
+    const int b = (v * NW + wave) * 64 + lane;
+    r.pwv[v] = b < G ? pm[b] : -INFINITY;
+    r.plv[v] = b < G ? pl[b] : 0.f;
+  }
+}
+template <int NC>
+MHIMX_DEV void fin_rows_merge(const FinRowsRegs<NC>& r, float* red, float* acc16, const float* __restrict__ pm, const float* __restrict__ pz, int G,
+                              int E, int e0, float& m_r, float& L_r, float& z_r) {
+  constexpr int NT = 16 * NC, NW = NT / 64;
+  const int tid = threadIdx.x, lane = tid & 63, wave = tid >> 6;
+  const int g = tid / NC, c = tid % NC, e = e0 + c;
+  const float (&pzv)[8] = r.pzv;
+  const float (&pmv)[8] = r.pmv;
+  const float (&plv)[16 / NW] = r.plv;
+  const float (&pwv)[16 / NW] = r.pwv;
+  float m = pwv[0];
+#pragma unroll
+  for (int v = 1; v < 16 / NW; ++v) m = fmaxf(m, pwv[v]);
+  m = wave_max(m);
+  if (lane == 0) red[wave] = m;
+  __syncthreads();
+  float mx = red[0];
+#pragma unroll
+  for (int w = 1; w < NW; ++w) mx = fmaxf(mx, red[w]);
+  __syncthreads();
+#pragma unroll
+  for (int v = 0; v < 16 / NW; ++v) {
+    const float lp = wave_sum(fin_mul(plv[v], fin_wgt(pwv[v], mx)));
+    if (lane == 0) red[v * NW + wave] = lp;
+  }
+  __syncthreads();
+  float L = 0.f;
+#pragma unroll
+  for (int w = 0; w < 16; ++w) L += red[w];
+  float acc = 0.f;
+  if (e < E) {
+#pragma unroll
+    for (int q = 0; q < 8; ++q)
+      if (g + 16 * q < G) acc = fmaf(pzv[q], fin_wgt(pmv[q], mx), acc);
+#pragma unroll 8
+    for (int b = g + 128; b < G; b += 16) acc = fmaf(pz[(int64_t)b * E + e], fin_wgt(pm[b], mx), acc);
+  }
+  acc16[g * NC + c] = acc;
+  __syncthreads();
+  float a = 0.f;
+  if (tid < NC) {
+#pragma unroll
+    for (int w = 0; w < 16; ++w) a += acc16[w * NC + tid];
+  }
+  m_r = mx; L_r = L; z_r = a;
+}
+
+MHIMX_DEV void fin_rows_rider(int block, float* lds, const FinRowsRide& r) {
+  float m_r, L_r, z_r;
+  FinRowsRegs<FIN_ROWS_NC> rg;
+  fin_rows_load(rg, r.pm, r.pl, r.pz, r.G, FIN_E, block * FIN_ROWS_NC);
+  fin_rows_merge(rg, lds, lds + 16, r.pm, r.pz, r.G, FIN_E, block * FIN_ROWS_NC, m_r, L_r, z_r);
+  if (threadIdx.x < FIN_ROWS_NC) r.z_r[block * FIN_ROWS_NC + threadIdx.x] = z_r;
+  if (block == 0 && threadIdx.x == 0) { r.lvl[0] = m_r; r.lvl[1] = L_r; }
+}
+
+MHIMX_DEV void fin_tok_weights(const float* __restrict__ wa_t, int a, int ch, float (&wv)[64]) {
+  const float* wp = wa_t + (int64_t)(ch * 64) * FIN_A + a;
+#pragma unroll
+  for (int u = 0; u < 64; ++u) wv[u] = wp[(int64_t)u * FIN_A];
+  asm volatile("s_waitcnt vmcnt(0)" ::: "memory");
+}
+template <int NTOK>
+MHIMX_DEV void fin_tok_products(const float (&wv)[64], const float* tk, int ld, float (&acc)[NTOK]) {
+#pragma unroll
+  for (int i = 0; i < NTOK; ++i) acc[i] = 0.f;
+#pragma unroll
+  for (int u4 = 0; u4 < 64; u4 += 4) {
+#pragma unroll
+    for (int i = 0; i < NTOK; ++i) {
+      const float4 tv = *reinterpret_cast<const float4*>(&tk[i * ld + u4]);
+      acc[i] += tv.x * wv[u4] + tv.y * wv[u4 + 1] + tv.z * wv[u4 + 2] + tv.w * wv[u4 + 3];
+    }
+  }
+}
+MHIMX_DEV float fin_chunk_sum(const float* up, int i, int a, const float* __restrict__ ba) {
+  constexpr int S = FIN_MAXTOK * FIN_A;
+  const float* p = up + i * FIN_A + a;
+  const float v = ((p[0] + p[S]) + (p[2 * S] + p[3 * S])) + ((p[4 * S] + p[5 * S]) + (p[6 * S] + p[7 * S]));
+  return v + (ba ? ba[a] : 0.f);
+}
+MHIMX_DEV float fin_tok_score(const float* us_i, const float* __restrict__ wc, const float* __restrict__ bc, int A, int act) {
+  const int lane = threadIdx.x & 63;
+  float v = 0.f;
+  for (int a = lane; a < A; a += 64) v += wc[a] * act_fwd(us_i[a], act);
+  return wave_sum(v) + (bc ? bc[0] : 0.f);
+}
+MHIMX_DEV void fin_combine(float m_r, float L_r, float z_r, const float* stok, int K, const float (&tke)[FIN_MAXTOK], float& mx, float& L, float& z) {
+  mx = m_r;
+  for (int i = 0; i < K; ++i) mx = fmaxf(mx, stok[i]);
+  const float c = fin_wgt(m_r, mx);
+  L = fin_mul(c, L_r);
+  float wt[FIN_MAXTOK];
+#pragma unroll
+  for (int i = 0; i < FIN_MAXTOK; ++i) {
+    wt[i] = i < K ? __expf(stok[i] - mx) : 0.f;
+    L += wt[i];
+  }
+  float a = fin_mul(c, z_r);
+#pragma unroll
+  for (int i = 0; i < FIN_MAXTOK; ++i)
+    if (i < K) a = fmaf(wt[i], tke[i], a);
+  z = a / L;
+}
+
+}
diff --git a/mhim_mil_amd/csrc/mca2.hip b/mhim_mil_amd/csrc/mca2.hip
--- a/mhim_mil_amd/csrc/mca2.hip
+++ b/mhim_mil_amd/csrc/mca2.hip
@@ -1,6 +1,7 @@
 #include <math.h>
 #include <string.h>
 
+#include "fin_tail.hpp"
 #include "mca2_rows.hpp"
 
 namespace mhimx {
@@ -39,8 +40,15 @@
 template <int MODE>
 __global__ __launch_bounds__(M2_THREADS) void merge2_partials_kernel(M2Parts in, int live_only, const float* __restrict__ ln_w,
                                                                     const float* __restrict__ ln_b, float* __restrict__ out,
-                                                                    float* __restrict__ stats, float* __restrict__ raw_stats, BagBatch bb) {
+                                                                    float* __restrict__ stats, float* __restrict__ raw_stats, FinRowsRide fr,
+                                                                    BagBatch bb) {
   __shared__ float lds[M2_PARTIALS_LDS];
+  static_assert(M2_PARTIALS_LDS >= 16 + 16 * FIN_ROWS_NC, "the level-one riders fit the kernel's LDS");
+  if (MODE == 1 && fr.blocks > 0 && (int)blockIdx.x >= (int)gridDim.x - fr.blocks) {
+    if (blockIdx.z) { MHIMX_BAG(fr.pm); MHIMX_BAG(fr.pl); MHIMX_BAG(fr.pz); MHIMX_BAG(fr.lvl); MHIMX_BAG(fr.z_r); }
+    fin_rows_rider((int)blockIdx.x - ((int)gridDim.x - fr.blocks), lds, fr);
+    return;
+  }
   if (blockIdx.z) {
     in.pm = bag_ptr(in.pm, bb); in.pl = bag_ptr(in.pl, bb); in.psd = bag_ptr(in.psd, bb); in.y = bag_ptr(in.y, bb);
     MHIMX_BAG(out); MHIMX_BAG(stats); MHIMX_BAG(raw_stats);
@@ -107,7 +115,7 @@
 
 int merge2_side_launch(hipStream_t st, int stage, const Merge2Side& sd) {
   if (stage == 1) hipLaunchKernelGGL(merge2_partials_kernel<0>, bgrid((unsigned)(sd.J * 4)), dim3(M2_THREADS), 0, st, m2_parts_tiles(sd.w, sd.w.upart),
-                                     sd.w.own_n > 0 ? 1 : 0, sd.ln_w, sd.ln_b, const_cast<float*>(sd.U), (float*)nullptr, (float*)nullptr, cur_batch());
+                                     sd.w.own_n > 0 ? 1 : 0, sd.ln_w, sd.ln_b, const_cast<float*>(sd.U), (float*)nullptr, (float*)nullptr, FinRowsRide{}, cur_batch());
   else if (stage == 2) hipLaunchKernelGGL(merge2_grads1_kernel, bgrid(M2_GRADS1_BLOCKS), dim3(M2_THREADS), 0, st, sd, cur_batch());
   else hipLaunchKernelGGL(merge2_grads2_kernel, bgrid(M2_GRADS2_BLOCKS), dim3(M2_THREADS), 0, st, sd, cur_batch());
   MHIMX_LAUNCH_CHECK();
@@ -179,8 +187,13 @@
   Merge2Ws w;
   if (int r = merge2_fwd_rows(st, m, X, R, ws, ws_bytes, &w)) return r;
   const int J = M2_H * (int)m->k;
-  hipLaunchKernelGGL(merge2_partials_kernel<1>, bgrid((unsigned)(J * 4)), dim3(M2_THREADS), 0, st, m2_parts_tiles(w, w.ypart), 0, m->ln_w, m->ln_b, w.Y,
-                     w.stats, (float*)nullptr, cur_batch());
+  FinRowsRide fr = {};
+  if (m->tail_ride && m->tail_ride->armed) {
+    fr = fin_tail_ride(m->tail_ride);
+    m->tail_ride->rode = 1;
+  }
+  hipLaunchKernelGGL(merge2_partials_kernel<1>, bgrid((unsigned)(J * 4 + fr.blocks)), dim3(M2_THREADS), 0, st, m2_parts_tiles(w, w.ypart), 0, m->ln_w,
+                     m->ln_b, w.Y, w.stats, (float*)nullptr, fr, cur_batch());
   MHIMX_LAUNCH_CHECK();
   return merge2_fwd_tail(st, m, z, q_new, update_q, w);
 }
@@ -191,7 +204,7 @@
   if (int r = merge2_fwd_rows(st, m, X, R, ws, ws_bytes, &w)) return r;
   const int J = M2_H * (int)m->k;
   hipLaunchKernelGGL(merge2_partials_kernel<2>, dim3((unsigned)(J * 4)), dim3(M2_THREADS), 0, st, m2_parts_tiles(w, w.ypart), 0, m->ln_w, m->ln_b,
-                     part + 3 * M2_JP, (float*)nullptr, part, BagBatch{});
+                     part + 3 * M2_JP, (float*)nullptr, part, FinRowsRide{}, BagBatch{});
   MHIMX_LAUNCH_CHECK();
   return 0;
 }
@@ -205,7 +218,7 @@
   MHIMX_CHECK_ARG(ar.ok(), "merge_fwd_finish: workspace too small");
   const int J = M2_H * (int)m->k;
   hipLaunchKernelGGL(merge2_partials_kernel<1>, dim3((unsigned)(J * 4)), dim3(M2_THREADS), 0, st, m2_parts_shards(parts, W), 0, m->ln_w, m->ln_b, w.Y,
-                     w.stats, (float*)nullptr, BagBatch{});
+                     w.stats, (float*)nullptr, FinRowsRide{}, BagBatch{});
   MHIMX_LAUNCH_CHECK();
   return merge2_fwd_tail(st, m, z, q_new, update_q, w);
 }
diff --git a/mhim_mil_amd/csrc/rows.hip b/mhim_mil_amd/csrc/rows.hip
--- a/mhim_mil_amd/csrc/rows.hip
+++ b/mhim_mil_amd/csrc/rows.hip
@@ -1,6 +1,7 @@
 #include <math.h>
 #include <string.h>
 
+#include "fin_tail.hpp"
 #include "mca2_rows.hpp"
 #include "reduce_jobs.hpp"
 
@@ -183,7 +184,6 @@
   if (blockIdx.x == 0 && threadIdx.x == 0) { stats[0] = mx; stats[1] = L; }
 }
 
-constexpr int FIN_MAXTOK = 6;
 #ifdef MHIMX_FT_PROF
 __device__ unsigned long long ft_prof[16];
 #define FT_STAMP(i) do { __syncthreads(); if (threadIdx.x == 0 && blockIdx.x == 0) ft_prof[i] = wall_clock64(); } while (0)
@@ -197,27 +197,29 @@
                                                                          const float* __restrict__ wa, const float* __restrict__ wa_t,
                                                                          const float* __restrict__ ba, const float* __restrict__ wc,
                                                                          const float* __restrict__ bc, int A, int act,
-                                                                         float* __restrict__ u_pre_tail, float* __restrict__ s_tail, BagBatch bb) {
+                                                                         float* __restrict__ u_pre_tail, float* __restrict__ s_tail,
+                                                                         const float* __restrict__ lvl, const float* __restrict__ z_r1,
+                                                                         BagBatch bb) {
   if (blockIdx.z) {
     MHIMX_BAG(pm); MHIMX_BAG(pl); MHIMX_BAG(pz); MHIMX_BAG(stats); MHIMX_BAG(z); MHIMX_BAG(T); MHIMX_BAG(rows_tail); MHIMX_BAG(wa_t); MHIMX_BAG(u_pre_tail);
-    MHIMX_BAG(s_tail);
+    MHIMX_BAG(s_tail); MHIMX_BAG(lvl); MHIMX_BAG(z_r1);
   }
   __shared__ float red[16];
-  __shared__ float wgt[2 * MAX_PART];
   __shared__ float acc16[16][64];
   __shared__ __attribute__((aligned(16))) float tks[FIN_MAXTOK][512];
   __shared__ float up[8][FIN_MAXTOK][128];
   __shared__ float us[FIN_MAXTOK][128];
   __shared__ float stok[8];
   const int tid = threadIdx.x, lane = tid & 63, wave = tid >> 6;
+  const int e = blockIdx.x * 64 + lane;
   FT_STAMP(0);
-  const float pm1 = tid < G ? pm[tid] : -INFINITY, pl1 = tid < G ? pl[tid] : 0.f;
-  const int e = blockIdx.x * 64 + lane;
-  float pzv[8];
-#pragma unroll
-  for (int q = 0; q < 8; ++q) {
-    const int b = wave + 16 * q;
-    pzv[q] = (e < E && b < G) ? pz[(int64_t)b * E + e] : 0.f;
+  FinRowsRegs<64> rg;
+  float m_r = 0.f, L_r = 0.f, zr = 0.f;
+  if (lvl) {
+    m_r = lvl[0]; L_r = lvl[1];
+    if (tid < 64 && e < E) zr = z_r1[e];
+  } else {
+    fin_rows_load(rg, pm, pl, pz, G, E, blockIdx.x * 64);
   }
   for (int idx = tid; idx < FIN_MAXTOK * (E / 4); idx += FIN_THREADS) {
     const int i = idx / (E / 4), c4 = idx - i * (E / 4);
@@ -228,34 +230,18 @@
     }
     reinterpret_cast<float4*>(&tks[i][0])[c4] = v;
   }
-  if (wa_t && A == 128 && E == 512) {
+  if (wa_t && A == FIN_A && E == FIN_E) {
     const int a = tid & 127, ch = tid >> 7;
-    const float* wp = wa_t + (int64_t)(ch * 64) * A + a;
     float acc[FIN_MAXTOK];
-#pragma unroll
-    for (int i = 0; i < FIN_MAXTOK; ++i) acc[i] = 0.f;
     float wv[64];
-#pragma unroll
-    for (int u = 0; u < 64; ++u) wv[u] = wp[(int64_t)u * A];
-    asm volatile("s_waitcnt vmcnt(0)" ::: "memory");
+    fin_tok_weights(wa_t, a, ch, wv);
     __syncthreads();
     FT_STAMP(1);
-#pragma unroll
-    for (int u4 = 0; u4 < 64; u4 += 4) {
-#pragma unroll
-      for (int i = 0; i < FIN_MAXTOK; ++i) {
-        const float4 tv = *reinterpret_cast<const float4*>(&tks[i][ch * 64 + u4]);
-        acc[i] += tv.x * wv[u4] + tv.y * wv[u4 + 1] + tv.z * wv[u4 + 2] + tv.w * wv[u4 + 3];
-      }
-    }
+    fin_tok_products<FIN_MAXTOK>(wv, &tks[0][ch * 64], 512, acc);
 #pragma unroll
     for (int i = 0; i < FIN_MAXTOK; ++i) up[ch][i][a] = acc[i];
     __syncthreads();
-    if (tid < K * 128) {
-      const int i = tid >> 7, aa = tid & 127;
-      float v = ((up[0][i][aa] + up[1][i][aa]) + (up[2][i][aa] + up[3][i][aa])) + ((up[4][i][aa] + up[5][i][aa]) + (up[6][i][aa] + up[7][i][aa]));
-      us[i][aa] = v + (ba ? ba[aa] : 0.f);
-    }
+    if (tid < K * 128) us[tid >> 7][tid & 127] = fin_chunk_sum(&up[0][0][0], tid >> 7, tid & 127, ba);
   } else {
     float4 w0[8], w1[8];
 #pragma unroll
@@ -282,62 +268,25 @@
   if (blockIdx.x == 0)
     for (int idx = tid; idx < K * A; idx += FIN_THREADS) u_pre_tail[idx] = us[idx / A][idx % A];
   if (wave < K) {
-    float v = 0.f;
-    for (int a = lane; a < A; a += 64) v += wc[a] * act_fwd(us[wave][a], act);
-    v = wave_sum(v) + (bc ? bc[0] : 0.f);
+    const float v = fin_tok_score(us[wave], wc, bc, A, act);
     if (lane == 0) {
       stok[wave] = v;
       if (blockIdx.x == 0) s_tail[wave] = v;
     }
   }
   FT_STAMP(3);
-  float m = wave_max(pm1);
-  if (lane == 0) red[wave] = m;
-  __syncthreads();
-  float mx = red[0];
-#pragma unroll
-  for (int w = 1; w < 16; ++w) mx = fmaxf(mx, red[w]);
-  for (int i = 0; i < K; ++i) mx = fmaxf(mx, stok[i]);
-  __syncthreads();
-  float lp = 0.f;
-  if (tid < G) {
-    const float w = (pm1 == -INFINITY) ? 0.f : __expf(pm1 - mx);
-    wgt[tid] = w;
-    lp = pl1 * w;
-  }
-  lp = wave_sum(lp);
-  if (lane == 0) red[wave] = lp;
-  __syncthreads();
-  float L = 0.f;
-#pragma unroll
-  for (int w = 0; w < 16; ++w) L += red[w];
-  float wt[FIN_MAXTOK];
-#pragma unroll
-  for (int i = 0; i < FIN_MAXTOK; ++i) {
-    wt[i] = i < K ? __expf(stok[i] - mx) : 0.f;
-    L += wt[i];
-  }
+  if (lvl) __syncthreads();
+  else fin_rows_merge(rg, red, &acc16[0][0], pm, pz, G, E, blockIdx.x * 64, m_r, L_r, zr);
   FT_STAMP(4);
-  float acc = 0.f;
-  if (e < E) {
-#pragma unroll
-    for (int q = 0; q < 8; ++q)
-      if (wave + 16 * q < G) acc += pzv[q] * wgt[wave + 16 * q];
-#pragma unroll 8
-    for (int b = wave + 128; b < G; b += 16) acc += pz[(int64_t)b * E + e] * wgt[b];
-  }
-  acc16[wave][lane] = acc;
-  __syncthreads();
-  if (wave == 0 && e < E) {
-    float a = 0.f;
-#pragma unroll
-    for (int w = 0; w < 16; ++w) a += acc16[w][lane];
-#pragma unroll
-    for (int i = 0; i < FIN_MAXTOK; ++i)
-      if (i < K) a += wt[i] * tks[i][e];
-    z[e] = a / L;
-  }
-  if (blockIdx.x == 0 && tid == 0) { stats[0] = mx; stats[1] = L; }
+  if (tid < 64) {
+    float tke[FIN_MAXTOK];
+#pragma unroll
+    for (int i = 0; i < FIN_MAXTOK; ++i) tke[i] = (i < K && e < E) ? tks[i][e] : 0.f;
+    float mx, L, zv;
+    fin_combine(m_r, L_r, zr, stok, K, tke, mx, L, zv);
+    if (e < E) z[e] = zv;
+    if (blockIdx.x == 0 && tid == 0) { stats[0] = mx; stats[1] = L; }
+  }
   FT_STAMP(5);
 }
 
@@ -913,7 +862,18 @@
                     "pool_fwd: the two-call forward takes the one-pass scorer shapes, one segment, 1..%d tail tokens, no class projections", FIN_MAXTOK);
     const int tiles = (int)cdiv(Ms1, 32);
     const int G1 = tiles < MAX_PART ? tiles : MAX_PART;
+    float* const lvl = w.pm + MAX_PART;
+    float* const z_r = w.pz + (int64_t)MAX_PART * E;
+    const int64_t* rows_tail = (io->rows1 && io->tail_row0 < 0) ? io->rows1 + Ms1 : nullptr;
+    const int64_t row0 = io->rows1 ? io->tail_row0 : Ms1;
     if (io->phase == 1) {
+      if (io->tail_ride) {
+        mhimx_tail_ride* ride = io->tail_ride;
+        ride->rode = 0;
+        ride->armed = 1;
+        const TailRideArgs a = {w.pm, w.pl, w.pz, lvl, z_r, (int32_t)G1, 0};
+        memcpy(ride->blob, &a, sizeof(a));
+      }
       M2RowsFwd mfbuf;
       const void* mf = nullptr;
       io->rode_merge = 0;
@@ -927,9 +887,10 @@
                                       w.pz, MAX_PART, io->rows1, nullptr, io->ride_jobs, io->n_ride_jobs, mf);
       return g1 < 0 ? g1 : 0;
     }
+    const bool rode = io->tail_ride && io->tail_ride->armed && io->tail_ride->rode;
     hipLaunchKernelGGL(pool_finalize_tok_kernel, bgrid((unsigned)cdiv(E, 64)), dim3(FIN_THREADS), 0, st, w.pm, w.pl, w.pz, G1, (int)E, io->stats, io->z, io->T1,
-                       (io->rows1 && io->tail_row0 < 0) ? io->rows1 + Ms1 : nullptr, io->rows1 ? io->tail_row0 : Ms1, (int)K, sc->wa, io->tail_wa_t, sc->ba, sc->wc,
-                       sc->bc, (int)A, sc->act, u_pre + Ms1 * ldu, io->s + Ms1, cur_batch());
+                       rows_tail, row0, (int)K, sc->wa, io->tail_wa_t, sc->ba, sc->wc, sc->bc, (int)A, sc->act, u_pre + Ms1 * ldu, io->s + Ms1,
+                       rode ? lvl : (const float*)nullptr, z_r, cur_batch());
     MHIMX_LAUNCH_CHECK();
     return 0;
   }
diff --git a/mhim_mil_amd/csrc/step.hip b/mhim_mil_amd/csrc/step.hip
--- a/mhim_mil_amd/csrc/step.hip
+++ b/mhim_mil_amd/csrc/step.hip
@@ -225,20 +225,22 @@
   io.ws = g.pool_ws; io.ws_bytes = g.pool_ws_bytes; io.rows1 = g.rows_all + g.R;
   io.tail_row0 = -1;
   io.phase = 1; io.tail_tokens = (int32_t)k;
+  f->tail = mhimx_tail_ride{};
   if (dag) {
     if (int r = dag_edge(dag->ev[0], dag->main_st, dag->side_st)) return r;
   } else {
     io.ride_merge = &mw; io.ride_X = g.Hbuf; io.ride_R = g.R; io.ride_ws = g.merge_ws; io.ride_ws_bytes = g.merge_ws_bytes;
+    io.tail_ride = &f->tail; mw.tail_ride = &f->tail;
   }
   if (int r = mhimx_abmil_pool_fwd(dag ? dag->side_st : stream, &f->sc_s, &io)) return r;
   mw.rows_done = io.rode_merge;
   if (int r = mhimx_merge_fwd(stream, &mw, g.Hbuf, g.R, g.Hbuf + g.N * E, g.q_out, 1, g.merge_ws, g.merge_ws_bytes)) return r;
-  mw.rows_done = 0;
+  mw.rows_done = 0; mw.tail_ride = nullptr;
   if (dag)
     if (int r = dag_edge(dag->ev[1], dag->side_st, dag->main_st)) return r;
   io.phase = 2; io.tail_wa_t = im.wa_t; io.tail_row0 = g.N;
   if (int r = mhimx_abmil_pool_fwd(stream, &f->sc_s, &io)) return r;
-  io.phase = 0; io.ride_merge = nullptr;
+  io.phase = 0; io.ride_merge = nullptr; io.tail_ride = nullptr;
   return 0;
 }
 
diff --git a/mhim_mil_amd/csrc/step_mid.hpp b/mhim_mil_amd/csrc/step_mid.hpp
--- a/mhim_mil_amd/csrc/step_mid.hpp
+++ b/mhim_mil_amd/csrc/step_mid.hpp
@@ -16,7 +16,7 @@
   void* merge_ws; int64_t merge_ws_bytes;
 };
 struct MidDag { hipStream_t main_st, side_st; hipEvent_t* ev; };
-struct MidFwd { mhimx_merge mw; mhimx_scorer sc_s; mhimx_pool_io io_s; };
+struct MidFwd { mhimx_merge mw; mhimx_scorer sc_s; mhimx_pool_io io_s; mhimx_tail_ride tail; };
 struct MidImg { void* img; const void* dact; float* part; };
 
 mhimx_merge mid_merge_params(const mhimx_step_cfg& c);
diff --git a/mhim_mil_amd/mhim.py b/mhim_mil_amd/mhim.py
--- a/mhim_mil_amd/mhim.py
+++ b/mhim_mil_amd/mhim.py
@@ -564,9 +564,10 @@
                 q_param = self.merge.global_q_mm.data.view(self.merge.k, -1)
             k = self.merge.k
             if "merge_ws" in prep and k <= 6 and rows_all.numel() - plan.R > k:
-                st, rode = ops.abmil_pool_fwd_split(sc, Hbuf, rows_all[plan.R:], k, ride_merge=(mw, Hbuf, prep["merge_ws"]))
+                st, rode = ops.abmil_pool_fwd_split(sc, Hbuf, rows_all[plan.R:], k, ride_merge=(mw, Hbuf, prep["merge_ws"]),
+                                                    tail_ride=True)
                 _, _, mws = ops.merge_fwd(mw, Hbuf, z_out=Hbuf[N:], update_q=plan.training, q_out=q_param if plan.training else None,
-                                          ws=prep["merge_ws"], rows_done=rode)
+                                          ws=prep["merge_ws"], rows_done=rode, tail_ride=st.tail_ride)
                 ops.abmil_pool_fwd_finish(sc, st, wa_t=prep.get("wa_t"), tail_row0=N)
             else:
                 _, _, mws = ops.merge_fwd(mw, Hbuf, z_out=Hbuf[N:], update_q=plan.training, q_out=q_param if plan.training else None,
diff --git a/mhim_mil_amd/ops.py b/mhim_mil_amd/ops.py
--- a/mhim_mil_amd/ops.py
+++ b/mhim_mil_amd/ops.py
@@ -337,12 +337,17 @@
                         ride_jobs=None if self.ride is None else C.cast(self.ride[0], C.c_void_p), n_ride_jobs=0 if self.ride is None else self.ride[1])
 
 
-def abmil_pool_fwd_split(sc: ScorerW, T1, rows1, tail_tokens, ride_merge=None):
+def abmil_pool_fwd_split(sc: ScorerW, T1, rows1, tail_tokens, ride_merge=None, tail_ride=False, ws=None):
     _chk(T1, name="T1"); _chk(rows1, torch.int64, "rows1")
     st = PoolState(T1, None, 0, None, rows1=rows1)
     st.tail_tokens = int(tail_tokens)
+    st.ws = ws
     io = st.io(sc)
     io.phase, io.tail_tokens = 1, st.tail_tokens
+    st.tail_ride = None
+    if tail_ride:
+        st.tail_ride = L.TailRide()
+        io.tail_ride = C.pointer(st.tail_ride)
     if ride_merge is not None:
         mw, X, ws = ride_merge
         io.ride_merge, io.ride_X = C.cast(C.pointer(mw.c), C.c_void_p), _p(X)
@@ -355,6 +360,8 @@
     io = st.io(sc)
     io.phase, io.tail_tokens = 2, st.tail_tokens
     io.tail_wa_t, io.tail_row0 = _p(wa_t), int(tail_row0)
+    if getattr(st, "tail_ride", None) is not None:
+        io.tail_ride = C.pointer(st.tail_ride)
     L.check(L.lib().mhimx_abmil_pool_fwd(_stream(), C.byref(sc.c), C.byref(io)), "mhimx_abmil_pool_fwd (phase 2)")
     return st
 
@@ -513,7 +520,7 @@
         return torch.empty(n, device=device, dtype=torch.uint8)
 
 
-def merge_fwd(mw: MergeW, X, z_out=None, update_q=True, ws=None, q_out=None, rows_done=False):
+def merge_fwd(mw: MergeW, X, z_out=None, update_q=True, ws=None, q_out=None, rows_done=False, tail_ride=None):
     _chk(X, name="X")
     R = X.shape[0] if mw.x_rows is None else mw.x_rows.shape[0]
     dev = X.device
@@ -521,9 +528,12 @@
     q_new = (q_out if q_out is not None else torch.empty((mw.k, mw.E), device=dev)) if update_q else None
     ws = ws if ws is not None else mw.ws_for(R, dev)
     mw.c.rows_done = int(bool(rows_done))
+    if tail_ride is not None:
+        mw.c.tail_ride = C.pointer(tail_ride)
     L.check(L.lib().mhimx_merge_fwd(_stream(), C.byref(mw.c), _p(X), R, _p(z), _p(q_new), int(bool(update_q)), _p(ws),
                                     ws.numel()), "mhimx_merge_fwd")
     mw.c.rows_done = 0
+    mw.c.tail_ride = None
     return z, q_new, ws
 
 
```

Measured after the change: 33.23 million patch-instances/s (median of 6 runs). About the same (+0.6%).
